# YuePanEdward/MULLS

Measured on AMD Instinct MI355X. Metric: scan-pair registrations/sec (64-beam ~120k pts, 20 ICP iters); dT vs ref, higher is better.
Workload: dtype f32

## Files before the change

### mulls_amd/csrc/batch.cpp

```cpp
#include "batch.h"

namespace mulls_drv
{
void rows12(const double colmajor[16], double out[12])
{
	for (int r = 0; r < 3; r++)
		for (int c = 0; c < 4; c++)
			out[r * 4 + c] = colmajor[r + 4 * c];
}


void fill_crop_box(const RunParams &rp, const double tgt_bound[6], const uint32_t keys[6], mulls_result &R)
{
	R.cropped = rp.crop ? 1 : 0;
	for (int k = 0; k < 3 && rp.crop; k++)
	{
		const uint32_t kmin = keys[k], kmax = keys[3 + k];
		const bool none = kmin == 0xffffffffu && kmax == 0u;
		const double mmin = none ? 1.7976931348623157e308 : (double)ord_to_float(kmin);
		const double mmax = none ? -1.7976931348623157e308 : (double)ord_to_float(kmax);
		const double b1min = tgt_bound[k], b1max = tgt_bound[3 + k];
		const float pad = 1.0f;
		R.crop_box[k] = ((b1min > mmin) ? b1min : mmin) - pad;
		R.crop_box[3 + k] = ((b1max < mmax) ? b1max : mmax) + pad;
// ... 537 lines not shown
			d.src_off = (uint32_t)so;
			d.tgt_off = (uint32_t)to;
			so += d.src_cap;
			to += t.n;
			if (t.n > MULLS_BIG_CLOUD)
			{
				const uint32_t slot = (uint32_t)B->big_clouds_h.size(), first = (uint32_t)B->big_segs_h.size();
				d.big_slot = slot + 1u;
				for (uint32_t k = 0; k < t.n; k += MULLS_SEG)
					B->big_segs_h.push_back({(uint32_t)p, (uint32_t)c, k, slot});
				B->big_clouds_h.push_back({(uint32_t)p, (uint32_t)c, first, (uint32_t)B->big_segs_h.size() - first});
				B->n_big_tgt++;
			}
			if (d.src_cap > MULLS_BIG_CLOUD)
			{
				const uint32_t slot = (uint32_t)B->big_clouds_h.size(), first = (uint32_t)B->big_segs_h.size();
				d.src_big_slot = slot + 1u;
				for (uint32_t k = 0; k < d.src_cap; k += MULLS_SEG)
					B->big_segs_h.push_back({(uint32_t)p, (uint32_t)c | MULLS_BIG_SRC_SIDE, k, slot});
				B->big_clouds_h.push_back({(uint32_t)p, (uint32_t)c | MULLS_BIG_SRC_SIDE, first, (uint32_t)B->big_segs_h.size() - first});
			}
		}
		{
			uint64_t src_total = 0;
			bool seg = false;
			for (int c = 0; c < MULLS_NC; c++)
			{
				const CloudDesc &d = B->descs_h[p * MULLS_NC + c];
				src_total += d.src_n0;
				seg = seg || d.src_big_slot != 0u;
			}
			B->src_one_wg[p] = !seg && src_total <= MULLS_SRC_SETUP_CAP;
		}
		for (int c = 0; c < MULLS_NC; c++)
		{
			const CloudDesc &d = B->descs_h[p * MULLS_NC + c];
			const uint32_t chunks = d.src_cap > 8192u ? 8u : 1u;
			for (uint32_t k = 0; k < d.src_cap; k += MULLS_BLOCK * chunks)
			{
				Job j = {(uint32_t)p, (uint32_t)c, k, chunks};
				(B->src_one_wg[p] ? one_wg_jobs : B->setup_jobs_h).push_back(j);
			}
		}
		rows12(pairs[p].init_guess, B->setup_h[p].guess);
		std::memcpy(B->setup_h[p].tgt_bound, pairs[p].tgt_bound, sizeof(double) * 6);
		{
			Mat4 g;
			std::memcpy(g.v, pairs[p].init_guess, sizeof(g.v));
			const Mat4 gi = mulls::invert4(g);
			mulls::rotation_quaternion(gi, B->setup_h[p].inv_q);
			B->setup_h[p].inv_t[0] = gi.at(0, 3);
			B->setup_h[p].inv_t[1] = gi.at(1, 3);
			B->setup_h[p].inv_t[2] = gi.at(2, 3);
			B->setup_h[p].inv_t[3] = std::acos(std::min(1.0, std::fabs(B->setup_h[p].inv_q[0])));
		}
	}
	B->n_setup_jobs_rest = (uint32_t)B->setup_jobs_h.size();
	B->setup_jobs_h.insert(B->setup_jobs_h.end(), one_wg_jobs.begin(), one_wg_jobs.end());
	if (stage_rec >= (1ull << 32) || so >= (1ull << 31) || to >= (1ull << 31))
	{
		ctx->err = "batch too large (>= 2^31 points)";
		return MULLS_E_INVALID;
	}
	B->n_src = so;
	B->n_tgt = to;

	int rc = MULLS_OK;
	auto A = [&](int r) { if (rc == MULLS_OK) rc = r; };
	bool winner_grew = false, cand_grew = false;
	const size_t SG = (size_t)ctx->opt[MULLS_OPT_STAGGER];
	A(grow(ctx, &B->stage, &B->cap_stage, stage_rec));
	A(grow(ctx, &B->tmp_pos, &B->cap_src[0], so, nullptr, 12 * SG));
	A(grow(ctx, &B->tmp_nrm, &B->cap_src[1], so, nullptr, 13 * SG));
	A(grow(ctx, &B->spos, &B->cap_src[2], so, nullptr, 1 * SG));
	A(grow(ctx, &B->snrm, &B->cap_src[3], so, nullptr, 2 * SG));
	A(grow(ctx, &B->flag, &B->cap_src[4], so, nullptr, 3 * SG));
	A(grow(ctx, &B->match, &B->cap_src[5], so, nullptr, 4 * SG));
	A(grow(ctx, &B->nn_idx, &B->cap_src[6], so, nullptr, 5 * SG));
	A(grow(ctx, &B->wd, &B->cap_src[7], so, nullptr, 6 * SG));
	A(grow(ctx, &B->nn_d2, &B->cap_src[8], so, nullptr, 7 * SG));
	A(grow(ctx, &B->nn_hint, &B->cap_src[9], 2 * so, nullptr, 8 * SG));
	A(grow(ctx, &B->mq, &B->cap_src[10], 2 * so, nullptr, 9 * SG));
	A(grow(ctx, &B->nn_cand, &B->cap_src[11], so, &cand_grew, 14 * SG));
	A(grow(ctx, &B->tpos, &B->cap_tgt[0], to));
	A(grow(ctx, &B->tnrm, &B->cap_tgt[1], to));
	A(grow(ctx, &B->tsorted, &B->cap_tgt[2], to, nullptr, 10 * SG));
	A(grow(ctx, &B->tmap, &B->cap_tgt[4], to, nullptr, 11 * SG));
	A(grow(ctx, &B->winner, &B->cap_tgt[3], to, &winner_grew));
	A(grow(ctx, &B->descs, &B->cap_pairs[0], (size_t)n * MULLS_NC));
	A(grow(ctx, &B->setup, &B->cap_pairs[1], (size_t)n));
	A(grow(ctx, &B->states, &B->cap_pairs[2], (size_t)n));
	A(grow(ctx, &B->outs, &B->cap_outs, (size_t)n));
	A(grow(ctx, &B->bbox, &B->cap_pairs[3], (size_t)n * 6));
	A(grow(ctx, &B->grids, &B->cap_pairs[4], (size_t)n * MULLS_NC));
	A(grow(ctx, &B->setup_jobs, &B->cap_setup_jobs, B->setup_jobs_h.size()));
	A(grow(ctx, &B->big_segs, &B->cap_big[0], B->big_segs_h.size()));
	A(grow(ctx, &B->big_clouds, &B->cap_big[1], B->big_clouds_h.size()));
	A(grow(ctx, &B->seg_cnt, &B->cap_big[2], B->big_segs_h.size()));
	A(grow(ctx, &B->big_box, &B->cap_big[3], (B->big_clouds_h.size() + B->big_segs_h.size()) * 6));
	if (!B->ticket)
	{
		A(dmalloc(ctx, &B->ticket, 32));
		if (rc == MULLS_OK && hipMemset(B->ticket, 0, 32 * sizeof(uint32_t)) != hipSuccess)
			rc = MULLS_E_HIP;
	}
	A(grow_pinned(ctx, &B->states_h, &B->cap_pin[0], (size_t)n, hipHostMallocMapped));
	A(grow_pinned(ctx, &B->outs_h, &B->cap_pin[1], (size_t)n, hipHostMallocMapped));
	A(grow_pinned(ctx, &B->bbox_h, &B->cap_pin[2], (size_t)n * 6, hipHostMallocDefault));
	A(grow_pinned(ctx, &B->upload_h, &B->cap_pin[3], std::max<size_t>(stage_rec, 1) * 16, hipHostMallocDefault));
	if (rc == MULLS_OK && !B->epoch_h)
	{
		if (hipHostMalloc((void **)&B->epoch_h, 256, hipHostMallocMapped) != hipSuccess)
			rc = MULLS_E_HIP;
		else
			std::memset((void *)B->epoch_h, 0, 256);
	}
	if (rc != MULLS_OK)
		return rc;
	if (hipHostGetDevicePointer((void **)&B->states_pin, B->states_h, 0) != hipSuccess ||
		hipHostGetDevicePointer((void **)&B->outs_pin, B->outs_h, 0) != hipSuccess ||
		hipHostGetDevicePointer((void **)&B->epoch_dev, (void *)B->epoch_h, 0) != hipSuccess)
	{
		ctx->err = "pinned host memory setup failed";
		return MULLS_E_HIP;
	}
	std::memset(B->states_h, 0, sizeof(PairState) * n);
	for (int p = 0; p < n; p++)
		for (int k = 0; k < 6; k++)
			B->bbox_h[p * 6 + k] = k < 3 ? 0xffffffffu : 0u;

	struct DevCopy
	{
		size_t dst;
		const void *src;
		size_t bytes;
	};
	std::vector<DevCopy> dev_copies;
	struct HostCopy
	{
		uint8_t *dst;
		const uint8_t *src;
		uint32_t n, stride, fmt;
	};
	std::vector<HostCopy> host_copies;
	std::vector<size_t> first_copy_of_pair(n + 1, 0);
	for (int p = 0; p < n; p++)
	{
		first_copy_of_pair[p] = host_copies.size();
		for (int c = 0; c < MULLS_NC; c++)
		{
			const CloudDesc &d = B->descs_h[p * MULLS_NC + c];
			const mulls_cloud *cl[3] = {&pairs[p].src[c], &pairs[p].tgt[c], &pairs[p].src_down[c]};
			const uint32_t off[3] = {d.src_stage, d.tgt_stage, d.sd_stage}, cnt[3] = {d.src_n0, d.tgt_n0, d.sd_n0};
			const uint32_t fmt[3] = {d.stage_fmt & 3u, (d.stage_fmt >> 2) & 3u, (d.stage_fmt >> 4) & 3u};
			for (int k = 0; k < (d.sd_stage != d.src_stage ? 3 : 2); k++)
			{
				if (!cnt[k])
					continue;
				const uint8_t *src = (const uint8_t *)cl[k]->pts;
				if (fmt[k] == MULLS_STAGE_AOS48)
				{
					if (cl[k]->stride != MULLS_POINT_BYTES)
					{
						ctx->err = "device-resident cloud with stride != 48";
						return MULLS_E_INVALID;
					}
// ... 324 lines not shown
```

### mulls_amd/csrc/batch.h

```cpp
#pragma once
#include <hip/hip_runtime_api.h>

#include <algorithm>
#include <atomic>
#include <chrono>
#include <cmath>
#include <cstdio>
#include <cstdlib>
#include <cstring>
#include <string>
#include <vector>

#include "../../include/mulls_hip.h"
#include "device_types.h"
#include "hostmath.h"
#include "icp_step.h"
#include "launch.h"
#include "ctx.h"

struct SegCopier
{
	mulls_ctx *ctx;
	std::vector<CopySeg> segs;
	struct Pending
	{
		void *dst;
		const void *src;
		size_t bytes;
	};
	std::vector<Pending> host;
	explicit SegCopier(mulls_ctx *c) : ctx(c) {}
	void add_host(void *dst, const void *src, size_t bytes)
	{
		if (bytes)
			host.push_back({dst, src, bytes});
	}
	void add_dev(void *dst, const void *src, size_t bytes)
	{
		const size_t piece = (size_t)0xfffffff0u;
		for (size_t off = 0; off < bytes; off += piece)
		{
			const size_t b = std::min(piece, bytes - off);
			segs.push_back({(unsigned long long)(uintptr_t)dst + off, (unsigned long long)(uintptr_t)src + off, (uint32_t)b, 0u});
		}
	}
	int flush(hipStream_t st);
};

struct mulls_batch : BatchDev
{
	int n = 0;
	size_t n_src = 0, n_tgt = 0;
	std::vector<CloudDesc> descs_h;
	std::vector<PairSetup> setup_h;
	std::vector<Job> setup_jobs_h;
	uint32_t n_setup_jobs_rest = 0;
	std::vector<uint8_t> src_one_wg;
	std::vector<uint32_t> setup_tab_h;
	uint32_t tg_split[MULLS_TG_BUCKETS + 1] = {}, crop_split[4] = {}, srcp_split[2] = {};
	size_t cap_setup_tab = 0;
	std::vector<Job> big_segs_h, big_clouds_h;
	uint32_t n_big_tgt = 0;
	std::vector<Job> jobs_h;
	std::vector<Job> cjobs_h;
	std::vector<Job> cjobs_dev_h;
	std::vector<Job> bjobs_h;
	std::vector<Job> fjobs_h;
	std::vector<Job> ejobs_h;
	std::vector<uint32_t> lclouds_h;
	int tier_mode = -1;
	std::vector<Job> tjobs_h;
	std::vector<uint32_t> ajobs_h;
	uint32_t ajob_split[2][4] = {{0, 0, 0, 0}, {0, 0, 0, 0}};
	IcpOut *icp_outs_pin = nullptr;
	size_t cap_icp_pin = 0;
	std::string jobs_key;
	uint32_t njobs = 0;
	uint4 *nn_cand = nullptr;
	uint32_t tick = 1;
	size_t cap_outs = 0;
	size_t cap_big[4] = {};
	size_t cap_bjobs[4] = {};
	size_t cap_bm_cs = 0;
	size_t cap_bm_rank = 0;
	size_t cap_ajobs = 0;
	size_t cap_icp_outs = 0;
	size_t cap_steps = 0;
	uint32_t epoch2 = 0, epoch3 = 0;
	int nsub = 1;
	double fill_ms = 0.0, fill_pack_ms = 0.0;
	uint64_t fill_bytes = 0;
	size_t cap_wl = 0;
	unsigned long long *dbg = nullptr;
	size_t cap_bm = 0, cap_pf = 0;
	PairState *states_h = nullptr;
	PairOut *outs_h = nullptr;
	volatile uint32_t *epoch_h = nullptr;
	uint32_t *epoch_dev = nullptr;
	uint32_t epoch = 0;
	uint32_t epoch1 = 0;
	uint32_t *bbox_h = nullptr;
	uint8_t *upload_h = nullptr;
	CloudDesc *descs_init = nullptr;
	uint32_t *bbox_init = nullptr;
	std::string dev_key;
	size_t cap_jobs[6] = {}, cap_cells[2] = {};
	size_t cap_stage = 0, cap_src[13] = {}, cap_tgt[5] = {}, cap_pairs[5] = {}, cap_setup_jobs = 0, cap_pin[4] = {};
};

namespace mulls_drv
{
using mulls::Mat4;
using mulls::Mat6;

inline float ord_to_float(uint32_t k)
{
	const uint32_t u = (k & 0x80000000u) ? (k & 0x7fffffffu) : ~k;
	float f;
	std::memcpy(&f, &u, sizeof(f));
	return f;
}
inline int metric_of(int c) { return (c == MULLS_PILLAR || c == MULLS_BEAM) ? 1 : (c == MULLS_VERTEX ? 2 : 0); }
inline int packed(int r, int c) { return r * 6 - r * (r - 1) / 2 + (c - r); }
void rows12(const double colmajor[16], double out[12]);

struct PairHost : mulls::PairIter
{
	bool first = true;
	uint32_t alive_prev[MULLS_NC];
};

void fill_crop_box(const RunParams &rp, const double tgt_bound[6], const uint32_t keys[6], mulls_result &R);
int check_params(mulls_ctx *ctx, const mulls_params *P);
void init_cert(const mulls_ctx *ctx, RunParams &rp);
int subbatch_count(const mulls_ctx *ctx, int n);
void options_init(mulls_ctx *ctx);
bool option_value_ok(int option, double *value);
uint32_t lds_dedup_max_pts();
void assign_tiers(mulls_batch *B, const uint8_t used[MULLS_NC], int mode);
void build_jobs(mulls_batch *B, const mulls_params *P, int nsub, int mode);
int wait_epoch_word(mulls_ctx *ctx, volatile uint32_t *word, uint32_t want, hipEvent_t last = nullptr, hipStream_t stream = nullptr);
inline int wait_epoch(mulls_ctx *ctx, mulls_batch *B) { return wait_epoch_word(ctx, B->epoch_h, B->epoch); }
void unpack_out(const mulls_batch *B, const uint8_t used[MULLS_NC], int p, PairOut &o, bool comb = false);
uint32_t lds_cells_for(uint32_t cap);
int choose_tier(const mulls_ctx *ctx, const mulls_batch *B, const uint8_t used[MULLS_NC], uint32_t *lds_cap, const mulls_params *P_mixed = nullptr);
int batch_fill(mulls_ctx *ctx, mulls_batch *B, const mulls_pair *pairs, int n, const mulls_params *P = nullptr);
int prepare_run(mulls_ctx *ctx, mulls_batch *B, const mulls_params *P_jobs, RunParams &rp, uint32_t *lds_cap_out, int *tier_out, int nsub = 0, bool allow_mixed = false);
void queue_clone_crop(hipStream_t st, const mulls_batch *B, const RunParams &rp);
bool setup_former_shape(const RunParams &rp);
int apply_keep_masks(mulls_ctx *ctx, const mulls_batch *B, const std::vector<uint8_t> &skeep, const std::vector<uint8_t> &tkeep, const char *what);
void queue_target_grids(hipStream_t st, const mulls_batch *B, const RunParams &rp, int tier, bool fused_tgt);
int queue_tier_search(mulls_ctx *ctx, const mulls_batch *B, const RunParams &rp, int tier, uint32_t lds_cap, uint32_t parity);
mulls::IcpConst icp_const(const mulls_params *P);
int take_epochs(mulls_ctx *ctx, mulls_batch *B, uint32_t n, RunParams &rp);

struct EvTimer
{
	mulls_ctx *ctx;
	hipStream_t stream = nullptr;
	int base = 0;
	int used = 0;
// ... 36 lines not shown
```

### mulls_amd/csrc/device_types.h

```cpp
#pragma once
#include <stdint.h>

#define MULLS_NC 6
#define MULLS_NTERM 27
#define MULLS_BLOCK 256
#define MULLS_SRC_PER_THREAD 2
#define MULLS_SRC_PER_BLOCK (MULLS_BLOCK * MULLS_SRC_PER_THREAD)
#define MULLS_NN_BLOCK 128
#define MULLS_NN_PTS 4
#define MULLS_TILE 2048

#define MULLS_MAXCELLS 65536u
#define MULLS_BM_MAXWORDS (1u << 22)
#define MULLS_BM_TOTALWORDS (1u << 28)
#define MULLS_BM_H0 0.25f
#define MULLS_LDS_BLOCK 1024
#define MULLS_LDS_MAXPTS 9728u
#define MULLS_ACC_BLOCK 128
#define MULLS_LDS_QCHUNK 1024u
#define MULLS_LDS_AUX (320u + 2u * MULLS_LDS_QCHUNK)
#define MULLS_CERT_BLOCK 512
#define MULLS_CERT_SMALL 64u
#define MULLS_CERT_SMALL_LOCKSTEP 512u
#define MULLS_LDS_CELL_RESERVE 9216
#ifndef MULLS_LDS_GROUP
#define MULLS_LDS_GROUP 8u
#endif
#define MULLS_TG_BUCKETS 4
#define MULLS_SRC_SETUP_CAP 4096u
#define MULLS_BIG_CLOUD 16384u
#define MULLS_BIG_SRC_SIDE 0x100u
#define MULLS_SEG 4096u
#define MULLS_GRID_GROUP 16u
#define MULLS_BIG_BLOCK 512
#define MULLS_BIG_CLASS_MAX (3u * MULLS_BIG_BLOCK)
#define MULLS_JOB_CLASS 0x80000000u
#define MULLS_SMALL_SRC_MAX 4096u
#define MULLS_TIER_BRUTE 0u
#define MULLS_TIER_BM 1u
#define MULLS_TIER_LDS 2u
#define MULLS_GRID_H0 1.3f

#define MULLS_F_ALIVE 1u
#define MULLS_F_VALID 2u

struct CloudDesc
{
	uint32_t src_stage;
	uint32_t tgt_stage;
	uint32_t src_n0;
	uint32_t tgt_n0;
	uint32_t src_off;
	uint32_t tgt_off;
	uint32_t src_n;
	uint32_t tgt_n;
	uint32_t alive_cur;
	uint32_t alive_next;
	uint32_t n_matched;
	uint32_t valid_next;
	uint32_t n_valid;
	uint32_t job_begin;
	uint32_t job_end;
	uint32_t sd_stage;
	uint32_t sd_n0;
	uint32_t src_cap;
	uint32_t big_slot;
	uint32_t src_big_slot;
	uint32_t n_search;
	uint32_t stage_fmt;
	uint32_t tier;
	uint32_t grid_slot;
};
#define MULLS_STAGE_AOS48 0u
#define MULLS_STAGE_PACK32 1u
#define MULLS_STAGE_PACK28 2u

struct GridDesc
{
	float ox, oy, oz;
	float inv_h, h;
	uint32_t nx, ny, nz;
	uint32_t ncell;
	uint32_t cell_off;
	uint32_t wpr;
	uint32_t nocc;
};

struct PairState
{
	double T[12];
	double x[6];
	float thr[MULLS_NC];
	int32_t iter;
	int32_t active;
	int32_t want_residual;
	int32_t pad_[3];
};

struct PairSetup
{
	double guess[12];
	double tgt_bound[6];
	double inv_q[4];
	double inv_t[4];
};

#define MULLS_NTERM_PAD 28
struct PairOut
{
	double sums[MULLS_NC][MULLS_NTERM_PAD];
	double comb[MULLS_NTERM_PAD];
	uint32_t n_valid[MULLS_NC];
	uint32_t n_alive[MULLS_NC];
	uint32_t src_n[MULLS_NC];
	uint32_t tgt_n[MULLS_NC];
	uint32_t bbox[6];
	uint32_t pad_[2];
};

struct IcpOut
{
	double T[16];
	double info[36];
	double sigma2;
	unsigned long long src_pts, tgt_pts, corr_pts;
	float ratio;
	int32_t code, iters, singular, trace_len;
	uint32_t ncorr[MULLS_NC], nsrc0[MULLS_NC], ntgt0[MULLS_NC], bbox[6];
	uint32_t pad_;
	unsigned long long tgt_job_pts, pair_evals;
};

struct Job
{
	uint32_t pair;
	uint32_t cls;
	uint32_t start;
	uint32_t count;
};

#define MULLS_COPY_SEGS 24
struct CopySeg
{
	unsigned long long dst, src;
	uint32_t bytes, pad_;
};
struct CopyArgs
{
	CopySeg seg[MULLS_COPY_SEGS];
};

struct RunParams
{
	uint8_t used[MULLS_NC];
	uint8_t w_balance, w_resid, w_dist, w_inten;
	uint8_t crop;
	uint8_t undistort;
	uint8_t normal_shooting;
	uint8_t faithful;
	uint8_t rej_strict;
	float z_xy_ratio;
	float win_pt, win_pl, win_li;
	uint8_t force_class_w;
	uint8_t bm_auto;
	float class_w_value;
	double cos_bearing;
	int32_t resid_from_iter;
	uint32_t debug_stop;
	uint32_t cell_stride;
	uint32_t grid_maxcells;
	float grid_h0;
	float bm_h0;
	uint32_t bm_maxwords;
	uint32_t bm_stride;
	uint32_t pull_comb;
	uint32_t lds_dedup;
	uint32_t tick_base;
	uint32_t cert;
	float cert_slack_min, cert_slack_max, cert_slack_rate;
	uint32_t kcert;
	uint32_t kcert_min;
	uint4 *cand;
	const float4 *tgt_stage;
	const uint16_t *tgt_map;
	unsigned long long *dbg_ticks;
};
```

### mulls_amd/csrc/device_util.h

```cpp

#pragma once
#include <hip/hip_runtime.h>
#include <stdint.h>

#include "device_types.h"

#pragma clang fp contract(off)

__device__ __forceinline__ uint32_t xcd_job(uint32_t b, uint32_t n)
{
	const uint32_t q = n >> 3, r = n & 7u, x = b & 7u;
	return x * q + min(x, r) + (b >> 3);
}

namespace
{

typedef float f2 __attribute__((ext_vector_type(2)));

__device__ __forceinline__ uint32_t f2ord(float f)
{
	uint32_t u = __float_as_uint(f);
	return (u & 0x80000000u) ? ~u : (u | 0x80000000u);
}
__device__ __forceinline__ float ord2f(uint32_t k)
{
	uint32_t u = (k & 0x80000000u) ? (k & 0x7fffffffu) : ~k;
	return __uint_as_float(u);
}

__device__ __forceinline__ void load_staged(const float4 *__restrict__ stage, uint32_t off, uint32_t fmt, uint32_t n, uint32_t i, float4 &pos, float4 &nrm)
{
	if (fmt == MULLS_STAGE_PACK32)
	{
		pos = stage[(size_t)off + i];
		nrm = stage[(size_t)off + n + i];
	}
	else if (fmt == MULLS_STAGE_PACK28)
	{
		pos = stage[(size_t)off + i];
		const float *f = reinterpret_cast<const float *>(stage + (size_t)off + n) + 3u * (size_t)i;
		nrm = make_float4(f[0], f[1], f[2], 0.0f);
	}
	else
	{
		const float4 *rec = stage + (size_t)off + (size_t)i * 3;
		const float4 a = rec[0], b = rec[1], c = rec[2];
		pos = make_float4(a.x, a.y, a.z, c.x);
		nrm = make_float4(b.x, b.y, b.z, c.y);
	}
}
__device__ __forceinline__ void identity_step(float4 &p, float4 &n)
{
	const double x = p.x, y = p.y, z = p.z, nx = n.x, ny = n.y, nz = n.z;
	p.x = (float)(1.0 * x + 0.0 * y + 0.0 * z + 0.0);
	p.y = (float)(0.0 * x + 1.0 * y + 0.0 * z + 0.0);
	p.z = (float)(0.0 * x + 0.0 * y + 1.0 * z + 0.0);
	n.x = (float)(1.0 * nx + 0.0 * ny + 0.0 * nz);
	n.y = (float)(0.0 * nx + 1.0 * ny + 0.0 * nz);
	n.z = (float)(0.0 * nx + 0.0 * ny + 1.0 * nz);
}
__device__ __forceinline__ float4 load_staged_pos(const float4 *__restrict__ stage, uint32_t off, uint32_t fmt, uint32_t i)
{
	return fmt == MULLS_STAGE_AOS48 ? stage[(size_t)off + (size_t)i * 3] : stage[(size_t)off + i];
}

__device__ __forceinline__ void tgt_record(const float4 *__restrict__ tgt_stage, const uint16_t *__restrict__ tgt_map, const CloudDesc &d, uint32_t m,
											const float4 *__restrict__ tpos, const float4 *__restrict__ tnrm, float4 &q, float4 &n)
{
	if (tgt_map)
		load_staged(tgt_stage, d.tgt_stage, (d.stage_fmt >> 2) & 3u, d.tgt_n0, tgt_map[d.tgt_off + m], q, n);
	else
		q = tpos[d.tgt_off + m], n = tnrm[d.tgt_off + m];
}
__device__ __forceinline__ float4 tgt_point(const float4 *__restrict__ tgt_stage, const uint16_t *__restrict__ tgt_map, const CloudDesc &d, uint32_t m,
											 const float4 *__restrict__ tpos)
{
	return tgt_map ? load_staged_pos(tgt_stage, d.tgt_stage, (d.stage_fmt >> 2) & 3u, tgt_map[d.tgt_off + m]) : tpos[d.tgt_off + m];
}

__device__ __forceinline__ bool class_called(const RunParams &rp, const CloudDesc &d, int cls)
{
	return rp.used[cls] && d.alive_cur >= 3u && d.tgt_n >= 3u;
}

__device__ __forceinline__ uint32_t block_sum_u32(uint32_t v, uint32_t *lds4)
{
	for (int off = 32; off > 0; off >>= 1)
		v += __shfl_down(v, off);
	int lane = threadIdx.x & 63, wave = threadIdx.x >> 6;
	__syncthreads();
	if (lane == 0)
		lds4[wave] = v;
	__syncthreads();
	return lds4[0] + lds4[1] + lds4[2] + lds4[3];
}

}

namespace
{
__device__ __forceinline__ int grid_cell(float v, float o, float inv_h, uint32_t n)
{
	const float c = floorf((v - o) * inv_h);
	return (int)fminf(fmaxf(c, 0.0f), (float)(n - 1u));
}
__device__ __forceinline__ uint32_t grid_cell_id(const GridDesc &g, float x, float y, float z)
{
	return ((uint32_t)grid_cell(z, g.oz, g.inv_h, g.nz) * g.ny + (uint32_t)grid_cell(y, g.oy, g.inv_h, g.ny)) * g.nx +
		   (uint32_t)grid_cell(x, g.ox, g.inv_h, g.nx);
}
struct BmGrid
{
	const unsigned long long *bm;
	const uint32_t *pf;
	const uint32_t *cs;
};
__device__ __forceinline__ void bm_row_range(const BmGrid &B, uint32_t rowword, uint32_t xa, uint32_t xb, uint32_t &lo, uint32_t &hi)
{
	const uint32_t wa = rowword + (xa >> 6), wb = rowword + (xb >> 6);
	const unsigned long long A = B.bm[wa], Z = B.bm[wb];
	const uint32_t r0 = B.pf[wa] + (uint32_t)__popcll(A & ((1ull << (xa & 63u)) - 1ull));
	const uint32_t r1 = B.pf[wb] + (uint32_t)__popcll(Z & (~0ull >> (63u - (xb & 63u))));
	lo = hi = 0;
	if (r1 > r0)
	{
		lo = B.cs[r0];
		hi = B.cs[r1];
	}
}
__device__ __forceinline__ void grid_scan_box(const GridDesc &g, const BmGrid &B, const float4 *__restrict__ ts,
											   float px, float py, float pz, float R, uint32_t sub, float &best, int &bi)
{
	const float Rm = R * 1.0001f + 1e-4f;
	const int x0 = grid_cell(px - Rm, g.ox, g.inv_h, g.nx), x1 = grid_cell(px + Rm, g.ox, g.inv_h, g.nx);
	const int y0 = grid_cell(py - Rm, g.oy, g.inv_h, g.ny), y1 = grid_cell(py + Rm, g.oy, g.inv_h, g.ny);
	const int z0 = grid_cell(pz - Rm, g.oz, g.inv_h, g.nz), z1 = grid_cell(pz + Rm, g.oz, g.inv_h, g.nz);
	const int nyc = y1 - y0 + 1, nrows = nyc * (z1 - z0 + 1);
	const uint32_t gshift = (threadIdx.x & 63u) & ~(MULLS_GRID_GROUP - 1u);
	for (int base = 0; base < nrows; base += (int)MULLS_GRID_GROUP)
	{
		const int j = base + (int)sub;
		uint32_t lo = 0, hi = 0;
		if (j < nrows)
		{
			const uint32_t rowword = ((uint32_t)(z0 + j / nyc) * g.ny + (uint32_t)(y0 + j % nyc)) * g.wpr;
			bm_row_range(B, rowword, (uint32_t)x0, (uint32_t)x1, lo, hi);
		}
		const uint32_t nonempty = (uint32_t)(__ballot(hi > lo) >> gshift) & 0xffffu;
		if (!nonempty)
			continue;
#pragma unroll
		for (int half = 0; half < 2; half++)
		{
			if (!((nonempty >> (8 * half)) & 0xffu))
				continue;
			float4 q[8];
			bool ok[8];
#pragma unroll
			for (int jj = 0; jj < 8; jj++)
			{
				const uint32_t t = __shfl(lo, 8 * half + jj, MULLS_GRID_GROUP) + sub;
// ... 122 lines not shown
```

### mulls_amd/csrc/driver.cpp

```cpp
#include "batch.h"

#include <sched.h>
#include <cstdio>
#include <cstdlib>

#include <mutex>
#include <unordered_map>
namespace
{
std::mutex g_stagger_mu;
std::unordered_map<void *, void *> g_stagger;
}
void staggered_note(void *p, void *base)
{
	std::lock_guard<std::mutex> lk(g_stagger_mu);
	g_stagger[p] = base;
}
void *staggered_base(void *p, bool forget)
{
	std::lock_guard<std::mutex> lk(g_stagger_mu);
	auto it = g_stagger.find(p);
	if (it == g_stagger.end())
		return p;
	void *b = it->second;
// ... 233 lines not shown
		while (!ctx->blocks.empty())
			mulls_block_destroy(ctx, ctx->blocks.back());
		for (auto &e : ctx->ev)
			if (e)
				(void)hipEventDestroy(e);
		if (ctx->ev_setup)
			(void)hipEventDestroy(ctx->ev_setup);
		if (ctx->stream2)
			(void)hipStreamDestroy(ctx->stream2);
		if (ctx->stream)
			(void)hipStreamDestroy(ctx->stream);
		delete ctx;
	}

	const char *mulls_last_error(const mulls_ctx *ctx) { return ctx ? ctx->err.c_str() : "null context"; }

	int mulls_set_profiling(mulls_ctx *ctx, int on)
	try
	{
		if (!ctx)
			return MULLS_E_INVALID;
		ctx->profiling = on == 2 ? 2 : (on != 0 ? 1 : 0);
		return MULLS_OK;
	}
	catch (...)
	{
		return mulls::abi_caught(const_cast<mulls_ctx *>(ctx));
	}

	int mulls_get_profile(const mulls_ctx *ctx, mulls_profile *out)
	try
	{
		if (!ctx || !out)
			return MULLS_E_INVALID;
		*out = ctx->prof;
		return MULLS_OK;
	}
	catch (...)
	{
		return mulls::abi_caught(const_cast<mulls_ctx *>(ctx));
	}

	void *mulls_stream(mulls_ctx *ctx) { return ctx ? (void *)ctx->stream : nullptr; }

	int mulls_set_option(mulls_ctx *ctx, int option, double value)
	{
		if (!ctx || !option_known(option))
			return MULLS_E_INVALID;
		if (!option_value_ok(option, &value))
		{
			ctx->err = "mulls_set_option: value out of the option's range";
			return MULLS_E_INVALID;
		}
		ctx->opt[option] = value;
		return MULLS_OK;
	}
	int mulls_get_option(const mulls_ctx *ctx, int option, double *value)
	{
		if (!ctx || !value || !option_known(option))
			return MULLS_E_INVALID;
		*value = ctx->opt[option];
		return MULLS_OK;
	}

	int mulls_set_nn_mode(mulls_ctx *ctx, int mode)
	try
	{
		if (!ctx || mode < 0 || mode > 4)
			return MULLS_E_INVALID;
		ctx->nn_mode = mode;
		return MULLS_OK;
	}
	catch (...)
	{
		return mulls::abi_caught(const_cast<mulls_ctx *>(ctx));
	}

	void mulls_batch_destroy(mulls_ctx *ctx, mulls_batch *B)
	{
		if (!B)
			return;
		if (ctx)
			(void)hipSetDevice(ctx->device);
		void *dev[] = {B->stage, B->tmp_pos, B->tmp_nrm, B->spos, B->snrm, B->tpos, B->tnrm, B->flag, B->match, B->nn_idx, B->nn_hint, B->nn_cand, B->mq, B->wd,
					   B->nn_d2, B->winner, B->descs, B->setup, B->states, B->outs, B->ticket, B->bbox, B->setup_jobs, B->big_segs, B->big_clouds, B->seg_cnt, B->big_box, B->jobs, B->partial,
					   B->tjobs, B->cjobs, B->bjobs, B->fjobs, B->ejobs, B->lclouds, B->bm_cs, B->wl, B->wl_ctr, B->grids, B->tsorted, B->tmap, B->dbg, B->cell_cnt, B->cell_start, B->bm, B->pf, B->descs_init, B->bbox_init,
					   B->ajobs, B->icp_outs, B->steps, B->bm_rank, B->setup_tab};
		for (void *p : dev)
			if (p)
				staggered_free(p);
		if (B->states_h)
			(void)hipHostFree(B->states_h);
		if (B->outs_h)
			(void)hipHostFree(B->outs_h);
		if (B->bbox_h)
			(void)hipHostFree(B->bbox_h);
		if (B->epoch_h)
			(void)hipHostFree((void *)B->epoch_h);
		if (B->upload_h)
			(void)hipHostFree(B->upload_h);
		if (B->icp_outs_pin)
			(void)hipHostFree(B->icp_outs_pin);
		delete B;
	}

	int mulls_batch_create(mulls_ctx *ctx, const mulls_pair *pairs, int n, mulls_batch **out)
	try
	{
		if (!ctx || !pairs || n <= 0 || !out)
			return MULLS_E_INVALID;
		*out = nullptr;
		mulls_batch *B = new mulls_batch();
		const int rc = batch_fill(ctx, B, pairs, n);
		if (rc != MULLS_OK)
		{
			mulls_batch_destroy(ctx, B);
			return rc;
		}
		*out = B;
		return MULLS_OK;
	}
	catch (...)
	{
		return mulls::abi_caught(const_cast<mulls_ctx *>(ctx));
	}


	int mulls_icp_batch(mulls_ctx *ctx, const mulls_pair *pairs, int n, const mulls_params *params, mulls_result *results)
	try
	{
		if (!ctx)
			return MULLS_E_INVALID;
		int rc = check_params(ctx, params);
		if (rc != MULLS_OK)
			return rc;
		if (!pairs || n <= 0 || !results)
			return MULLS_E_INVALID;
		if (!ctx->scratch)
			ctx->scratch = new mulls_batch();
		rc = batch_fill(ctx, ctx->scratch, pairs, n, params);
		if (rc != MULLS_OK)
			return rc;
		rc = mulls_batch_run(ctx, ctx->scratch, params, results);
		ctx->prof.ms_stage = ctx->scratch->fill_ms, ctx->prof.ms_stage_pack = ctx->scratch->fill_pack_ms, ctx->prof.stage_bytes = ctx->scratch->fill_bytes;
		return rc;
	}
	catch (...)
	{
		return mulls::abi_caught(const_cast<mulls_ctx *>(ctx));
	}

	int mulls_icp(mulls_ctx *ctx, const mulls_pair *pair, const mulls_params *params, mulls_result *result)
	try
	{
		return mulls_icp_batch(ctx, pair, 1, params, result);
	}
	catch (...)
	{
		return mulls::abi_caught(const_cast<mulls_ctx *>(ctx));
	}

}
```

### mulls_amd/csrc/k_reduce.hip

```cpp
#include "device_util.h"
#include "accum.h"
#include "solve_wave.h"

template <int LANES, int MIN_WG>
__global__ __launch_bounds__(LANES, MIN_WG) void k_accum(const uint32_t *__restrict__ leaders, const Job *__restrict__ jobs, const CloudDesc *__restrict__ descs,
														 const PairState *__restrict__ states, RunParams rp, const float4 *__restrict__ spos,
														 const float4 *__restrict__ mq, const uint8_t *__restrict__ flag, float *__restrict__ wd,
														 double *__restrict__ partial)
{
	extern __shared__ __attribute__((aligned(16))) unsigned char lds_raw[];
	__shared__ double part[MULLS_NTERM_PAD];
	const uint32_t job_idx = leaders[xcd_job(blockIdx.x, gridDim.x)];
	const Job job = jobs[job_idx];
	const PairState &ps = states[job.pair];
	if (!ps.active && !ps.want_residual)
		return;
	const CloudDesc *pd = descs + job.pair * MULLS_NC;
	const bool residual_pass = ps.want_residual != 0;
	int cnt[MULLS_NC];
	for (int c = 0; c < MULLS_NC; c++)
		cnt[c] = (int)(class_called(rp, pd[c], c) ? pd[c].valid_next : pd[c].n_valid);
	const AccumCtx A = accum_ctx(rp, job.cls, ps.iter, residual_pass, class_weight(rp, job.cls, residual_pass, cnt));
	trip_sum<true, LANES>(A, ps.x, pd[job.cls], job.start, spos, mq, flag, wd, lds_raw, part);
	if (threadIdx.x < MULLS_NTERM)
		partial[(size_t)job_idx * MULLS_NTERM + threadIdx.x] = part[threadIdx.x];
}

namespace
{
template <typename TS, int W0, int WIN, int MODE, int METRIC, int A0>
__device__ __forceinline__ void add_window(const AccumCtx &A, const double *x, const float4 P, const float4 Q, const float4 N, float wi, float &w, double *acc, const float *wpre)
{
	TS t[WIN];
#pragma unroll
	for (int k = 0; k < WIN; k++)
		t[k] = (TS)0;
	point_terms<TS, W0, WIN, MODE, METRIC>(A, x, P, Q, N, wi, w, t, wpre);
#pragma unroll
	for (int k = 0; k < WIN; k++)
		acc[W0 - A0 + k] += (double)t[k];
}
#ifndef MULLS_ACCW_WIN
#define MULLS_ACCW_WIN 9
#endif
#ifndef MULLS_ACCW_WIN_D
#define MULLS_ACCW_WIN_D 12
#endif
template <typename TS, int W0, int REM, int MODE, int METRIC, int A0>
__device__ __forceinline__ void add_windows(const AccumCtx &A, const double *x, const float4 P, const float4 Q, const float4 N, float wi, float &w, double *acc, const float *wpre)
{
	constexpr int WMAX = sizeof(TS) == 8 ? MULLS_ACCW_WIN_D : MULLS_ACCW_WIN;
	constexpr int WIN = REM < WMAX ? REM : WMAX;
	add_window<TS, W0, WIN, MODE, METRIC, A0>(A, x, P, Q, N, wi, w, acc, wpre);
	if constexpr (REM > WIN)
		add_windows<TS, W0 + WIN, REM - WIN, MODE, METRIC, A0>(A, x, P, Q, N, wi, w, acc, wpre);
}
template <typename TS, int NT, int MODE, int METRIC, int T0, int NTW>
__device__ __forceinline__ void wave_trip(const AccumCtx &A, const double *x, const CloudDesc &d, uint32_t trip0, const float4 *__restrict__ spos, const float4 *__restrict__ mq,
										   const uint8_t *__restrict__ flag, float *__restrict__ wd, double *__restrict__ out, bool owner)
{
	const uint32_t lane = threadIdx.x & 63u;
	const uint32_t src_n = d.src_n, src_off = d.src_off;
	const uint32_t n_here = min(src_n - trip0, (uint32_t)MULLS_ACC_LANES), iters = (n_here + 63u) >> 6;
	const uint32_t last = src_off + src_n - 1u;
	struct Rec
	{
		uint32_t f;
		float4 P, Q;
		float3 N;
		float w;
	};
	const bool need_w = A.residual_pass, writes_w = !A.residual_pass && (METRIC != 2 || !A.faithful);
	auto load = [&](uint32_t i) {
		Rec r;
		const uint32_t g = min(src_off + trip0 + lane + 64u * i, last);
		r.f = flag[g];
		r.P = spos[g], r.Q = mq[2u * g], r.N = *reinterpret_cast<const float3 *>(mq + 2u * g + 1u);
		r.w = need_w ? wd[g] : 0.0f;
		return r;
	};
	double acc[NTW];
#pragma unroll
	for (int k = 0; k < NTW; k++)
		acc[k] = -0.0;
#define MULLS_PIN_REC(r) asm volatile("" : "+v"((r).f), "+v"((r).P.x), "+v"((r).Q.x), "+v"((r).N.x), "+v"((r).w))
#if MULLS_ACCW_PREFETCH
	Rec cur = load(0);
#endif
	for (uint32_t i = 0; i < iters; i++)
	{
#if MULLS_ACCW_PREFETCH
		MULLS_PIN_REC(cur);
		Rec nxt = cur;
		if (i + 1u < iters)
			nxt = load(i + 1u);
#else
		Rec cur = load(i);
		MULLS_PIN_REC(cur);
#endif
		const uint32_t s = trip0 + lane + 64u * i;
		const bool valid = s < src_n && (cur.f & (MULLS_F_ALIVE | MULLS_F_VALID)) == (MULLS_F_ALIVE | MULLS_F_VALID);
		if (valid)
		{
			float w = cur.w;
			const float4 N4 = make_float4(cur.N.x, cur.N.y, cur.N.z, 0.0f);
			const float wi = (A.inten_w && !A.residual_pass) ? point_wi(cur.P, cur.Q) : 1.0f;
			const float wpre = A.residual_pass ? 0.0f : corr_weight(A, METRIC, cur.P, cur.Q, N4, wi);
			add_windows<TS, T0, NTW, MODE, METRIC, T0>(A, x, cur.P, cur.Q, N4, wi, w, acc, A.residual_pass ? nullptr : &wpre);
			if (owner && writes_w)
				wd[src_off + s] = w;
		}
#if MULLS_ACCW_PREFETCH
		cur = nxt;
#endif
	}
	if (NTW == NT && lane < MULLS_NTERM)
	{
		const bool has = MODE == 1 ? li_slot((int)lane) >= 0 : (int)lane < NT;
		if (!has)
			out[lane] = 0.0;
	}
#pragma unroll
	for (int k = 0; k < NTW; k++)
	{
		double sum = acc[k];
		sum = dpp_add_f64<0xB1>(sum);
		sum = dpp_add_f64<0x4E>(sum);
		sum = dpp_add_f64<0x141>(sum);
		sum = dpp_add_f64<0x140>(sum);
		sum = dpp_add_f64_rows<0x142, 0xa>(sum);
		sum = dpp_add_f64_rows<0x143, 0xc>(sum);
		acc[k] = sum;
	}
	if (lane == 63u)
	{
#pragma unroll
		for (int k = 0; k < NTW; k++)
			out[MODE == 1 ? li_term(T0 + k) : T0 + k] = acc[k];
	}
}
}

#ifndef MULLS_ACCW_SPLIT
#define MULLS_ACCW_SPLIT 1
#endif
#ifndef MULLS_ACCW_PREFETCH
#define MULLS_ACCW_PREFETCH 0
#endif
#ifndef MULLS_ACCW_OCC
#define MULLS_ACCW_OCC 4
#endif
#define MULLS_ACCW_WAVES 4
__global__ __launch_bounds__(64 * MULLS_ACCW_WAVES, MULLS_ACCW_OCC) void k_accum_wave(const uint32_t *__restrict__ leaders, uint32_t n_trips, const Job *__restrict__ jobs,
																					   const CloudDesc *__restrict__ descs, const PairState *__restrict__ states, RunParams rp,
																					   const float4 *__restrict__ spos, const float4 *__restrict__ mq, const uint8_t *__restrict__ flag,
																					   float *__restrict__ wd, double *__restrict__ partial)
{
	const uint32_t wave = threadIdx.x >> 6, part = wave % MULLS_ACCW_SPLIT;
	const uint32_t trip = blockIdx.x * (MULLS_ACCW_WAVES / MULLS_ACCW_SPLIT) + wave / MULLS_ACCW_SPLIT;
	if (trip >= n_trips)
		return;
	const uint32_t job_idx = leaders[trip];
	const Job job = jobs[job_idx];
	const PairState &ps = states[job.pair];
	if (!ps.active && !ps.want_residual)
		return;
	const CloudDesc *pd = descs + job.pair * MULLS_NC;
	const bool residual_pass = ps.want_residual != 0;
	int cnt[MULLS_NC];
	for (int c = 0; c < MULLS_NC; c++)
		cnt[c] = (int)(class_called(rp, pd[c], c) ? pd[c].valid_next : pd[c].n_valid);
	const AccumCtx A = accum_ctx(rp, job.cls, ps.iter, residual_pass, class_weight(rp, job.cls, residual_pass, cnt));
	const CloudDesc &d = pd[job.cls];
	double *out = partial + (size_t)job_idx * MULLS_NTERM;
	if (d.src_n <= job.start)
	{
		if (part == 0u && (threadIdx.x & 63u) < MULLS_NTERM)
			out[threadIdx.x & 63u] = 0.0;
		return;
	}
	if (residual_pass || A.metric == 1)
	{
		if (part)
			return;
		if (!residual_pass)
			wave_trip<double, 12, 1, 1, 0, 12>(A, ps.x, d, job.start, spos, mq, flag, wd, out, true);
		else if (A.metric == 0)
			wave_trip<double, 2, 0, 0, 0, 2>(A, ps.x, d, job.start, spos, mq, flag, wd, out, true);
		else if (A.metric == 1)
			wave_trip<double, 2, 0, 1, 0, 2>(A, ps.x, d, job.start, spos, mq, flag, wd, out, true);
		else
			wave_trip<double, 2, 0, 2, 0, 2>(A, ps.x, d, job.start, spos, mq, flag, wd, out, true);
	}
#if MULLS_ACCW_SPLIT == 2
	else if (A.metric == 0)
	{
		if (part == 0u)
			wave_trip<float, 27, 0, 0, 0, 14>(A, ps.x, d, job.start, spos, mq, flag, wd, out, true);
		else
			wave_trip<float, 27, 0, 0, 14, 13>(A, ps.x, d, job.start, spos, mq, flag, wd, out, false);
	}
	else
	{
		if (part == 0u)
			wave_trip<float, 27, 0, 2, 0, 14>(A, ps.x, d, job.start, spos, mq, flag, wd, out, true);
		else
			wave_trip<float, 27, 0, 2, 14, 13>(A, ps.x, d, job.start, spos, mq, flag, wd, out, false);
	}
#else
	else if (A.metric == 0)
		wave_trip<float, 27, 0, 0, 0, 27>(A, ps.x, d, job.start, spos, mq, flag, wd, out, true);
	else
		wave_trip<float, 27, 0, 2, 0, 27>(A, ps.x, d, job.start, spos, mq, flag, wd, out, true);
#endif
}

namespace
{
struct FinishLds
{
	double sums[MULLS_NC][MULLS_NTERM_PAD], comb[MULLS_NTERM_PAD];
	uint32_t cnt[32];
};
__device__ __forceinline__ void finish_pair(CloudDesc *pd, const PairState &ps, const RunParams &rp, const double *__restrict__ partial,
											 PairOut &o, const uint32_t *__restrict__ pair_bbox, FinishLds *M = nullptr)
{
	if (threadIdx.x >= 192 && threadIdx.x < 198)
	{
		const uint32_t v = pair_bbox[threadIdx.x - 192];
		o.bbox[threadIdx.x - 192] = v;
		if (M)
			M->cnt[24 + threadIdx.x - 192] = v;
	}
	if (threadIdx.x < MULLS_NC * MULLS_NTERM)
	{
		const int c = threadIdx.x / MULLS_NTERM, t = threadIdx.x % MULLS_NTERM;
		if (rp.used[c])
		{
			constexpr uint32_t STEP = MULLS_ACC_LANES / MULLS_SRC_PER_BLOCK;
			double sum = 0.0;
			uint32_t j = pd[c].job_begin;
			const uint32_t je = pd[c].job_end;
			for (; j + 32u * STEP <= je; j += 32u * STEP)
			{
				double v[32];
#pragma unroll
				for (uint32_t k = 0; k < 32u; k++)
					v[k] = partial[(size_t)(j + k * STEP) * MULLS_NTERM + t];
#pragma unroll
				for (uint32_t k = 0; k < 32u; k++)
					sum += v[k];
			}
			for (; j + 16u * STEP <= je; j += 16u * STEP)
			{
				double v[16];
#pragma unroll
				for (uint32_t k = 0; k < 16u; k++)
					v[k] = partial[(size_t)(j + k * STEP) * MULLS_NTERM + t];
#pragma unroll
				for (uint32_t k = 0; k < 16u; k++)
					sum += v[k];
			}
			for (; j < je; j += STEP)
				sum += partial[(size_t)j * MULLS_NTERM + t];
			o.sums[c][t] = sum;
			if (M)
				M->sums[c][t] = sum;
		}
	}
	__syncthreads();
	if (rp.pull_comb && threadIdx.x >= 64 && threadIdx.x < 64 + MULLS_NTERM)
	{
		if (M)
		{
			combine_rows(rp, ps.want_residual != 0, M->sums, M->comb, (int)threadIdx.x - 64);
			o.comb[threadIdx.x - 64] = M->comb[threadIdx.x - 64];
		}
		else
			combine_rows(rp, ps.want_residual != 0, o.sums, o.comb, (int)threadIdx.x - 64);
	}
	if (threadIdx.x < MULLS_NC)
	{
		const int c = threadIdx.x;
		CloudDesc &d = pd[c];
		if (ps.active)
		{
			if (class_called(rp, d, c))
			{
				d.n_valid = d.valid_next;
				d.alive_cur = d.alive_next;
			}
			d.alive_next = 0;
			d.valid_next = 0;
			d.n_matched = 0;
		}
		o.n_valid[c] = d.n_valid;
// ... 411 lines not shown
	__syncthreads();
	if (threadIdx.x < MULLS_NTERM_PAD)
		L.comb[threadIdx.x] = F.comb[threadIdx.x];
	else if (threadIdx.x >= 64u && threadIdx.x < 94u)
		L.cnt[threadIdx.x - 64u] = F.cnt[threadIdx.x - 64u];
	const bool left = step_pair(pair, descs, states, rp, K, out, steps, results, brute, L, sw);
	if (threadIdx.x == 0)
	{
		unsigned long long *t64 = reinterpret_cast<unsigned long long *>(ticket);
		const unsigned long long old = atomicAdd(t64, ((unsigned long long)(left ? 1u : 0u) << 32) | 1ull);
		if ((uint32_t)old == gridDim.x - 1u)
		{
			const uint32_t n_left = (uint32_t)(old >> 32) + (left ? 1u : 0u);
			*t64 = 0ull;
			__threadfence_system();
			*host_word = (unsigned long long)epoch << 32 | n_left;
		}
	}
}

__global__ __launch_bounds__(1024) void k_step_publish(const PairState *__restrict__ states, uint32_t npairs, volatile unsigned long long *host_word, uint32_t epoch)
{
	int mine = 0;
	for (uint32_t p = threadIdx.x; p < npairs; p += 1024u)
		mine += (states[p].active || states[p].want_residual) ? 1 : 0;
	__shared__ uint32_t s_left;
	if (threadIdx.x == 0)
		s_left = 0u;
	__syncthreads();
	for (int off = 32; off > 0; off >>= 1)
		mine += __shfl_down(mine, off);
	if ((threadIdx.x & 63u) == 0u && mine)
		atomicAdd(&s_left, (uint32_t)mine);
	__syncthreads();
	if (threadIdx.x == 0)
	{
		__threadfence_system();
		*host_word = (unsigned long long)epoch << 32 | s_left;
	}
}

static_assert(sizeof(PairState) % 16 == 0, "PairState must be a whole number of uint4 words");
__global__ void k_push_states(const uint4 *__restrict__ host_words, uint4 *__restrict__ dev_words, uint32_t nwords)
{
	const uint32_t i = blockIdx.x * blockDim.x + threadIdx.x;
	if (i < nwords)
		dev_words[i] = host_words[i];
}

__global__ void k_transform_aos(float4 *__restrict__ recs, uint32_t n, const double *__restrict__ T )
{
	const uint32_t i = blockIdx.x * blockDim.x + threadIdx.x;
	if (i >= n)
		return;
	float4 a = recs[(size_t)i * 3], b = recs[(size_t)i * 3 + 1];
	double x = a.x, y = a.y, z = a.z, nx = b.x, ny = b.y, nz = b.z;
	a.x = (float)(T[0] * x + T[1] * y + T[2] * z + T[3]);
	a.y = (float)(T[4] * x + T[5] * y + T[6] * z + T[7]);
	a.z = (float)(T[8] * x + T[9] * y + T[10] * z + T[11]);
	b.x = (float)(T[0] * nx + T[1] * ny + T[2] * nz);
	b.y = (float)(T[4] * nx + T[5] * ny + T[6] * nz);
	b.z = (float)(T[8] * nx + T[9] * ny + T[10] * nz);
	recs[(size_t)i * 3] = a;
	recs[(size_t)i * 3 + 1] = b;
}

__global__ void k_set_corr(uint32_t src_off, const int32_t *__restrict__ cs, const int32_t *__restrict__ ct, const float *__restrict__ cd,
						   uint32_t n, uint8_t *__restrict__ flag, int32_t *__restrict__ match, float *__restrict__ wd, uint32_t tgt_off,
						   const float4 *__restrict__ tpos, const float4 *__restrict__ tnrm, float4 *__restrict__ mq)
{
	const uint32_t i = blockIdx.x * blockDim.x + threadIdx.x;
	if (i >= n)
		return;
	const uint32_t g = src_off + (uint32_t)cs[i];
	flag[g] = MULLS_F_ALIVE | MULLS_F_VALID;
	match[g] = ct[i];
	mq[2u * g] = tpos[tgt_off + (uint32_t)ct[i]];
	mq[2u * g + 1u] = tnrm[tgt_off + (uint32_t)ct[i]];
	wd[g] = cd ? cd[i] : 0.0f;
}

#include "launch.h"

void launch_accum(hipStream_t st, const BatchDev &b, const RunParams &rp, const uint32_t split[4], bool single, uint32_t wave_min_trips)
{
	(void)dev_launch<3>([](DevLaunch &) {
		return hipFuncSetAttribute(reinterpret_cast<const void *>(k_accum<1024, 2>), hipFuncAttributeMaxDynamicSharedMemorySize, (int)MULLS_RED_BYTES_HALF) == hipSuccess;
	});
	const uint32_t n_trips = split[3] - split[0];
	if (wave_min_trips && n_trips >= wave_min_trips && rp.faithful && rp.pull_comb)
	{
		hipLaunchKernelGGL(k_accum_wave, dim3((n_trips + MULLS_ACCW_WAVES / MULLS_ACCW_SPLIT - 1u) / (MULLS_ACCW_WAVES / MULLS_ACCW_SPLIT)), dim3(64 * MULLS_ACCW_WAVES), 0, st, b.ajobs + split[0], n_trips, b.jobs, b.descs, b.states, rp, b.spos,
						   b.mq, b.flag, b.wd, b.partial);
		return;
	}
	if (single)
	{
		if (split[3] > split[0])
			hipLaunchKernelGGL((k_accum<1024, 2>), dim3(split[3] - split[0]), dim3(1024), MULLS_RED_BYTES_HALF, st, b.ajobs + split[0], b.jobs, b.descs, b.states, rp, b.spos, b.mq,
							   b.flag, b.wd, b.partial);
		return;
	}
	if (split[1] > split[0])
		hipLaunchKernelGGL((k_accum<1024, 2>), dim3(split[1] - split[0]), dim3(1024), MULLS_RED_BYTES_HALF, st, b.ajobs + split[0], b.jobs, b.descs, b.states, rp, b.spos, b.mq, b.flag,
						   b.wd, b.partial);
	if (split[2] > split[1])
		hipLaunchKernelGGL((k_accum<512, 4>), dim3(split[2] - split[1]), dim3(512), MULLS_RED_BYTES_HALF / 2, st, b.ajobs + split[1], b.jobs, b.descs, b.states, rp, b.spos, b.mq, b.flag,
						   b.wd, b.partial);
	if (split[3] > split[2])
		hipLaunchKernelGGL((k_accum<256, 8>), dim3(split[3] - split[2]), dim3(256), MULLS_RED_BYTES_HALF / 4, st, b.ajobs + split[2], b.jobs, b.descs, b.states, rp, b.spos, b.mq, b.flag,
						   b.wd, b.partial);
}

void launch_finish(hipStream_t st, const BatchDev &b, const RunParams &rp, uint32_t pair_base, uint32_t npairs, uint32_t *ticket, volatile uint32_t *host_epoch, uint32_t epoch)
{
	if (!npairs)
		return;
	const bool direct = rp.pull_comb && npairs <= 64u;
	hipLaunchKernelGGL(k_finish, dim3(npairs), dim3(MULLS_BLOCK), 0, st, b.descs, b.states, rp, b.partial, b.outs, b.bbox, pair_base,
					   direct ? reinterpret_cast<uint4 *>(b.outs_pin) : nullptr, ticket, host_epoch, epoch);
	if (direct)
		return;
	uint32_t n_used = 0;
	for (int c = 0; c < MULLS_NC; c++)
		n_used += rp.used[c] ? 1u : 0u;
	const uint32_t nwords = npairs * (8u + (MULLS_NTERM_PAD / 2u) * (rp.pull_comb ? 1u : n_used));
	hipLaunchKernelGGL(k_pull_outs, dim3((nwords + MULLS_BLOCK - 1) / MULLS_BLOCK), dim3(MULLS_BLOCK), 0, st, reinterpret_cast<const uint4 *>(b.outs),
					   reinterpret_cast<uint4 *>(b.outs_pin), rp, pair_base, npairs, ticket, host_epoch, epoch);
}

void launch_step_init(hipStream_t st, const BatchDev &b, const mulls::IcpConst &K, uint32_t npairs)
{
	if (npairs)
		hipLaunchKernelGGL(k_step_init, dim3((npairs + 63u) / 64u), dim3(64), 0, st, npairs, b.setup, K, b.steps, b.states);
}

void launch_finish_step(hipStream_t st, const BatchDev &b, const RunParams &rp, const mulls::IcpConst &K, uint32_t pair_base, uint32_t npairs, unsigned long long *host_word, uint32_t epoch,
						int brute, uint32_t *ticket, bool sum_step)
{
	if (!npairs)
		return;
	if (ticket)
	{
		hipLaunchKernelGGL(k_finish_step, dim3(npairs), dim3(MULLS_BLOCK), 0, st, b.descs, b.states, rp, K, b.partial, b.outs, b.bbox, b.steps, b.icp_outs, brute, ticket, host_word, epoch,
						   pair_base);
		return;
	}
	if (sum_step && rp.pull_comb)
		hipLaunchKernelGGL(k_sum_step, dim3(npairs), dim3(64), 0, st, b.descs, b.states, rp, K, b.partial, b.outs, b.bbox, b.steps, b.icp_outs, brute, pair_base);
	else
	{
		hipLaunchKernelGGL(k_finish, dim3(npairs), dim3(MULLS_BLOCK), 0, st, b.descs, b.states, rp, b.partial, b.outs, b.bbox, pair_base, static_cast<uint4 *>(nullptr),
						   static_cast<uint32_t *>(nullptr), static_cast<volatile uint32_t *>(nullptr), 0u);
		hipLaunchKernelGGL(k_step, dim3(npairs), dim3(64), 0, st, b.descs, b.states, rp, K, b.outs, b.steps, b.icp_outs, brute, pair_base);
	}
	hipLaunchKernelGGL(k_step_publish, dim3(1), dim3(1024), 0, st, b.states + pair_base, npairs, host_word, epoch);
}

void launch_push_states(hipStream_t st, const BatchDev &b, uint32_t pair_base, uint32_t npairs)
{
	const PairState *host_states = b.states_pin + pair_base;
	PairState *dev_states = b.states + pair_base;
	const uint32_t nwords = npairs * (uint32_t)(sizeof(PairState) / 16);
	if (nwords)
		hipLaunchKernelGGL(k_push_states, dim3((nwords + 255) / 256), dim3(256), 0, st, reinterpret_cast<const uint4 *>(host_states),
						   reinterpret_cast<uint4 *>(dev_states), nwords);
}

void launch_transform_aos(hipStream_t st, float4 *recs, uint32_t n, const double *T12)
{
	if (n)
		hipLaunchKernelGGL(k_transform_aos, dim3((n + 255) / 256), dim3(256), 0, st, recs, n, T12);
}
// ... 7 lines not shown
```

### mulls_amd/csrc/k_search.hip

```cpp
#include "device_util.h"
#include "lds_tier.h"
#include "big_tier.h"

template <int NPTS>
__device__ __forceinline__ void nn_scan_group(const float *__restrict__ X, const float *__restrict__ Y, const float *__restrict__ Z, uint32_t j,
											   const float (&px)[NPTS], const float (&py)[NPTS], const float (&pz)[NPTS], float (&best)[NPTS],
											   uint32_t (&grp)[NPTS], uint32_t gidx)
{
	const float4 x0 = *reinterpret_cast<const float4 *>(X + j), x1 = *reinterpret_cast<const float4 *>(X + j + 4);
	const float4 y0 = *reinterpret_cast<const float4 *>(Y + j), y1 = *reinterpret_cast<const float4 *>(Y + j + 4);
	const float4 z0 = *reinterpret_cast<const float4 *>(Z + j), z1 = *reinterpret_cast<const float4 *>(Z + j + 4);
	const float tx[8] = {x0.x, x0.y, x0.z, x0.w, x1.x, x1.y, x1.z, x1.w};
	const float ty[8] = {y0.x, y0.y, y0.z, y0.w, y1.x, y1.y, y1.z, y1.w};
	const float tz[8] = {z0.x, z0.y, z0.z, z0.w, z1.x, z1.y, z1.z, z1.w};
#pragma unroll
	for (int u = 0; u < NPTS; u++)
	{
		float dd[8];
#pragma unroll
		for (int v = 0; v < 8; v++)
		{
			const float dx = px[u] - tx[v], dy = py[u] - ty[v], dz = pz[u] - tz[v];
			dd[v] = (dx * dx + dy * dy) + dz * dz;
		}
// ... 251 lines not shown
	const Job job = cjobs[blockIdx.x];
	const PairState &ps = states[job.pair];
	if (!ps.active || (rp.normal_shooting && (job.cls == 0 || job.cls == 2 || job.cls == 4)))
		return;
	CloudDesc &d = descs[job.pair * MULLS_NC + job.cls];
	const GridDesc g = grids[job.pair * MULLS_NC + job.cls];
	__shared__ CertLds<MULLS_CERT_SMALL> s_cert;
	const bool direct = first && first_goes_direct(rp, d, job.cls);
	if (!direct)
	{
		if (cert_job<MULLS_LDS_BLOCK, MULLS_CERT_SMALL, true, 3>(s_cert, rp, ps, job, d, g, reinterpret_cast<uint32_t *>(lds_raw), spos, snrm, cell_start, tsorted, flag, nn_idx, nn_d2, winner,
																 tnrm, match, wd, tpos, nn_hint, mq, fused_park(lds_raw, cap)))
			return;
		__syncthreads();
	}
	lds_search_class(rp, ps, job, d, g, lds_layout(lds_raw, cap, rp.grid_maxcells), lds_raw, spos, snrm, cell_start, tsorted, flag, nn_idx, nn_d2, winner, tnrm, match,
					 wd, tpos, nn_hint, mq, direct);
}

__global__ __launch_bounds__(MULLS_LDS_BLOCK) void k_cert_mixed(uint32_t n_lds, const Job *__restrict__ cjobs, const Job *__restrict__ bjobs, uint32_t split,
																 CloudDesc *__restrict__ descs, const PairState *__restrict__ states, RunParams rp, float4 *__restrict__ spos,
																 float4 *__restrict__ snrm, const GridDesc *__restrict__ grids, const uint32_t *__restrict__ cell_start,
																 const unsigned long long *__restrict__ bm, const uint32_t *__restrict__ pf, const uint32_t *__restrict__ cs,
																 const float4 *__restrict__ tsorted, uint8_t *flag, int32_t *__restrict__ nn_idx, float *__restrict__ nn_d2,
																 unsigned long long *__restrict__ winner, const float4 *__restrict__ tnrm, int32_t *__restrict__ match,
																 float *__restrict__ wd, const float4 *__restrict__ tpos, int32_t *__restrict__ nn_hint, float4 *__restrict__ mq, uint32_t cap,
																 uint32_t first)
{
	extern __shared__ __attribute__((aligned(16))) unsigned char lds_raw[];
	if (blockIdx.x < n_lds)
	{
		const Job job = cjobs[blockIdx.x];
		const PairState &ps = states[job.pair];
		if (!ps.active)
			return;
		CloudDesc &d = descs[job.pair * MULLS_NC + job.cls];
		const GridDesc g = grids[job.pair * MULLS_NC + job.cls];
		__shared__ CertLds<MULLS_CERT_SMALL> s_cert;
		const bool direct = first && first_goes_direct(rp, d, job.cls);
		if (!direct)
		{
			if (cert_job<MULLS_LDS_BLOCK, MULLS_CERT_SMALL, true, 3>(s_cert, rp, ps, job, d, g, reinterpret_cast<uint32_t *>(lds_raw), spos, snrm, cell_start, tsorted, flag, nn_idx, nn_d2,
																	 winner, tnrm, match, wd, tpos, nn_hint, mq, fused_park(lds_raw, cap)))
				return;
			__syncthreads();
		}
		lds_search_class(rp, ps, job, d, g, lds_layout(lds_raw, cap, rp.grid_maxcells), lds_raw, spos, snrm, cell_start, tsorted, flag, nn_idx, nn_d2, winner, tnrm, match, wd, tpos,
						 nn_hint, mq, direct);
		return;
	}
	if (threadIdx.x >= MULLS_BIG_BLOCK)
		return;
	const uint32_t wg = blockIdx.x - n_lds;
	const Job job = bjobs[wg / split];
	const uint32_t part = wg % split;
	const PairState &ps = states[job.pair];
	if (!ps.active)
		return;
	const uint32_t ci = job.pair * MULLS_NC + job.cls;
	CloudDesc &d = descs[ci];
	const bool class_level = (job.count & MULLS_JOB_CLASS) != 0u;
	const uint32_t cnt = (job.count & ~MULLS_JOB_CLASS) ? (job.count & ~MULLS_JOB_CLASS) : (uint32_t)MULLS_SRC_PER_BLOCK;
	uint32_t q0, q1;
	if (class_level)
	{
		if (part)
			return;
		q0 = 0u, q1 = min(d.src_n, cnt);
	}
	else
	{
		const uint32_t per = cnt / split;
		q0 = job.start + part * per, q1 = min(d.src_n, q0 + per);
		if (q0 >= q1)
			return;
	}
	const GridDesc g = grids[ci];
	const BmGrid B = {bm + g.cell_off, pf + g.cell_off, cs + d.tgt_off + ci};
	cert_big<MULLS_BIG_BLOCK, 3>(*reinterpret_cast<BigLds<MULLS_BIG_BLOCK * 3> *>(lds_raw), rp, ps, job.cls, q0, q1, class_level, d, g, B, tsorted + d.tgt_off, spos, snrm, flag, nn_idx,
								 nn_d2, winner, tnrm, match, wd, tpos, reinterpret_cast<int2 *>(nn_hint), mq);
}

__global__ __launch_bounds__(MULLS_LDS_BLOCK) void k_nn_lds(const Job *__restrict__ cjobs, CloudDesc *__restrict__ descs,
															 const PairState *__restrict__ states, RunParams rp, const float4 *__restrict__ spos,
															 const float4 *__restrict__ snrm, const GridDesc *__restrict__ grids,
															 const uint32_t *__restrict__ cell_start, const float4 *__restrict__ tsorted,
															 uint8_t *flag, int32_t *__restrict__ nn_idx, float *__restrict__ nn_d2,
															 unsigned long long *__restrict__ winner, const float4 *__restrict__ tnrm, int32_t *__restrict__ match,
															 float *__restrict__ wd, const float4 *__restrict__ tpos, int32_t *__restrict__ nn_hint, float4 *__restrict__ mq,
															 uint32_t cap, const uint32_t *__restrict__ wl, uint32_t *__restrict__ wl_ctr, uint32_t parity, uint32_t first_njobs)
{
	extern __shared__ __attribute__((aligned(16))) unsigned char lds_raw[];
	const LdsLayout Y = lds_layout(lds_raw, cap, rp.grid_maxcells);

	const uint32_t n_queued = first_njobs ? first_njobs : wl_ctr[2u * parity];
	for (;;)
	{
		__syncthreads();
		if (threadIdx.x == 0)
			Y.HIST[65] = atomicAdd(&wl_ctr[2u * parity + 1u], 1u);
		__syncthreads();
		const uint32_t ticket = Y.HIST[65];
		if (ticket >= n_queued)
			return;
		const Job job = cjobs[first_njobs ? ticket : wl[ticket]];
		CloudDesc &d = descs[job.pair * MULLS_NC + job.cls];
		if (first_njobs && !(states[job.pair].active && first_goes_direct(rp, d, job.cls)))
			continue;
		lds_search_class(rp, states[job.pair], job, d, grids[job.pair * MULLS_NC + job.cls], Y, lds_raw, spos, snrm, cell_start, tsorted, flag, nn_idx, nn_d2, winner, tnrm,
						 match, wd, tpos, nn_hint, mq, first_njobs != 0u);
	}
}

__global__ __launch_bounds__(MULLS_BLOCK) void k_nn_shoot(const Job *__restrict__ jobs, CloudDesc *__restrict__ descs,
														   const PairState *__restrict__ states, RunParams rp, float4 *__restrict__ spos,
														   float4 *__restrict__ snrm, const float4 *__restrict__ tpos,
														   const uint8_t *__restrict__ flag, int32_t *__restrict__ nn_idx, float *__restrict__ nn_d2,
														   unsigned long long *__restrict__ winner)
{
	__shared__ float4 tile[1024];
	const Job job = jobs[blockIdx.x];
	if (!(job.cls == 0 || job.cls == 2 || job.cls == 4))
		return;
	const PairState &ps = states[job.pair];
	if (!ps.active)
		return;
	CloudDesc &d = descs[job.pair * MULLS_NC + job.cls];
	const uint32_t src_n = d.src_n, tgt_n = d.tgt_n, alive_cur = d.alive_cur;
	const bool called = class_called(rp, d, job.cls);
	const float r = 2.5f * ps.thr[job.cls];
	const double max_distance = (double)r;
	const bool gate = alive_cur >= 500u;
	const unsigned long long key_hi = (unsigned long long)(0xffffffffu - (rp.tick_base + (uint32_t)ps.iter)) << 32;
	uint32_t matched_cnt = 0;
	for (int u = 0; u < MULLS_SRC_PER_THREAD; u++)
	{
		const uint32_t s = job.start + threadIdx.x + u * MULLS_BLOCK;
		const bool alive = s < src_n && (flag[d.src_off + s] & MULLS_F_ALIVE);
		float px = 0, py = 0, pz = 0, nx = 0, ny = 0, nz = 0;
		if (alive)
		{
			const float4 p = spos[d.src_off + s], n = snrm[d.src_off + s];
			const double *T = ps.T;
			const double x = p.x, y = p.y, z = p.z, ax = n.x, ay = n.y, az = n.z;
			px = (float)(T[0] * x + T[1] * y + T[2] * z + T[3]);
			py = (float)(T[4] * x + T[5] * y + T[6] * z + T[7]);
			pz = (float)(T[8] * x + T[9] * y + T[10] * z + T[11]);
			nx = (float)(T[0] * ax + T[1] * ay + T[2] * az);
			ny = (float)(T[4] * ax + T[5] * ay + T[6] * az);
			nz = (float)(T[8] * ax + T[9] * ay + T[10] * az);
			spos[d.src_off + s] = make_float4(px, py, pz, p.w);
			snrm[d.src_off + s] = make_float4(nx, ny, nz, n.w);
		}
		if (!called)
			continue;
		float kd[10];
		int ki[10];
#pragma unroll
		for (int j = 0; j < 10; j++)
		{
			kd[j] = __builtin_inff();
			ki[j] = 0x7fffffff;
		}
		for (uint32_t base = 0; base < tgt_n; base += 1024)
		{
			const uint32_t nt = min(1024u, tgt_n - base);
			__syncthreads();
			for (uint32_t k = threadIdx.x; k < nt; k += MULLS_BLOCK)
// ... 198 lines not shown
```

### mulls_amd/csrc/k_setup.hip

```cpp
#include "device_util.h"
#include "crop_grid.h"
#include "detmath.h"
#include "scan_math.h"

__global__ __launch_bounds__(MULLS_BLOCK) void k_clone_src(const Job *__restrict__ jobs, const CloudDesc *__restrict__ descs,
															const PairSetup *__restrict__ setup, const float4 *__restrict__ stage,
															float4 *__restrict__ tmp_pos, float4 *__restrict__ tmp_nrm,
															uint32_t *__restrict__ bbox , RunParams rp)
{
	__shared__ uint32_t box_red[MULLS_BLOCK / 64][6];
	const Job job = jobs[blockIdx.x];
	const CloudDesc &d = descs[job.pair * MULLS_NC + job.cls];
	const bool regen = rp.undistort && job.cls != 5;
	const uint32_t n_in = regen ? d.sd_n0 : d.src_n0;
	const PairSetup &su = setup[job.pair];
	const double *G = su.guess;
	uint32_t k[6] = {0xffffffffu, 0xffffffffu, 0xffffffffu, 0u, 0u, 0u};
	const uint32_t reps = job.count ? job.count : 1u;
	for (uint32_t rep_chunk = 0; rep_chunk < reps; rep_chunk++)
	{
		const uint32_t s = job.start + rep_chunk * MULLS_BLOCK + threadIdx.x;
		if (s >= n_in)
			continue;
		float x = 0, y = 0, z = 0;
// ... 121 lines not shown
			{
				load_staged(stage, d.tgt_stage, (d.stage_fmt >> 2) & 3u, d.tgt_n0, i, p, q);
			}
			else
			{
				p = tmp_pos[off + i];
				q = tmp_nrm[off + i];
			}
		}
		bool keep = in;
		if (crop && in)
			keep = crop_keep(p, lo, hi);
		const unsigned long long bal = __ballot(keep);
		const uint32_t before = __popcll(bal & ((1ull << lane) - 1ull));
		__syncthreads();
		if (lane == 0)
			wave_cnt[wave] = __popcll(bal);
		__syncthreads();
		uint32_t wbase = 0, total = 0;
		for (int w = 0; w < 4; w++)
		{
			if (w < wave)
				wbase += wave_cnt[w];
			total += wave_cnt[w];
		}
		if (keep)
		{
			const uint32_t dst = off + running + wbase + before;
			if (side)
			{
				tpos[dst] = p;
				tnrm[dst] = q;
				if (fabsf(p.x) <= 1.0e18f && fabsf(p.y) <= 1.0e18f && fabsf(p.z) <= 1.0e18f)
				{
					bmin[0] = fminf(bmin[0], p.x), bmin[1] = fminf(bmin[1], p.y), bmin[2] = fminf(bmin[2], p.z);
					bmax[0] = fmaxf(bmax[0], p.x), bmax[1] = fmaxf(bmax[1], p.y), bmax[2] = fmaxf(bmax[2], p.z);
				}
			}
			else
			{
				identity_step(p, q);
				spos[dst] = p;
				snrm[dst] = q;
				flag[dst] = MULLS_F_ALIVE;
				match[dst] = -1;
				wd[dst] = 0.0f;
			}
		}
		running += total;
	}
	if (side && grids)
	{
		for (int k = 0; k < 3; k++)
			for (int off = 32; off > 0; off >>= 1)
			{
				bmin[k] = fminf(bmin[k], __shfl_down(bmin[k], off));
				bmax[k] = fmaxf(bmax[k], __shfl_down(bmax[k], off));
			}
		__syncthreads();
		if (lane == 0)
			for (int k = 0; k < 3; k++)
			{
				box_red[wave][k] = bmin[k];
				box_red[wave][3 + k] = bmax[k];
			}
		__syncthreads();
		if (threadIdx.x == 0)
		{
			float lo3[3], hi3[3];
			for (int k = 0; k < 3; k++)
			{
				lo3[k] = fminf(fminf(box_red[0][k], box_red[1][k]), fminf(box_red[2][k], box_red[3][k]));
				hi3[k] = fmaxf(fmaxf(box_red[0][3 + k], box_red[1][3 + k]), fmaxf(box_red[2][3 + k], box_red[3][3 + k]));
			}
			grids[pair * MULLS_NC + cls] = make_grid(lo3, hi3, running, rp, d, cls);
		}
	}
	if (threadIdx.x == 0)
	{
		if (side)
			d.tgt_n = running;
		else
		{
			d.src_n = running;
			d.alive_cur = running;
			d.alive_next = 0;
			d.n_matched = 0;
			d.valid_next = 0;
			d.n_valid = 0;
		}
	}
}

#define MULLS_SS_LANES 512u
#define MULLS_SS_WAVES (MULLS_SS_LANES / 64u)
#define MULLS_SS_TRIPS (MULLS_SRC_SETUP_CAP / MULLS_SS_LANES)
static_assert(MULLS_SS_TRIPS * MULLS_SS_WAVES == 64u, "one wave scans the (trip, wave) counts, one per lane");
__global__ __launch_bounds__(MULLS_SS_LANES, 4) void k_src_setup(const uint32_t *__restrict__ pairs, CloudDesc *__restrict__ descs, const PairSetup *__restrict__ setup,
																	const float4 *__restrict__ stage, float4 *__restrict__ spos, float4 *__restrict__ snrm, uint8_t *__restrict__ flag,
																	int32_t *__restrict__ match, float *__restrict__ wd, uint32_t *__restrict__ bbox, RunParams rp)
{
	__shared__ uint32_t first[MULLS_NC + 1];
	__shared__ uint32_t c_stage[MULLS_NC], c_fmt[MULLS_NC], c_off[MULLS_NC];
	__shared__ uint32_t ucnt[MULLS_SS_TRIPS * MULLS_SS_WAVES];
	__shared__ uint32_t box_red[MULLS_SS_WAVES][6];
	__shared__ uint32_t box_keys[6];
	__shared__ uint32_t cls_base[MULLS_NC + 1];
	const uint32_t pair = pairs[blockIdx.x];
	CloudDesc *pd = descs + (size_t)pair * MULLS_NC;
	const int lane = threadIdx.x & 63, wave = threadIdx.x >> 6;
	if (threadIdx.x == 0)
	{
		uint32_t at = 0;
		for (int c = 0; c < MULLS_NC; c++)
		{
			first[c] = at;
			at += pd[c].src_n0;
			c_stage[c] = pd[c].src_stage, c_fmt[c] = pd[c].stage_fmt & 3u, c_off[c] = pd[c].src_off;
		}
		first[MULLS_NC] = at;
	}
	__syncthreads();
	uint32_t st_[MULLS_NC + 1];
	for (int c = 0; c <= MULLS_NC; c++)
		st_[c] = first[c];
	const uint32_t total = st_[MULLS_NC];
	const PairSetup &su = setup[pair];
	const double *G = su.guess;
	float4 a[MULLS_SS_TRIPS], b[MULLS_SS_TRIPS];
	uint32_t clsmask = 0;
#pragma unroll
	for (uint32_t t = 0; t < MULLS_SS_TRIPS; t++)
	{
		const uint32_t s = t * MULLS_SS_LANES + threadIdx.x;
		uint32_t c = 0;
		for (int k = 1; k < MULLS_NC; k++)
			c += s >= st_[k] ? 1u : 0u;
		clsmask |= c << (3u * t);
		a[t] = b[t] = make_float4(0, 0, 0, 0);
		if (s < total)
			load_staged(stage, c_stage[c], c_fmt[c], first[c + 1] - first[c], s - first[c], a[t], b[t]);
	}
	__builtin_amdgcn_sched_barrier(0);
	uint32_t k6[6] = {0xffffffffu, 0xffffffffu, 0xffffffffu, 0u, 0u, 0u};
#pragma unroll
	for (uint32_t t = 0; t < MULLS_SS_TRIPS; t++)
	{
		const uint32_t s = t * MULLS_SS_LANES + threadIdx.x, c = (clsmask >> (3u * t)) & 7u;
		if (s < total)
		{
			const double px = a[t].x, py = a[t].y, pz = a[t].z, nx = b[t].x, ny = b[t].y, nz = b[t].z;
			const float x = (float)(G[0] * px + G[1] * py + G[2] * pz + G[3]);
			const float y = (float)(G[4] * px + G[5] * py + G[6] * pz + G[7]);
			const float z = (float)(G[8] * px + G[9] * py + G[10] * pz + G[11]);
			const float onx = (float)(G[0] * nx + G[1] * ny + G[2] * nz);
			const float ony = (float)(G[4] * nx + G[5] * ny + G[6] * nz);
			const float onz = (float)(G[8] * nx + G[9] * ny + G[10] * nz);
			a[t] = make_float4(x, y, z, a[t].w);
			b[t] = make_float4(onx, ony, onz, b[t].w);
			if (c <= 2u)
			{
				k6[0] = min(k6[0], f2ord(x)), k6[1] = min(k6[1], f2ord(y)), k6[2] = min(k6[2], f2ord(z));
				k6[3] = max(k6[3], f2ord(x)), k6[4] = max(k6[4], f2ord(y)), k6[5] = max(k6[5], f2ord(z));
			}
		}
	}
	for (int off = 32; off > 0; off >>= 1)
		for (int j = 0; j < 3; j++)
		{
			k6[j] = min(k6[j], (uint32_t)__shfl_down(k6[j], off));
			k6[3 + j] = max(k6[3 + j], (uint32_t)__shfl_down(k6[3 + j], off));
		}
	if (lane == 0)
		for (int j = 0; j < 6; j++)
			box_red[wave][j] = k6[j];
	__syncthreads();
	if (threadIdx.x < 6)
	{
		uint32_t v = box_red[0][threadIdx.x];
		for (uint32_t w = 1; w < MULLS_SS_WAVES; w++)
			v = threadIdx.x < 3 ? min(v, box_red[w][threadIdx.x]) : max(v, box_red[w][threadIdx.x]);
		box_keys[threadIdx.x] = v;
		bbox[pair * 6 + threadIdx.x] = v;
	}
	__syncthreads();
	double lo[3], hi[3];
	if (rp.crop)
		crop_box_keys(box_keys, su, lo, hi);
	uint32_t keepmask = 0;
#pragma unroll
	for (uint32_t t = 0; t < MULLS_SS_TRIPS; t++)
	{
		const uint32_t s = t * MULLS_SS_LANES + threadIdx.x;
		const bool keep = s < total && (!rp.crop || crop_keep(a[t], lo, hi));
		const unsigned long long bal = __ballot(keep);
		keepmask |= keep ? (1u << t) : 0u;
		if (lane == 0)
			ucnt[t * MULLS_SS_WAVES + (uint32_t)wave] = (uint32_t)__popcll(bal);
	}
	__syncthreads();
	if (wave == 0)
	{
		const uint32_t v = ucnt[lane];
		uint32_t incl = v;
		for (int off = 1; off < 64; off <<= 1)
		{
			const uint32_t o = __shfl_up(incl, off);
			if (lane >= off)
				incl += o;
		}
		ucnt[lane] = incl - v;
		if (lane == 63)
		{
			for (int c = 0; c <= MULLS_NC; c++)
				if (st_[c] >= total)
					cls_base[c] = incl;
		}
	}
	__syncthreads();
	uint32_t rank[MULLS_SS_TRIPS];
#pragma unroll
	for (uint32_t t = 0; t < MULLS_SS_TRIPS; t++)
	{
		const uint32_t s = t * MULLS_SS_LANES + threadIdx.x;
		const bool keep = (keepmask >> t) & 1u;
		rank[t] = ucnt[t * MULLS_SS_WAVES + (uint32_t)wave] + (uint32_t)__popcll(__ballot(keep) & ((1ull << lane) - 1ull));
		if (s < total)
			for (int c = 0; c < MULLS_NC; c++)
				if (s == st_[c])
					cls_base[c] = rank[t];
	}
	__syncthreads();
#pragma unroll
	for (uint32_t t = 0; t < MULLS_SS_TRIPS; t++)
		if ((keepmask >> t) & 1u)
		{
			const uint32_t c = (clsmask >> (3u * t)) & 7u;
			const uint32_t dst = c_off[c] + rank[t] - cls_base[c];
			float4 p = a[t], q = b[t];
			identity_step(p, q);
			spos[dst] = p;
			snrm[dst] = q;
			flag[dst] = MULLS_F_ALIVE;
			match[dst] = -1;
			wd[dst] = 0.0f;
		}
	if (threadIdx.x < MULLS_NC)
	{
		CloudDesc &d = pd[threadIdx.x];
		const uint32_t n = cls_base[threadIdx.x + 1] - cls_base[threadIdx.x];
		d.src_n = n;
		d.alive_cur = n;
		d.alive_next = 0;
		d.n_matched = 0;
		d.valid_next = 0;
		d.n_valid = 0;
	}
}

__global__ __launch_bounds__(MULLS_BLOCK) void k_crop_big_count(const Job *__restrict__ segs, const CloudDesc *__restrict__ descs,
																 const PairSetup *__restrict__ setup, const uint32_t *__restrict__ bbox,
																 const float4 *__restrict__ stage, const float4 *__restrict__ tmp_pos, RunParams rp,
																 uint32_t *__restrict__ seg_cnt, uint32_t *__restrict__ seg_box)
{
	__shared__ uint32_t red4[4];
	const Job sg = segs[blockIdx.x];
	const uint32_t cls = sg.cls & 0xffu;
	const bool src_side = (sg.cls & MULLS_BIG_SRC_SIDE) != 0u;
	const CloudDesc &d = descs[sg.pair * MULLS_NC + cls];
	const uint32_t n0 = src_side ? ((rp.undistort && cls != 5u) ? d.sd_n0 : d.src_n0) : d.tgt_n0;
	double lo[3], hi[3];
	if (rp.crop)
		crop_box(sg.pair, bbox, setup, lo, hi);
	uint32_t mine = 0;
	float bmin[3] = {__builtin_inff(), __builtin_inff(), __builtin_inff()}, bmax[3] = {-__builtin_inff(), -__builtin_inff(), -__builtin_inff()};
	for (uint32_t k = 0; k < MULLS_SEG; k += MULLS_BLOCK)
	{
		const uint32_t i = sg.start + k + threadIdx.x;
		if (i < n0)
		{
			const float4 p = src_side ? tmp_pos[d.src_off + i] : load_staged_pos(stage, d.tgt_stage, (d.stage_fmt >> 2) & 3u, i);
			if (!rp.crop || crop_keep(p, lo, hi))
			{
				mine++;
				if (fabsf(p.x) <= 1.0e18f && fabsf(p.y) <= 1.0e18f && fabsf(p.z) <= 1.0e18f)
				{
					bmin[0] = fminf(bmin[0], p.x), bmin[1] = fminf(bmin[1], p.y), bmin[2] = fminf(bmin[2], p.z);
					bmax[0] = fmaxf(bmax[0], p.x), bmax[1] = fmaxf(bmax[1], p.y), bmax[2] = fmaxf(bmax[2], p.z);
				}
			}
		}
	}
	__shared__ uint32_t box4[4][6];
	for (int k = 0; k < 3; k++)
	{
		for (int off = 32; off > 0; off >>= 1)
		{
			bmin[k] = fminf(bmin[k], __shfl_down(bmin[k], off));
			bmax[k] = fmaxf(bmax[k], __shfl_down(bmax[k], off));
		}
		if ((threadIdx.x & 63) == 0)
		{
			const bool any = bmin[k] <= bmax[k];
			box4[threadIdx.x >> 6][k] = any ? f2ord(bmin[k]) : 0xffffffffu;
			box4[threadIdx.x >> 6][3 + k] = any ? f2ord(bmax[k]) : 0u;
		}
	}
	const uint32_t total = block_sum_u32(mine, red4);
	if (threadIdx.x == 0)
		seg_cnt[blockIdx.x] = total;
	if (threadIdx.x < 6 && !src_side)
	{
		const uint32_t k = threadIdx.x;
		const uint32_t a = box4[0][k], b = box4[1][k], c = box4[2][k], e = box4[3][k];
		seg_box[(size_t)blockIdx.x * 6u + k] = k < 3 ? min(min(a, b), min(c, e)) : max(max(a, b), max(c, e));
	}
}

__global__ __launch_bounds__(64) void k_crop_big_scan(const Job *__restrict__ clouds, CloudDesc *__restrict__ descs, RunParams rp,
													   uint32_t *__restrict__ seg_cnt, const uint32_t *__restrict__ seg_box,
													   GridDesc *__restrict__ grids)
{
	const Job bc = clouds[blockIdx.x];
	const bool want_box = !(bc.cls & MULLS_BIG_SRC_SIDE) && grids != nullptr;
	uint32_t running = 0;
	uint32_t box[6] = {0xffffffffu, 0xffffffffu, 0xffffffffu, 0u, 0u, 0u};
	for (uint32_t base = 0; base < bc.count; base += 64)
	{
		const uint32_t s = base + threadIdx.x;
		if (want_box && s < bc.count)
			for (int k = 0; k < 6; k++)
			{
				const uint32_t b = seg_box[(size_t)(bc.start + s) * 6u + k];
				box[k] = k < 3 ? min(box[k], b) : max(box[k], b);
			}
		const uint32_t v = s < bc.count ? seg_cnt[bc.start + s] : 0u;
		uint32_t incl = v;
		for (int off = 1; off < 64; off <<= 1)
		{
			const uint32_t o = __shfl_up(incl, off);
			if ((int)threadIdx.x >= off)
				incl += o;
		}
		if (s < bc.count)
			seg_cnt[bc.start + s] = running + incl - v;
		running += __shfl(incl, 63);
	}
	if (want_box)
		for (int k = 0; k < 6; k++)
			for (int off = 32; off > 0; off >>= 1)
			{
				const uint32_t o = (uint32_t)__shfl_down((int)box[k], off);
				box[k] = k < 3 ? min(box[k], o) : max(box[k], o);
			}
	if (threadIdx.x == 0 && (bc.cls & MULLS_BIG_SRC_SIDE))
	{
		CloudDesc &d = descs[bc.pair * MULLS_NC + (bc.cls & 0xffu)];
		d.src_n = running;
		d.alive_cur = running;
		d.alive_next = 0;
		d.n_matched = 0;
		d.valid_next = 0;
		d.n_valid = 0;
	}
	else if (threadIdx.x == 0)
	{
		descs[bc.pair * MULLS_NC + bc.cls].tgt_n = running;
		if (grids)
		{
			float lo3[3], hi3[3];
			for (int k = 0; k < 3; k++)
			{
				lo3[k] = running ? ord2f(box[k]) : __builtin_inff();
				hi3[k] = running ? ord2f(box[3 + k]) : -__builtin_inff();
			}
			grids[bc.pair * MULLS_NC + bc.cls] = make_grid(lo3, hi3, running, rp, descs[bc.pair * MULLS_NC + bc.cls], bc.cls);
		}
	}
}

__global__ __launch_bounds__(MULLS_BLOCK) void k_crop_big_scatter(const Job *__restrict__ segs, const CloudDesc *__restrict__ descs,
																   const PairSetup *__restrict__ setup, const uint32_t *__restrict__ bbox,
																   const float4 *__restrict__ stage, RunParams rp,
																   const uint32_t *__restrict__ seg_base, float4 *__restrict__ tpos,
																   float4 *__restrict__ tnrm, const float4 *__restrict__ tmp_pos, const float4 *__restrict__ tmp_nrm,
																   float4 *__restrict__ spos, float4 *__restrict__ snrm, uint8_t *__restrict__ flag,
																   int32_t *__restrict__ match, float *__restrict__ wd)
{
	__shared__ uint32_t wave_cnt[4];
	const Job sg = segs[blockIdx.x];
	const uint32_t cls = sg.cls & 0xffu;
	const bool src_side = (sg.cls & MULLS_BIG_SRC_SIDE) != 0u;
	const CloudDesc &d = descs[sg.pair * MULLS_NC + cls];
	const uint32_t n0 = src_side ? ((rp.undistort && cls != 5u) ? d.sd_n0 : d.src_n0) : d.tgt_n0;
	double lo[3], hi[3];
	if (rp.crop)
		crop_box(sg.pair, bbox, setup, lo, hi);
	const int lane = threadIdx.x & 63, wave = threadIdx.x >> 6;
	uint32_t running = seg_base[blockIdx.x];
	for (uint32_t k = 0; k < MULLS_SEG; k += MULLS_BLOCK)
	{
		const uint32_t i = sg.start + k + threadIdx.x;
		bool keep = false;
		float4 p = make_float4(0, 0, 0, 0), q = make_float4(0, 0, 0, 0);
		if (i < n0)
		{
			if (src_side)
				p = tmp_pos[d.src_off + i], q = tmp_nrm[d.src_off + i];
			else
				load_staged(stage, d.tgt_stage, (d.stage_fmt >> 2) & 3u, d.tgt_n0, i, p, q);
			keep = !rp.crop || crop_keep(p, lo, hi);
		}
		const unsigned long long bal = __ballot(keep);
		const uint32_t before = __popcll(bal & ((1ull << lane) - 1ull));
		__syncthreads();
		if (lane == 0)
			wave_cnt[wave] = __popcll(bal);
		__syncthreads();
		uint32_t wbase = 0, total = 0;
		for (int w = 0; w < 4; w++)
		{
			if (w < wave)
				wbase += wave_cnt[w];
			total += wave_cnt[w];
		}
		if (keep && src_side)
		{
			const uint32_t dst = d.src_off + running + wbase + before;
			identity_step(p, q);
			spos[dst] = p;
			snrm[dst] = q;
			flag[dst] = MULLS_F_ALIVE;
			match[dst] = -1;
			wd[dst] = 0.0f;
		}
		else if (keep)
		{
			tpos[d.tgt_off + running + wbase + before] = p;
			tnrm[d.tgt_off + running + wbase + before] = q;
		}
		running += total;
	}
}

__global__ __launch_bounds__(MULLS_BLOCK) void k_thin(CloudDesc *__restrict__ descs, const uint8_t *__restrict__ src_keep,
													   const uint8_t *__restrict__ tgt_keep, float4 *__restrict__ spos, float4 *__restrict__ snrm,
													   float4 *__restrict__ tpos, float4 *__restrict__ tnrm)
{
	__shared__ uint32_t wave_cnt[4];
	const uint32_t pair = blockIdx.x / (MULLS_NC * 2);
	const uint32_t cls = (blockIdx.x / 2) % MULLS_NC;
	const uint32_t side = blockIdx.x & 1;
	CloudDesc &d = descs[pair * MULLS_NC + cls];
	const uint32_t n0 = side ? d.tgt_n : d.src_n;
	const uint32_t off = side ? d.tgt_off : d.src_off;
	const uint8_t *keepm = (side ? tgt_keep : src_keep) + off;
	float4 *pos = side ? tpos : spos, *nrm = side ? tnrm : snrm;
	const int lane = threadIdx.x & 63, wave = threadIdx.x >> 6;
	uint32_t running = 0;
	for (uint32_t base = 0; base < n0; base += MULLS_BLOCK)
	{
		const uint32_t i = base + threadIdx.x;
		const bool in = i < n0;
		float4 p = make_float4(0, 0, 0, 0), q = make_float4(0, 0, 0, 0);
		bool keep = false;
		if (in)
		{
			p = pos[off + i];
			q = nrm[off + i];
			keep = keepm[i] != 0;
		}
		const unsigned long long bal = __ballot(keep);
		const uint32_t before = __popcll(bal & ((1ull << lane) - 1ull));
		__syncthreads();
		if (lane == 0)
			wave_cnt[wave] = __popcll(bal);
		__syncthreads();
		uint32_t wbase = 0, total = 0;
		for (int w = 0; w < 4; w++)
		{
			if (w < wave)
				wbase += wave_cnt[w];
			total += wave_cnt[w];
		}
		if (keep)
		{
			const uint32_t dst = off + running + wbase + before;
			pos[dst] = p;
			nrm[dst] = q;
		}
		running += total;
	}
	if (threadIdx.x == 0)
	{
		if (side)
			d.tgt_n = running;
		else
		{
			d.src_n = running;
			d.alive_cur = running;
		}
	}
}

using mulls::scan::MotionComp;
__global__ __launch_bounds__(MULLS_BLOCK) void k_motion_comp(float4 *__restrict__ recs, uint32_t n, MotionComp M)
{
	const uint32_t i = blockIdx.x * MULLS_BLOCK + threadIdx.x;
	if (i >= n)
		return;
	float4 a = recs[(size_t)i * 3];
	const float sc = recs[(size_t)i * 3 + 2].y;
	if (mulls::scan::motion_comp_point(a.x, a.y, a.z, sc, M))
		recs[(size_t)i * 3] = a;
}

__global__ __launch_bounds__(256) void k_copy_segs(CopyArgs a)
{
	const CopySeg s = a.seg[blockIdx.y];
	const uint32_t w16 = s.bytes >> 4, first = blockIdx.x * 1024u;
	if (first >= w16 + 1u)
		return;
	const uint4 *__restrict__ src = reinterpret_cast<const uint4 *>(s.src);
	uint4 *__restrict__ dst = reinterpret_cast<uint4 *>(s.dst);
	uint4 v[4];
#pragma unroll
	for (int k = 0; k < 4; k++)
	{
		const uint32_t w = first + threadIdx.x + 256u * (uint32_t)k;
		if (w < w16)
			v[k] = src[w];
	}
#pragma unroll
	for (int k = 0; k < 4; k++)
	{
		const uint32_t w = first + threadIdx.x + 256u * (uint32_t)k;
		if (w < w16)
			dst[w] = v[k];
	}
	if (blockIdx.x == 0 && threadIdx.x < ((s.bytes & 15u) >> 2))
		reinterpret_cast<uint32_t *>(s.dst)[(size_t)w16 * 4u + threadIdx.x] = reinterpret_cast<const uint32_t *>(s.src)[(size_t)w16 * 4u + threadIdx.x];
}

#include "launch.h"

void launch_motion_comp(hipStream_t st, float4 *recs, uint32_t n, const double q[4], const double t[3], float thre)
{
	if (!n)
		return;
	const MotionComp M = mulls::scan::motion_comp_of(q, t, thre);
	hipLaunchKernelGGL(k_motion_comp, dim3((n + MULLS_BLOCK - 1) / MULLS_BLOCK), dim3(MULLS_BLOCK), 0, st, recs, n, M);
}

void launch_clone_src(hipStream_t st, const BatchDev &b, const RunParams &rp, uint32_t njobs)
{
	if (njobs)
		hipLaunchKernelGGL(k_clone_src, dim3(njobs), dim3(MULLS_BLOCK), 0, st, b.setup_jobs, b.descs, b.setup, b.stage, b.tmp_pos, b.tmp_nrm, b.bbox, rp);
}

void launch_src_setup(hipStream_t st, const BatchDev &b, const RunParams &rp, const uint32_t *pairs, uint32_t npairs)
{
	if (npairs)
		hipLaunchKernelGGL(k_src_setup, dim3(npairs), dim3(MULLS_SS_LANES), 0, st, pairs, b.descs, b.setup, b.stage, b.spos, b.snrm, b.flag, b.match, b.wd, b.bbox, rp);
}

void launch_crop(hipStream_t st, const BatchDev &b, const RunParams &rp, uint32_t npairs, uint32_t nbig_segs, uint32_t nbig_clouds, const uint32_t *wgs, uint32_t nwgs)
{
	if (!npairs)
		return;
	if (!wgs)
		nwgs = npairs * MULLS_NC * 2;
	if (nwgs)
		hipLaunchKernelGGL(k_crop, dim3(nwgs), dim3(MULLS_BLOCK), 0, st, wgs, b.descs, b.setup, b.bbox, b.stage, b.tmp_pos, b.tmp_nrm, b.spos, b.snrm, b.tpos, b.tnrm, b.flag,
						   b.match, b.wd, rp, b.grids, b.big_box);
	if (nbig_clouds)
	{
		hipLaunchKernelGGL(k_crop_big_count, dim3(nbig_segs), dim3(MULLS_BLOCK), 0, st, b.big_segs, b.descs, b.setup, b.bbox, b.stage, b.tmp_pos, rp, b.seg_cnt, b.big_box + (size_t)nbig_clouds * 6u);
		hipLaunchKernelGGL(k_crop_big_scan, dim3(nbig_clouds), dim3(64), 0, st, b.big_clouds, b.descs, rp, b.seg_cnt, b.big_box + (size_t)nbig_clouds * 6u, b.grids);
		hipLaunchKernelGGL(k_crop_big_scatter, dim3(nbig_segs), dim3(MULLS_BLOCK), 0, st, b.big_segs, b.descs, b.setup, b.bbox, b.stage, rp, b.seg_cnt, b.tpos,
						   b.tnrm, b.tmp_pos, b.tmp_nrm, b.spos, b.snrm, b.flag, b.match, b.wd);
	}
}
// ... 23 lines not shown
```

### mulls_amd/csrc/launch.h

```cpp
#pragma once
#include <hip/hip_runtime_api.h>
#include <stdint.h>

#include "device_types.h"

#include <hip/hip_vector_types.h>
#include <mutex>

struct DevLaunch
{
	bool ready = false, ok = false;
	size_t dyn_max[2] = {0, 0};
	uint32_t n_cu = 256;
};
template <int TAG, class Init>
inline DevLaunch dev_launch(Init init)
{
	static std::mutex mu;
	static DevLaunch table[64];
	int dev = 0;
	if (hipGetDevice(&dev) != hipSuccess || dev < 0 || dev >= 64)
		dev = 0;
	std::lock_guard<std::mutex> lock(mu);
	DevLaunch &D = table[dev];
	if (!D.ready)
	{
		int cus = 0;
		if (hipDeviceGetAttribute(&cus, hipDeviceAttributeMultiprocessorCount, dev) == hipSuccess && cus > 0)
			D.n_cu = (uint32_t)cus;
		D.ok = init(D);
		D.ready = true;
	}
	return D;
}
namespace mulls
{
struct IcpConst;
struct StepState;
}
struct BatchDev
{
	float4 *stage = nullptr;
	float4 *tmp_pos = nullptr, *tmp_nrm = nullptr;
	float4 *spos = nullptr, *snrm = nullptr, *tpos = nullptr, *tnrm = nullptr;
	uint8_t *flag = nullptr;
	int32_t *match = nullptr, *nn_idx = nullptr, *nn_hint = nullptr;
	float4 *mq = nullptr;
	float *wd = nullptr, *nn_d2 = nullptr;
	unsigned long long *winner = nullptr;
	CloudDesc *descs = nullptr;
	PairSetup *setup = nullptr;
	PairState *states = nullptr;
	PairState *states_pin = nullptr;
	PairOut *outs = nullptr;
	PairOut *outs_pin = nullptr;
	uint32_t *bbox = nullptr;
	Job *setup_jobs = nullptr;
	uint32_t *setup_tab = nullptr;
	Job *big_segs = nullptr, *big_clouds = nullptr;
	uint32_t *seg_cnt = nullptr, *big_box = nullptr;
	Job *jobs = nullptr;
	double *partial = nullptr;
	Job *tjobs = nullptr;
	Job *cjobs = nullptr;
	Job *bjobs = nullptr, *fjobs = nullptr, *ejobs = nullptr;
	uint32_t *lclouds = nullptr;
	uint32_t *bm_cs = nullptr;
	uint32_t *bm_rank = nullptr;
	uint32_t *ajobs = nullptr;
	IcpOut *icp_outs = nullptr;
	mulls::StepState *steps = nullptr;
	uint32_t *wl = nullptr;
	uint32_t *wl_ctr = nullptr;
	GridDesc *grids = nullptr;
	float4 *tsorted = nullptr;
	uint16_t *tmap = nullptr;
	uint32_t *cell_cnt = nullptr, *cell_start = nullptr;
	unsigned long long *bm = nullptr;
	uint32_t *pf = nullptr;
	uint32_t *ticket = nullptr;
};
void launch_clone_src(hipStream_t st, const BatchDev &b, const RunParams &rp, uint32_t njobs);
void launch_crop(hipStream_t st, const BatchDev &b, const RunParams &rp, uint32_t npairs, uint32_t nbig_segs, uint32_t nbig_clouds, const uint32_t *wgs = nullptr, uint32_t nwgs = 0);
void launch_src_setup(hipStream_t st, const BatchDev &b, const RunParams &rp, const uint32_t *pairs, uint32_t npairs);
void launch_copy_segs(hipStream_t st, const CopySeg *segs, uint32_t n);
void launch_motion_comp(hipStream_t st, float4 *recs, uint32_t n, const double q[4], const double t[3], float thre);
void launch_thin(hipStream_t st, const BatchDev &b, uint32_t npairs, const uint8_t *src_keep, const uint8_t *tgt_keep);
int launch_tgt_grid(hipStream_t st, const BatchDev &b, const RunParams &rp, uint32_t npairs, const uint32_t *clouds = nullptr, const uint32_t *split = nullptr);
const uint32_t *tgt_grid_bucket_trips();
void launch_grid_build_sort(hipStream_t st, const BatchDev &b, const RunParams &rp, uint32_t npairs);
void launch_bm_build(hipStream_t st, const BatchDev &b, uint32_t nl, uint32_t ntjobs);
size_t nn_lds_bytes(uint32_t cap, uint32_t maxcells, bool dedup);
int launch_nn_lds(hipStream_t st, const BatchDev &b, const RunParams &rp, const Job *jobs, uint32_t njobs, uint32_t cap, uint32_t *wl, uint32_t *wl_ctr, uint32_t parity,
				  bool first = false);
int launch_cert_mixed(hipStream_t st, const BatchDev &b, const RunParams &rp, const Job *cjobs, uint32_t n_lds, const Job *bjobs, uint32_t n_big, uint32_t max_wgs, uint32_t rounds,
					  uint32_t cap, bool first = false);
void launch_cert_big(hipStream_t st, const BatchDev &b, const RunParams &rp, const Job *jobs, uint32_t njobs, uint32_t max_wgs);
void launch_nn(hipStream_t st, const BatchDev &b, const RunParams &rp, const Job *jobs, uint32_t njobs);
void launch_nn_shoot(hipStream_t st, const BatchDev &b, const RunParams &rp, const Job *jobs, uint32_t njobs);
void launch_filter(hipStream_t st, const BatchDev &b, const RunParams &rp, const Job *jobs, uint32_t njobs, bool big = false);
void launch_accum(hipStream_t st, const BatchDev &b, const RunParams &rp, const uint32_t split[4], bool single = false, uint32_t wave_min_trips = 0);
void launch_finish(hipStream_t st, const BatchDev &b, const RunParams &rp, uint32_t pair_base, uint32_t npairs, uint32_t *ticket, volatile uint32_t *host_epoch, uint32_t epoch);
void launch_push_states(hipStream_t st, const BatchDev &b, uint32_t pair_base, uint32_t npairs);
void launch_step_init(hipStream_t st, const BatchDev &b, const mulls::IcpConst &K, uint32_t npairs);
void launch_finish_step(hipStream_t st, const BatchDev &b, const RunParams &rp, const mulls::IcpConst &K, uint32_t pair_base, uint32_t npairs, unsigned long long *host_word, uint32_t epoch,
						int brute, uint32_t *ticket = nullptr, bool sum_step = false);
void launch_transform_aos(hipStream_t st, float4 *recs, uint32_t n, const double *T12);
void launch_set_corr(hipStream_t st, const BatchDev &b, uint32_t src_off, const int32_t *cs, const int32_t *ct, const float *cd, uint32_t n, uint32_t tgt_off);
```

### mulls_amd/csrc/lds_tier.h

```cpp
#pragma once
#include "device_util.h"
struct FilterCtx
{
	bool gate, any_match, normal_check, dedup_done, strict;
	float max_sqr;
	double cos_thre;
	unsigned long long key_hi;
	const float4 *tgt_stage;
	const uint16_t *tgt_map;
};
__device__ __forceinline__ void filter_point(const FilterCtx &F, const CloudDesc &d, uint32_t s, const float4 *__restrict__ snrm,
											  const float4 *__restrict__ tnrm, uint8_t *__restrict__ flag, const int32_t *__restrict__ nn_idx,
											  const float *__restrict__ nn_d2, int32_t *__restrict__ match, float *__restrict__ wd,
											  const unsigned long long *__restrict__ winner, const float4 *__restrict__ tpos,
											  float4 *__restrict__ mq, uint32_t &n_alive, uint32_t &n_valid)
{
	const uint32_t g = d.src_off + s;
	const uint32_t f = flag[g];
	if (!(f & MULLS_F_ALIVE))
		return;
	bool alive = true, valid, fresh = false;
	int m;
	float4 n2 = make_float4(0.0f, 0.0f, 0.0f, 0.0f);
	if (F.any_match)
// ... 464 lines not shown
	const bool matched = bi >= 0 && !((double)best > C.max_dist_sqr);
	const float lb_new = fminf(sqrtf(sec), Rfin);
	hint2[d.src_off + s] = make_int2((int32_t)(((uint32_t)bi & 0xffffu) | (min(trips, 31u) << 16)), __float_as_int(lb_new));
#if MULLS_LDS_KCERT
	if (C.cand)
		C.cand[d.src_off + s] = make_uint4(co.cx, co.cy, __float_as_uint(fminf(sqrtf(co.b2), Rfin) - lb_new), C.epoch);
#else
	(void)co;
#endif
	const uint32_t w0 = park[s], st = (w0 >> 24) & ~MULLS_FS_SEARCH;
	const int32_t pm = (int32_t)(w0 & 0xffffffu) - 2, m = matched ? bi : -1;
	park[s] = ((st | ((matched && bi == pm) ? MULLS_FS_STANDING : 0u)) << 24) | (uint32_t)(m + 2);
	park[(uint32_t)D0 + s] = __float_as_uint(best);
	if (matched && C.dedup)
		dedup_min<W16>(W, (uint32_t)bi, s);
	return matched;
}

template <int BLK, bool W16 = false>
__device__ __forceinline__ void class_tail(const RunParams &rp, const PairState &ps, const ClassCtx &C, CloudDesc &d, const Job &job, uint32_t q_end,
											uint32_t matched_cnt, uint32_t searched, const uint32_t *W, uint32_t *red, const float4 *__restrict__ snrm,
											const float4 *__restrict__ tnrm, uint8_t *flag, int32_t *__restrict__ nn_idx, float *__restrict__ nn_d2,
											int32_t *__restrict__ match, float *__restrict__ wd, const unsigned long long *__restrict__ winner,
											const float4 *__restrict__ tpos, float4 *__restrict__ mq)
{
	if (C.dedup)
	{
		__threadfence_block();
		__syncthreads();
		for (uint32_t s = job.start + threadIdx.x; s < q_end; s += BLK)
			if (flag[d.src_off + s] & MULLS_F_ALIVE)
			{
				const int m = nn_idx[d.src_off + s];
				if (m >= 0 && !dedup_holds<W16>(W, (uint32_t)m, s))
					nn_idx[d.src_off + s] = -1;
			}
	}
	for (int off = 32; off > 0; off >>= 1)
		matched_cnt += __shfl_down(matched_cnt, off);
	if (!rp.lds_dedup)
	{
		if ((threadIdx.x & 63) == 0 && matched_cnt)
			atomicAdd(&d.n_matched, matched_cnt);
		return;
	}
	__threadfence_block();
	__syncthreads();
	if ((threadIdx.x & 63) == 0)
		red[threadIdx.x >> 6] = matched_cnt;
	__syncthreads();
	uint32_t total_matched = 0;
	for (int w = 0; w < BLK / 64; w++)
		total_matched += red[w];
	const float thr = ps.thr[job.cls];
	const FilterCtx F = {C.gate, total_matched > 0u, job.cls != 5, true, rp.rej_strict != 0, thr * thr, rp.cos_bearing, C.key_hi, rp.tgt_stage, rp.tgt_map};
	uint32_t n_alive = 0, n_valid = 0;
	for (uint32_t s = job.start + threadIdx.x; s < q_end; s += BLK)
		filter_point(F, d, s, snrm, tnrm, flag, nn_idx, nn_d2, match, wd, winner, tpos, mq, n_alive, n_valid);
	for (int off = 32; off > 0; off >>= 1)
	{
		n_alive += __shfl_down(n_alive, off);
		n_valid += __shfl_down(n_valid, off);
	}
	if ((threadIdx.x & 63) == 0)
	{
		red[BLK / 64 + (threadIdx.x >> 6)] = n_alive;
		red[2 * (BLK / 64) + (threadIdx.x >> 6)] = n_valid;
	}
	__syncthreads();
	if (threadIdx.x == 0)
	{
		uint32_t ta = 0, tv = 0;
		for (int w = 0; w < BLK / 64; w++)
		{
			ta += red[BLK / 64 + w];
			tv += red[2 * (BLK / 64) + w];
		}
		d.n_matched = total_matched;
		d.alive_next = ta;
		d.valid_next = tv;
		d.n_search = searched;
	}
}
template <int BLK, int TRIPS, bool W16>
__device__ __forceinline__ void class_tail_flat(const RunParams &rp, const PairState &ps, const ClassCtx &C, CloudDesc &d, const Job &job, uint32_t q_end,
												 uint32_t matched_cnt, uint32_t searched, const uint32_t *W, uint32_t *red, const float4 *__restrict__ snrm,
												 const float4 *__restrict__ tnrm, uint8_t *flag, const int32_t *__restrict__ nn_idx, const float *__restrict__ nn_d2,
												 int32_t *__restrict__ match, float *__restrict__ wd, const float4 *__restrict__ tpos, float4 *__restrict__ mq)
{
	__threadfence_block();
	__syncthreads();
	uint32_t FL[TRIPS];
	int32_t M[TRIPS], PM[TRIPS];
	float D[TRIPS];
	float3 N1[TRIPS], T2[TRIPS];
	const uint32_t last = d.src_off + (q_end ? q_end - 1u : 0u);
#pragma unroll
	for (int k = 0; k < TRIPS; k++)
	{
		const uint32_t gi = min(d.src_off + threadIdx.x + (uint32_t)k * BLK, last);
		FL[k] = flag[gi];
		M[k] = nn_idx[gi];
		D[k] = nn_d2[gi];
		PM[k] = match[gi];
		N1[k] = *reinterpret_cast<const float3 *>(snrm + gi);
		T2[k] = *reinterpret_cast<const float3 *>(mq + 2u * gi + 1u);
	}
	for (int off = 32; off > 0; off >>= 1)
		matched_cnt += __shfl_down(matched_cnt, off);
	if ((threadIdx.x & 63) == 0)
		red[threadIdx.x >> 6] = matched_cnt;
	__syncthreads();
	uint32_t total_matched = 0;
	for (int w = 0; w < BLK / 64; w++)
		total_matched += red[w];
	const float thr = ps.thr[job.cls], max_sqr = thr * thr;
	const bool any_match = total_matched > 0u, normal_check = job.cls != 5, strict = rp.rej_strict != 0;
	uint32_t n_alive = 0, n_valid = 0;
#pragma unroll
	for (int k = 0; k < TRIPS; k++)
	{
		const uint32_t s = threadIdx.x + (uint32_t)k * BLK, gi = d.src_off + s;
		if (s >= q_end || !(FL[k] & MULLS_F_ALIVE))
			continue;
		int32_t m = M[k];
		if (C.dedup && m >= 0 && !dedup_holds<W16>(W, (uint32_t)m, s))
			m = -1;
		bool alive = true, valid;
		float3 n2 = T2[k];
		if (any_match)
		{
			valid = m >= 0;
			if (C.gate && m < 0)
			{
				alive = false;
				valid = false;
			}
			if (valid)
			{
				const float dist = D[k];
				valid = strict ? dist < max_sqr : !(dist > max_sqr);
				if (valid)
				{
					wd[gi] = dist;
					if (PM[k] != m)
					{
						match[gi] = m;
						float4 q2, n4;
						tgt_record(rp.tgt_stage, rp.tgt_map, d, (uint32_t)m, tpos, tnrm, q2, n4);
						mq[2u * gi] = q2;
						mq[2u * gi + 1u] = n4;
						n2 = make_float3(n4.x, n4.y, n4.z);
					}
				}
			}
		}
		else if (C.gate)
		{
			alive = false;
			valid = false;
		}
		else
			valid = (FL[k] & MULLS_F_VALID) != 0;
		if (valid && normal_check)
		{
			const double dot = (double)N1[k].x * (double)n2.x + (double)N1[k].y * (double)n2.y + (double)N1[k].z * (double)n2.z;
			const float c = (float)fabs(dot);
			if ((double)c < rp.cos_bearing)
				valid = false;
		}
		const uint32_t nf = (alive ? MULLS_F_ALIVE : 0u) | (valid ? MULLS_F_VALID : 0u);
		if (nf != FL[k])
			flag[gi] = (uint8_t)nf;
		n_alive += alive ? 1u : 0u;
		n_valid += valid ? 1u : 0u;
	}
	for (int off = 32; off > 0; off >>= 1)
	{
		n_alive += __shfl_down(n_alive, off);
		n_valid += __shfl_down(n_valid, off);
	}
	if ((threadIdx.x & 63) == 0)
	{
		red[BLK / 64 + (threadIdx.x >> 6)] = n_alive;
		red[2 * (BLK / 64) + (threadIdx.x >> 6)] = n_valid;
	}
	__syncthreads();
	if (threadIdx.x == 0)
	{
		uint32_t ta = 0, tv = 0;
		for (int w = 0; w < BLK / 64; w++)
		{
			ta += red[BLK / 64 + w];
			tv += red[2 * (BLK / 64) + w];
		}
		d.n_matched = total_matched;
		d.alive_next = ta;
		d.valid_next = tv;
		d.n_search = searched;
	}
}

template <int SMALL>
struct CertLds
{
	float4 uq[SMALL];
	uint32_t us[SMALL];
	static constexpr bool LOOK = MULLS_LDS_KCERT != 0 && SMALL >= 128 && SMALL <= MULLS_CERT_BLOCK;
	float um[LOOK ? SMALL : 1];
	uint32_t ucount, red[3 * 16];
};

#define MULLS_NEEDS_SEARCH (-2)

template <bool W16, class TPre, class TPos>
__device__ __forceinline__ bool kcert_point(const RunParams &rp, const uint4 cr, const int2 h, uint32_t iter, float px, float py, float pz, float moved, uint32_t tgt_n,
											 const TPre &pre, const TPos &pos, nnkey &bk, float &lb_next, uint4 &cr_next)
{
	constexpr int NO = W16 ? 4 : 2;
	const uint32_t hj = W16 ? ((uint32_t)h.x & 0xffffu) : (uint32_t)h.x;
	if (!(rp.kcert != 0u && cr.w - rp.tick_base <= iter))
		return false;
	const float hy = __int_as_float(h.y), crz = __uint_as_float(cr.z);
	const float Bp = (hy + crz) - 4.0f * 1.1920929e-7f * fmaxf(fabsf(hy), fabsf(crz));
	if (!(moved * 1.00001f < Bp * 0.99999f))
		return false;
	uint32_t ci[NO + 1], tok[NO + 1];
	bool ok[NO + 1];
	ci[0] = hj, ok[0] = true;
#pragma unroll
	for (int j = 0; j < NO; j++)
	{
		const uint32_t w = j < NO / 2 ? cr.x : cr.y, c = W16 ? (w >> ((j & 1) << 4)) & 0xffffu : w;
		ok[j + 1] = c < tgt_n;
		ci[j + 1] = ok[j + 1] ? c : hj;
	}
#pragma unroll
	for (int j = 0; j <= NO; j++)
		tok[j] = pre(ci[j]);
	float4 cp[NO + 1];
#pragma unroll
	for (int j = 0; j <= NO; j++)
		cp[j] = pos(tok[j]);
	bk = NNKEY_NONE;
	float sec = __builtin_inff();
	int slot = -1;
#pragma unroll
	for (int j = 0; j <= NO; j++)
	{
		const float dx = px - cp[j].x, dy = py - cp[j].y, dz = pz - cp[j].z;
		const float dj = ok[j] ? (dx * dx + dy * dy) + dz * dz : __builtin_inff();
		sec = __builtin_amdgcn_fmed3f(sec, dj, key_dist(bk));
		const nnkey kj = ok[j] ? nn_key(dj, ci[j]) : NNKEY_NONE;
		const bool take = kj < bk;
		bk = take ? kj : bk;
		slot = take ? j - 1 : slot;
	}
	const float best = key_dist(bk);
	if (!(best >= 0.0f) || !(sqrtf(best) * 1.00001f + moved * 1.00001f < Bp * 0.99999f))
		return false;
	const float Bn = Bp - moved * 1.00001f;
	lb_next = fminf(sqrtf(sec), Bn);
	if (W16)
	{
		const uint32_t sh = ((uint32_t)slot & 1u) << 4, keepm = ~(0xffffu << sh), put = hj << sh;
		cr_next.x = slot >= 0 && slot < NO / 2 ? (cr.x & keepm) | put : cr.x;
		cr_next.y = slot >= NO / 2 ? (cr.y & keepm) | put : cr.y;
	}
	else
	{
// ... 32 lines not shown
			uint4 cr_next;
			const float moved = CL.um[threadIdx.x];
			const uint32_t tgt_off = d.tgt_off, tgt_n = d.tgt_n, st_off = d.tgt_stage, st_mul = ((d.stage_fmt >> 2) & 3u) == MULLS_STAGE_AOS48 ? 3u : 1u;
			const uint16_t *__restrict__ tmap = rp.tgt_map;
			const float4 *__restrict__ stage = rp.tgt_stage;
			bool pass;
			if (tmap)
			{
				auto pre = [&](uint32_t i) -> uint32_t { return (uint32_t)tmap[tgt_off + i]; };
				auto pos = [&](uint32_t t) -> float4 { return stage[(size_t)st_off + (size_t)t * st_mul]; };
				pass = kcert_point<true>(rp, cr, h, (uint32_t)ps.iter, e.x, e.y, e.z, moved, tgt_n, pre, pos, bk, lb_next, cr_next);
			}
			else
			{
				auto pre = [&](uint32_t i) -> uint32_t { return i; };
				auto pos = [&](uint32_t t) -> float4 { return tpos[tgt_off + t]; };
				pass = kcert_point<true>(rp, cr, h, (uint32_t)ps.iter, e.x, e.y, e.z, moved, tgt_n, pre, pos, bk, lb_next, cr_next);
			}
			if (pass)
			{
				const float best = key_dist(bk);
				const uint32_t bi = (uint32_t)bk;
				const bool matched = !((double)best > C.max_dist_sqr);
				nn_idx[gi] = matched ? (int32_t)bi : -1;
				nn_d2[gi] = best;
				hint2[gi] = make_int2((int32_t)bi, __float_as_int(lb_next));
				C.cand[gi] = cr_next;
				if (matched)
				{
					matched_cnt++;
					if (C.dedup)
						dedup_min<W16>(W, bi, es);
					else if (C.gate)
						atomicMin(&winner[d.tgt_off + bi], C.key_hi | (unsigned long long)es);
				}
				keep = false;
			}
		}
	}
	const unsigned long long bal = __ballot(keep);
	const uint32_t lane = threadIdx.x & 63u, wave = threadIdx.x >> 6;
	if (rp.dbg_ticks)
	{
		const unsigned long long tried = __ballot(threadIdx.x < UL && (CL.us[min(threadIdx.x, (uint32_t)SMALL - 1u)] & MULLS_US_KCERT) != 0u);
		const unsigned long long passed = __ballot(threadIdx.x < UL && !keep);
		if (lane == 0u && tried)
		{
			atomicAdd(&rp.dbg_ticks[14], (unsigned long long)__popcll(tried));
			atomicAdd(&rp.dbg_ticks[15], (unsigned long long)__popcll(passed));
		}
	}
	if (lane == 0u)
		CL.red[wave] = (uint32_t)__popcll(bal);
	__syncthreads();
	uint32_t base = 0u, total = 0u;
	for (uint32_t w = 0; w < (uint32_t)(BLK / 64); w++)
	{
		const uint32_t c = CL.red[w];
		base += w < wave ? c : 0u;
		total += c;
	}
	if (keep)
	{
		const uint32_t k = base + (uint32_t)__popcll(bal & ((1ull << lane) - 1ull));
		CL.uq[k] = e;
		CL.us[k] = es;
	}
	__syncthreads();
	return total;
}

template <int BLK, bool W16, int SMALL>
__device__ __forceinline__ bool cert_class(CertLds<SMALL> &CL, const RunParams &rp, const PairState &ps, const Job &job, CloudDesc &d, const GridDesc &g, uint32_t *W,
											float4 *__restrict__ spos, float4 *__restrict__ snrm, const uint32_t *__restrict__ cell_start,
											const float4 *__restrict__ tsorted, uint8_t *flag, int32_t *__restrict__ nn_idx, float *__restrict__ nn_d2,
											unsigned long long *__restrict__ winner, const float4 *__restrict__ tnrm, int32_t *__restrict__ match,
											float *__restrict__ wd, const float4 *__restrict__ tpos, int32_t *__restrict__ nn_hint, float4 *__restrict__ mq)
{
	float4 *uq = CL.uq;
	uint32_t *us = CL.us, *red = CL.red;
	uint32_t &ucount = CL.ucount;
	int2 *__restrict__ hint2 = reinterpret_cast<int2 *>(nn_hint);

	const uint32_t src_n = d.src_n, tgt_n = d.tgt_n;
	const bool called = class_called(rp, d, job.cls);
	const ClassCtx C = class_ctx(rp, ps, g, job.cls, d.alive_cur, called);
	const bool have_prev = ps.iter > 0;
	const bool use_hint = called && have_prev;
	const bool kc = CertLds<SMALL>::LOOK && rp.kcert != 0u && use_hint && C.cand != nullptr;
	const uint32_t q_end = min(src_n, job.start + (job.count ? job.count : (uint32_t)MULLS_SRC_PER_BLOCK));
	if (C.dedup)
		dedup_init<W16>(W, tgt_n, BLK);
	if (threadIdx.x == 0)
		ucount = 0u;
	__syncthreads();

	uint32_t matched_cnt = 0;
	for (uint32_t s = job.start + threadIdx.x; s < q_end; s += BLK)
	{
		const uint32_t gi = d.src_off + s;
		const uint32_t fl = flag[gi];
		const float4 p = spos[gi], n = snrm[gi];
		const int2 h = hint2[gi];
		const int32_t pm0 = match[gi];
		const float4 q0 = mq[2u * gi];
		if (!(fl & MULLS_F_ALIVE))
			continue;
		uint32_t hv = 0xffffu;
		float lb = 0.0f;
		int32_t pm = -1;
		if (have_prev)
		{
			lb = __int_as_float(h.y);
			if (use_hint)
			{
				hv = (uint32_t)h.x;
				pm = pm0;
			}
		}
		const uint32_t hj = hv & 0xffffu;
		float4 tj = make_float4(0.0f, 0.0f, 0.0f, 0.0f);
		if (hj < tgt_n)
			tj = (int32_t)hj == pm ? q0 : tgt_point(rp.tgt_stage, rp.tgt_map, d, hj, tpos);
		const double *T = ps.T;
		const double x = p.x, y = p.y, z = p.z, nx = n.x, ny = n.y, nz = n.z;
		float4 out;
		out.x = (float)(T[0] * x + T[1] * y + T[2] * z + T[3]);
		out.y = (float)(T[4] * x + T[5] * y + T[6] * z + T[7]);
		out.z = (float)(T[8] * x + T[9] * y + T[10] * z + T[11]);
		const float onx = (float)(T[0] * nx + T[1] * ny + T[2] * nz);
		const float ony = (float)(T[4] * nx + T[5] * ny + T[6] * nz);
		const float onz = (float)(T[8] * nx + T[9] * ny + T[10] * nz);
		spos[gi] = make_float4(out.x, out.y, out.z, p.w);
		snrm[gi] = make_float4(onx, ony, onz, n.w);
		const float mx = out.x - p.x, my = out.y - p.y, mz = out.z - p.z;
		const float moved = sqrtf((mx * mx + my * my) + mz * mz);
		const float lb_next = lb - moved * 1.00001f;
		if (!called)
		{
			nn_hint[2u * gi + 1u] = __float_as_int(have_prev ? lb_next : 0.0f);
			continue;
		}
		out.w = __builtin_inff();
		bool certified = false;
		if (hj < tgt_n)
		{
			const float dx = out.x - tj.x, dy = out.y - tj.y, dz = out.z - tj.z;
			const float d0 = (dx * dx + dy * dy) + dz * dz;
			if (d0 >= 0.0f)
			{
				const float dh = sqrtf(d0);
				certified = rp.cert != 0u && (dh * 1.00001f + moved * 1.00001f < lb * 0.99999f);
				out.w = dh + fminf(fmaxf(rp.cert_slack_rate * moved, rp.cert_slack_min), rp.cert_slack_max);
				if (certified)
				{
					const bool matched = !((double)d0 > C.max_dist_sqr);
					nn_idx[gi] = matched ? (int32_t)hj : -1;
					nn_d2[gi] = d0;
					hint2[gi] = make_int2((int32_t)hj, __float_as_int(lb_next));
					if (matched)
					{
						matched_cnt++;
						if (C.dedup)
							dedup_min<W16>(W, hj, s);
						else if (C.gate)
							atomicMin(&winner[d.tgt_off + hj], C.key_hi | (unsigned long long)s);
					}
				}
			}
		}
		if (!certified)
		{
			nn_idx[gi] = MULLS_NEEDS_SEARCH;
			nn_d2[gi] = out.w;
			const uint32_t k = atomicAdd(&ucount, 1u);
			if (k < (uint32_t)SMALL)
			{
				const bool second = kc && hj < tgt_n;
				uq[k] = out;
				us[k] = second ? s | MULLS_US_KCERT : s;
				if (CertLds<SMALL>::LOOK)
					CL.um[k] = moved;
			}
		}
	}
	if (!called)
		return true;
	__syncthreads();
	uint32_t U = ucount;
	if (kc && U >= rp.kcert_min && U <= (uint32_t)SMALL)
		U = kcert_list<BLK, W16, SMALL>(CL, rp, ps, C, d, U, nn_idx, nn_d2, hint2, W, winner, tpos, matched_cnt);
	if (U > (uint32_t)SMALL)
		return false;
	const GlobGrid L = {tsorted + d.tgt_off, reinterpret_cast<const uint16_t *>(cell_start) + g.cell_off};
	const uint32_t sub = threadIdx.x & (MULLS_LDS_GROUP - 1u), grp = threadIdx.x / MULLS_LDS_GROUP;
	for (uint32_t i = grp; i < U; i += BLK / MULLS_LDS_GROUP)
	{
		nnkey bk;
		float sec, Rfin;
		uint32_t trips;
		CandOut co = {0xffffffffu, 0xffffffffu, 0.0f};
		search_query<MULLS_GLOB_CHUNK>(g, L, uq[i], C.r, C.m, sub, bk, sec, Rfin, trips, co);
		if (sub == 0 && commit_search<W16>(C, d, us[i] & ~MULLS_US_KCERT, bk, sec, Rfin, trips, co, nn_idx, nn_d2, hint2, W, winner))
			matched_cnt++;
	}
	class_tail<BLK, W16>(rp, ps, C, d, job, q_end, matched_cnt, U, W, red, snrm, tnrm, flag, nn_idx, nn_d2, match, wd, winner, tpos, mq);
	return true;
}

template <int BLK, int TRIPS, bool W16, int SMALL, bool PARK = false>
__device__ __forceinline__ bool cert_class_flat(CertLds<SMALL> &CL, const RunParams &rp, const PairState &ps, const Job &job, CloudDesc &d, const GridDesc &g, uint32_t *W,
												 float4 *__restrict__ spos, float4 *__restrict__ snrm, const uint32_t *__restrict__ cell_start,
												 const float4 *__restrict__ tsorted, uint8_t *flag, int32_t *__restrict__ nn_idx, float *__restrict__ nn_d2,
												 unsigned long long *__restrict__ winner, const float4 *__restrict__ tnrm, int32_t *__restrict__ match,
												 float *__restrict__ wd, const float4 *__restrict__ tpos, int32_t *__restrict__ nn_hint, float4 *__restrict__ mq, uint32_t *park = nullptr)
{
	float4 *uq = CL.uq;
	uint32_t *us = CL.us, *red = CL.red;
	uint32_t &ucount = CL.ucount;
	int2 *__restrict__ hint2 = reinterpret_cast<int2 *>(nn_hint);
	const uint32_t src_n = d.src_n, tgt_n = d.tgt_n;
	const ClassCtx C = class_ctx(rp, ps, g, job.cls, d.alive_cur, true);
	const bool have_prev = ps.iter > 0;
	const bool normal_check = job.cls != 5;
	const bool kc = CertLds<SMALL>::LOOK && rp.kcert != 0u && have_prev && C.cand != nullptr;
	const uint32_t q_end = src_n;
	unsigned long long t_prev = rp.dbg_ticks ? wall_clock64() : 0ull;
#define FLAT_TICK(k)                                                  \
	if (rp.dbg_ticks)                                                 \
	{                                                                 \
		const unsigned long long now_ = wall_clock64();               \
		if (threadIdx.x == 0)                                         \
			atomicAdd(&rp.dbg_ticks[k], now_ - t_prev);               \
		t_prev = now_;                                                \
	}

	struct Rec
	{
		uint32_t fl;
		int32_t pm;
		float3 p, n, q, t;
		int2 h;
	};
	const uint32_t last = d.src_off + (q_end ? q_end - 1u : 0u);
	auto load = [&](int k) {
		Rec r;
		const uint32_t gi = min(d.src_off + threadIdx.x + (uint32_t)k * BLK, last);
		r.fl = flag[gi];
		r.p = *reinterpret_cast<const float3 *>(spos + gi), r.n = *reinterpret_cast<const float3 *>(snrm + gi);
		r.h = hint2[gi];
		r.pm = match[gi];
		r.q = *reinterpret_cast<const float3 *>(mq + 2u * gi), r.t = *reinterpret_cast<const float3 *>(mq + 2u * gi + 1u);
		return r;
	};
	uint32_t STr[PARK ? 1 : TRIPS];
	int32_t Mr[PARK ? 1 : TRIPS];
	float D0r[PARK ? 1 : TRIPS];
	auto setSM = [&](int k, uint32_t st, int32_t m) {
		if (PARK)
			park[(uint32_t)k * BLK + threadIdx.x] = (st << 24) | (uint32_t)(m + 2);
		else
			STr[PARK ? 0 : k] = st, Mr[PARK ? 0 : k] = m;
	};
	auto getST = [&](int k) -> uint32_t { return PARK ? park[(uint32_t)k * BLK + threadIdx.x] >> 24 : STr[PARK ? 0 : k]; };
	auto getM = [&](int k) -> int32_t { return PARK ? (int32_t)(park[(uint32_t)k * BLK + threadIdx.x] & 0xffffffu) - 2 : Mr[PARK ? 0 : k]; };
	auto setD0 = [&](int k, float v) {
		if (PARK)
			park[(uint32_t)(TRIPS + k) * BLK + threadIdx.x] = __float_as_uint(v);
		else
			D0r[PARK ? 0 : k] = v;
	};
	auto getD0 = [&](int k) -> float { return PARK ? __uint_as_float(park[(uint32_t)(TRIPS + k) * BLK + threadIdx.x]) : D0r[PARK ? 0 : k]; };
	auto waits = [&](int k) -> bool { return PARK ? (getST(k) & MULLS_FS_SEARCH) != 0u : getM(k) == MULLS_NEEDS_SEARCH; };
	uint32_t matched_cnt = 0;
	auto cert = [&](int k, const Rec &r) {
		const uint32_t s = threadIdx.x + (uint32_t)k * BLK, gi = d.src_off + s;
		uint32_t st_k = 0u;
		int32_t m_k = -1;
		setSM(k, 0u, -1), setD0(k, 0.0f);
		if (s >= q_end || !(r.fl & MULLS_F_ALIVE))
			return;
		st_k = r.fl & (MULLS_FS_ALIVE | MULLS_FS_VALID);
		const float3 p = r.p, n = r.n;
		uint32_t hv = 0xffffu;
		float lb = 0.0f;
		int32_t pm = -1;
		if (have_prev)
		{
			lb = __int_as_float(r.h.y);
			hv = (uint32_t)r.h.x;
			pm = r.pm;
		}
		const uint32_t hj = hv & 0xffffu;
		float4 tj = make_float4(0.0f, 0.0f, 0.0f, 0.0f);
		if (hj < tgt_n)
			tj = (int32_t)hj == pm ? make_float4(r.q.x, r.q.y, r.q.z, 0.0f) : tgt_point(rp.tgt_stage, rp.tgt_map, d, hj, tpos);
		const double *T = ps.T;
		const double x = p.x, y = p.y, z = p.z, nx = n.x, ny = n.y, nz = n.z;
		float4 out;
		out.x = (float)(T[0] * x + T[1] * y + T[2] * z + T[3]);
		out.y = (float)(T[4] * x + T[5] * y + T[6] * z + T[7]);
		out.z = (float)(T[8] * x + T[9] * y + T[10] * z + T[11]);
		const float onx = (float)(T[0] * nx + T[1] * ny + T[2] * nz);
		const float ony = (float)(T[4] * nx + T[5] * ny + T[6] * nz);
// ... 181 lines not shown
					if (normal_check)
					{
						const float3 n1 = *reinterpret_cast<const float3 *>(snrm + gi);
						const double dot = (double)n1.x * (double)n2.x + (double)n1.y * (double)n2.y + (double)n1.z * (double)n2.z;
						const float c = (float)fabs(dot);
						dir_ok = !((double)c < rp.cos_bearing);
					}
				}
				valid = strict ? dist < max_sqr : !(dist > max_sqr);
				if (valid)
					wd[gi] = dist;
			}
		}
		else if (C.gate)
		{
			alive = false;
			valid = false;
		}
		else
			valid = (st & MULLS_FS_VALID) != 0;
		if (valid && normal_check && !dir_ok)
			valid = false;
		const uint32_t nf = (alive ? MULLS_F_ALIVE : 0u) | (valid ? MULLS_F_VALID : 0u);
		if (nf != (st & (MULLS_FS_ALIVE | MULLS_FS_VALID)))
			flag[gi] = (uint8_t)nf;
		n_alive += alive ? 1u : 0u;
		n_valid += valid ? 1u : 0u;
	}
	for (int off = 32; off > 0; off >>= 1)
	{
		n_alive += __shfl_down(n_alive, off);
		n_valid += __shfl_down(n_valid, off);
	}
	if ((threadIdx.x & 63) == 0)
	{
		red[BLK / 64 + (threadIdx.x >> 6)] = n_alive;
		red[2 * (BLK / 64) + (threadIdx.x >> 6)] = n_valid;
	}
	__syncthreads();
	if (threadIdx.x == 0)
	{
		uint32_t ta = 0, tv = 0;
		for (int w = 0; w < BLK / 64; w++)
		{
			ta += red[BLK / 64 + w];
			tv += red[2 * (BLK / 64) + w];
		}
		d.n_matched = total_matched;
		d.alive_next = ta;
		d.valid_next = tv;
		d.n_search = U;
	}
	FLAT_TICK(4)
	if (rp.dbg_ticks && threadIdx.x == 0)
		atomicAdd(&rp.dbg_ticks[6], 1ull);
#undef FLAT_TICK
	return true;
}

struct LdsLayout
{
	float4 *qpos;
	uint32_t *HIST;
	uint16_t *ORDER;
	float *P;
	uint16_t *IDX;
	uint16_t *CS;
	uint32_t *W;
};
__device__ __forceinline__ LdsLayout lds_layout(unsigned char *lds_raw, uint32_t cap, uint32_t grid_maxcells)
{
	LdsLayout L;
	L.qpos = reinterpret_cast<float4 *>(lds_raw);
	L.HIST = reinterpret_cast<uint32_t *>(L.qpos + MULLS_LDS_QCHUNK);
	L.ORDER = reinterpret_cast<uint16_t *>(L.HIST + 80);
	L.P = reinterpret_cast<float *>(reinterpret_cast<unsigned char *>(L.HIST) + MULLS_LDS_AUX);
	L.IDX = reinterpret_cast<uint16_t *>(L.P + 3u * cap);
	L.CS = L.IDX + cap;
	L.W = reinterpret_cast<uint32_t *>(L.CS + ((grid_maxcells + 8u) & ~1u));
	return L;
}

__device__ __forceinline__ void lds_search_class(const RunParams &rp, const PairState &ps, const Job &job, CloudDesc &d, const GridDesc &g,
												  const LdsLayout &Y, unsigned char *lds_raw, const float4 *__restrict__ spos,
												  const float4 *__restrict__ snrm, const uint32_t *__restrict__ cell_start,
												  const float4 *__restrict__ tsorted, uint8_t *flag, int32_t *__restrict__ nn_idx, float *__restrict__ nn_d2,
												  unsigned long long *__restrict__ winner, const float4 *__restrict__ tnrm, int32_t *__restrict__ match,
												  float *__restrict__ wd, const float4 *__restrict__ tpos, int32_t *__restrict__ nn_hint, float4 *__restrict__ mq,
												  bool first = false)
{
	unsigned long long t_prev = rp.dbg_ticks ? wall_clock64() : 0ull;
#define HEAVY_TICK(k)                                                 \
	if (rp.dbg_ticks)                                                 \
	{                                                                 \
		const unsigned long long now_ = wall_clock64();               \
		if (threadIdx.x == 0)                                         \
			atomicAdd(&rp.dbg_ticks[k], now_ - t_prev);               \
		t_prev = now_;                                                \
	}
	float4 *qpos = Y.qpos;
	uint32_t *HIST = Y.HIST;
	uint16_t *ORDER = Y.ORDER;
	float *P = Y.P;
	uint16_t *IDX = Y.IDX, *CS = Y.CS;
	uint32_t *W = Y.W;
	int2 *__restrict__ hint2 = reinterpret_cast<int2 *>(nn_hint);
	const uint32_t src_n = d.src_n, tgt_n = d.tgt_n;
	const ClassCtx C = class_ctx(rp, ps, g, job.cls, d.alive_cur, true);
	const uint32_t q_end = min(src_n, job.start + (job.count ? job.count : (uint32_t)MULLS_SRC_PER_BLOCK));
	const uint32_t q_cnt = q_end > job.start ? q_end - job.start : 0u, n_chunks = (q_cnt + MULLS_LDS_QCHUNK - 1u) / MULLS_LDS_QCHUNK;
	const uint32_t q_step = n_chunks ? (q_cnt + n_chunks - 1u) / n_chunks : 1u;

	float4 pf_p = make_float4(0.0f, 0.0f, 0.0f, 0.0f);
	float pf_w = 0.0f;
	uint32_t pf_hv = 0u, pf_f = 0u;
	int32_t pf_i = -1;
	auto prefetch = [&](uint32_t chunk) {
		const uint32_t s = chunk + threadIdx.x, gi = d.src_off + s;
		pf_f = 0u;
		pf_i = -1;
		if (chunk < q_end && s < min(q_end, chunk + q_step))
		{
			pf_f = flag[gi];
			pf_p = spos[gi];
			if (first)
				pf_i = MULLS_NEEDS_SEARCH, pf_w = __builtin_inff(), pf_hv = 0u;
			else
			{
				pf_i = nn_idx[gi];
				pf_w = nn_d2[gi];
				pf_hv = (uint32_t)hint2[gi].x;
			}
		}
	};
	prefetch(job.start);

	{
		const float4 *__restrict__ ts = tsorted + d.tgt_off;
		for (uint32_t k0 = threadIdx.x; k0 < tgt_n; k0 += 8 * MULLS_LDS_BLOCK)
		{
			float4 t[8];
#pragma unroll
			for (int u = 0; u < 8; u++)
			{
				const uint32_t k = k0 + u * MULLS_LDS_BLOCK;
				if (k < tgt_n)
					t[u] = ts[k];
			}
#pragma unroll
			for (int u = 0; u < 8; u++)
			{
				const uint32_t k = k0 + u * MULLS_LDS_BLOCK;
				if (k < tgt_n)
				{
					P[3u * k] = t[u].x;
					P[3u * k + 1u] = t[u].y;
					P[3u * k + 2u] = t[u].z;
					IDX[k] = (uint16_t)__float_as_int(t[u].w);
				}
			}
		}
		const uint4 *__restrict__ cs4 = reinterpret_cast<const uint4 *>(reinterpret_cast<const uint16_t *>(cell_start) + g.cell_off);
		const uint32_t nw = (g.ncell + 1u + 7u) >> 3;
		for (uint32_t w0 = threadIdx.x; w0 < nw; w0 += 2 * MULLS_LDS_BLOCK)
		{
			const uint32_t w1 = w0 + MULLS_LDS_BLOCK;
			const uint4 va = cs4[w0], vb = cs4[min(w1, nw - 1u)];
			reinterpret_cast<uint4 *>(CS)[w0] = va;
			if (w1 < nw)
				reinterpret_cast<uint4 *>(CS)[w1] = vb;
		}
	}
	if (C.dedup)
		for (uint32_t t = threadIdx.x; t < tgt_n; t += MULLS_LDS_BLOCK)
			W[t] = 0xffffffffu;
	const LdsGrid L = {P, IDX, CS};
	const uint32_t sub = threadIdx.x & (MULLS_LDS_GROUP - 1u);
	uint32_t matched_cnt = 0, searched = 0;

	if (threadIdx.x < 32u)
		HIST[threadIdx.x] = 0u;
	for (uint32_t chunk = job.start; chunk < q_end; chunk += q_step)
	{
		__syncthreads();
		HEAVY_TICK(chunk == job.start ? 8 : 10)
		uint32_t bucket = 0, rank = 0xffffffffu;
		if (threadIdx.x < MULLS_LDS_QCHUNK && (pf_f & MULLS_F_ALIVE))
		{
			if (pf_i == MULLS_NEEDS_SEARCH)
			{
				qpos[threadIdx.x] = make_float4(pf_p.x, pf_p.y, pf_p.z, pf_w);
				bucket = 31u - ((pf_hv >> 16) & 31u);
				if (!(pf_w < __builtin_inff()))
				{
					const uint32_t c = grid_cell_id(g, pf_p.x, pf_p.y, pf_p.z);
					bucket = CS[c + 1u] > CS[c] ? 8u : 0u;
				}
				rank = atomicAdd(&HIST[bucket], 1u);
			}
			else if (pf_i >= 0)
			{
				matched_cnt++;
				if (C.dedup)
					atomicMin(&W[pf_i], chunk + threadIdx.x);
			}
		}
		prefetch(chunk + q_step);
		__syncthreads();
		if (threadIdx.x < 32u)
		{
			const uint32_t v = HIST[threadIdx.x];
			uint32_t incl = v;
			for (int off = 1; off < 32; off <<= 1)
			{
				const uint32_t o = __shfl_up(incl, off);
				if ((int)threadIdx.x >= off)
					incl += o;
			}
			HIST[32u + threadIdx.x] = incl - v;
			HIST[threadIdx.x] = 0u;
			if (threadIdx.x == 31u)
			{
				HIST[64] = incl;
				HIST[66] = 0u;
			}
		}
		__syncthreads();
		if (rank != 0xffffffffu)
			ORDER[HIST[32u + bucket] + rank] = (uint16_t)threadIdx.x;
		__syncthreads();
		const uint32_t n_live = HIST[64];
		searched += n_live;
		HEAVY_TICK(9)

		for (;;)
		{
			uint32_t base = 0;
			if ((threadIdx.x & 63u) == 0u)
				base = atomicAdd(&HIST[66], 64u / MULLS_LDS_GROUP);
			base = (uint32_t)__builtin_amdgcn_readfirstlane((int)base);
			if (base >= n_live)
				break;
			const uint32_t i = base + (threadIdx.x & 63u) / MULLS_LDS_GROUP;
			if (i < n_live)
			{
				const uint32_t k = ORDER[i];
				nnkey bk;
				float sec, Rfin;
				uint32_t trips;
				CandOut co = {0xffffffffu, 0xffffffffu, 0.0f};
				search_query(g, L, qpos[k], C.r, C.m, sub, bk, sec, Rfin, trips, co);
				if (sub == 0 && commit_search(C, d, chunk + k, bk, sec, Rfin, trips, co, nn_idx, nn_d2, hint2, W, winner))
					matched_cnt++;
			}
		}
	}
	HEAVY_TICK(10)
	uint32_t *red = reinterpret_cast<uint32_t *>(lds_raw);
	if (rp.lds_dedup && rp.debug_stop != 9u && job.start == 0u && q_end <= 2u * MULLS_LDS_BLOCK)
		class_tail_flat<MULLS_LDS_BLOCK, 2, false>(rp, ps, C, d, job, q_end, matched_cnt, searched, W, red, snrm, tnrm, flag, nn_idx, nn_d2, match, wd, tpos, mq);
	else
		class_tail<MULLS_LDS_BLOCK>(rp, ps, C, d, job, q_end, matched_cnt, searched, W, red, snrm, tnrm, flag, nn_idx, nn_d2, match, wd, winner, tpos, mq);
	HEAVY_TICK(11)
	if (rp.dbg_ticks && threadIdx.x == 0)
		atomicAdd(&rp.dbg_ticks[12], 1ull);
#undef HEAVY_TICK
}
}
```

### mulls_amd/csrc/loop.cpp

```cpp
#include "batch.h"

using namespace mulls_drv;

namespace
{
struct Run
{
	mulls_ctx *ctx;
	mulls_batch *B;
	const mulls_params *P;
	mulls_result *results;
	int n;
	hipStream_t st;
	std::chrono::steady_clock::time_point wall0;
	EvTimer evt;
	RunParams rp;
	mulls::IcpConst K;
	uint32_t lds_cap = 0;
	uint32_t max_big_tgt = 0;
	int tier = 0;
	bool use_grid = false, dstep = false;
};
struct DrainOnError
{
// ... 2 lines not shown
	~DrainOnError()
	{
		if (armed)
		{
			(void)hipStreamSynchronize(ctx->stream);
			(void)hipStreamSynchronize(ctx->stream2);
		}
	}
};

int run_setup(Run &R)
{
	mulls_ctx *ctx = R.ctx;
	mulls_batch *B = R.B;
	const mulls_params *P = R.P;
	mulls_result *results = R.results;
	const int n = R.n;
	hipStream_t st = R.st;
	EvTimer &evt = R.evt;
	int rc;

	RunParams &rp = R.rp;
	std::memset(&rp, 0, sizeof(rp));
	rp.pull_comb = 1;
	for (int c = 0; c < MULLS_NC; c++)
		rp.used[c] = P->used_feature_type[c] == '1';
	rp.w_balance = P->weight_strategy[0] == '1';
	rp.w_resid = P->weight_strategy[1] == '1';
	rp.w_dist = P->weight_strategy[2] == '1';
	rp.w_inten = P->weight_strategy[3] == '1';
	rp.normal_shooting = P->normal_shooting_on != 0;
	rp.undistort = P->apply_motion_undistortion != 0;
	rp.crop = P->apply_intersection_filter != 0 && !rp.undistort;
	rp.faithful = P->faithful != 0;
	rp.rej_strict = P->rejector_strict != 0;
	rp.z_xy_ratio = P->z_xy_balanced_ratio;
	rp.win_pt = P->pt2pt_residual_window;
	rp.win_pl = P->pt2pl_residual_window;
	rp.win_li = P->pt2li_residual_window;
	rp.cos_bearing = std::cos(P->normal_bearing / 180.0 * M_PI);
	rp.resid_from_iter = 2;
	init_cert(ctx, rp);
	if ((rc = take_epochs(ctx, B, (uint32_t)std::max(P->max_iter_num, 0) + 2u, rp)) != MULLS_OK)
		return rc;
	rp.debug_stop = (uint32_t)ctx->opt[MULLS_OPT_DEBUG_STOP];

	bool dstep = P->max_iter_num > 0;
	for (int p = 0; p < n && dstep; p++)
		dstep = !(results[p].trace && results[p].trace_cap > 0);
	dstep = dstep && ctx->opt[MULLS_OPT_HOST_STEP] == 0.0;
	uint32_t lds_cap = 0;
	int tier = 0;
	const int dstep_nsub = (ctx->profiling == 0 && n >= (int)ctx->opt[MULLS_OPT_SPLIT_MIN_PAIRS] && n <= (int)ctx->opt[MULLS_OPT_SPLIT_MAX_PAIRS]) ? 2 : 1;
	rc = prepare_run(ctx, B, P, rp, &lds_cap, &tier, dstep ? dstep_nsub : 0, true);
	if (rc != MULLS_OK)
		return rc;
	const bool use_grid = tier != 0;
	R.lds_cap = lds_cap, R.tier = tier, R.use_grid = use_grid, R.dstep = dstep;
	R.max_big_tgt = 0;
	if (tier == 3)
		for (const CloudDesc &d : B->descs_h)
			if (d.tier == MULLS_TIER_BM)
				R.max_big_tgt = std::max(R.max_big_tgt, d.tgt_n0);

	bool fused_tgt = tier == 2 && ctx->opt[MULLS_OPT_FUSED_TGT_SETUP] != 0.0 && !P->keep_less_source_points && !rp.normal_shooting && B->n_big_tgt == 0;
	for (size_t k = 0; k < B->descs_h.size() && fused_tgt; k++)
		fused_tgt = B->descs_h[k].tgt_n0 <= MULLS_LDS_MAXPTS;
	fused_tgt = fused_tgt || tier == 3;
	if (fused_tgt)
	{
		rp.tgt_stage = B->stage;
		rp.tgt_map = B->tmap;
		rp.grid_maxcells = std::min(rp.grid_maxcells, 32767u);
	}

	if (rp.debug_stop == 20u || rp.debug_stop == 21u)
	{
		if (!B->dbg && dmalloc(ctx, &B->dbg, 16) != MULLS_OK)
			return MULLS_E_HIP;
		HIPCHK(ctx, hipMemsetAsync(B->dbg, 0, 16 * sizeof(unsigned long long), st));
		rp.dbg_ticks = B->dbg;
	}

	evt.begin(&ctx->prof.ms_setup);
	queue_clone_crop(st, B, rp);
	if (P->keep_less_source_points && !rp.undistort)
	{
		std::vector<CloudDesc> back(B->descs_h.size());
		HIPCHK(ctx, hipMemcpyAsync(back.data(), B->descs, sizeof(CloudDesc) * back.size(), hipMemcpyDeviceToHost, st));
		HIPCHK(ctx, hipStreamSynchronize(st));
		std::vector<uint8_t> skeep(std::max<size_t>(B->n_src, 1), 1), tkeep(std::max<size_t>(B->n_tgt, 1), 1);
		for (int p = 0; p < n; p++)
		{
			const CloudDesc *pd = &back[(size_t)p * MULLS_NC];
			auto T = [&](int c, int keep) { return thin_mask(tkeep.data() + pd[c].tgt_off, pd[c].tgt_n, keep, P->rng_seed, 0 * 6 + c); };
			auto S = [&](int c, int keep) { return thin_mask(skeep.data() + pd[c].src_off, pd[c].src_n, keep, P->rng_seed, 1 * 6 + c); };
			const uint32_t tg = T(MULLS_GROUND, (int)(pd[MULLS_GROUND].tgt_n / 2));
			const uint32_t tf = T(MULLS_FACADE, (int)(pd[MULLS_FACADE].tgt_n / 2));
			S(MULLS_GROUND, (int)(tg / 4));
			S(MULLS_FACADE, (int)(tf / 2));
			S(MULLS_PILLAR, (int)pd[MULLS_PILLAR].tgt_n);
			S(MULLS_BEAM, (int)pd[MULLS_BEAM].tgt_n);
			S(MULLS_ROOF, (int)pd[MULLS_ROOF].tgt_n);
			S(MULLS_VERTEX, (int)pd[MULLS_VERTEX].tgt_n);
		}
		if ((rc = apply_keep_masks(ctx, B, skeep, tkeep, "keep_less_source_points: ")) != MULLS_OK)
			return rc;
	}
	queue_target_grids(st, B, rp, tier, fused_tgt);
	evt.end();

	R.K = icp_const(P);
	return MULLS_OK;
}

struct Slice
{
	uint32_t job_lo = 0, job_n = 0, cjob_lo = 0, cjob_n = 0, bjob_lo = 0, bjob_n = 0, fjob_lo = 0, fjob_n = 0, ejob_lo = 0, ejob_n = 0;
	const uint32_t *ajob_split = nullptr;
};
Slice slice_of(const mulls_batch *B, int lo, int hi, int k)
{
	auto first_of = [](const std::vector<Job> &v, uint32_t pair) {
		return (uint32_t)(std::lower_bound(v.begin(), v.end(), pair, [](const Job &j, uint32_t q) { return j.pair < q; }) - v.begin());
	};
	Slice L;
	L.job_lo = first_of(B->jobs_h, (uint32_t)lo);
	L.job_n = first_of(B->jobs_h, (uint32_t)hi) - L.job_lo;
	L.cjob_lo = first_of(B->cjobs_h, (uint32_t)lo);
	L.cjob_n = first_of(B->cjobs_h, (uint32_t)hi) - L.cjob_lo;
	L.bjob_lo = first_of(B->bjobs_h, (uint32_t)lo);
	L.bjob_n = first_of(B->bjobs_h, (uint32_t)hi) - L.bjob_lo;
	L.fjob_lo = first_of(B->fjobs_h, (uint32_t)lo);
	L.fjob_n = first_of(B->fjobs_h, (uint32_t)hi) - L.fjob_lo;
	L.ejob_lo = first_of(B->ejobs_h, (uint32_t)lo);
	L.ejob_n = first_of(B->ejobs_h, (uint32_t)hi) - L.ejob_lo;
	L.ajob_split = B->ajob_split[k];
	return L;
}

int launch_search(Run &R, hipStream_t sst, const Slice &L, uint32_t *wl, uint32_t *wl_ctr, uint32_t parity, EvTimer &ev, int iter)
{
	mulls_ctx *ctx = R.ctx;
	const mulls_batch *B = R.B;
	const RunParams &rp = R.rp;
	const int tier = R.tier;
	const Job *jobs = B->jobs + L.job_lo;
	ev.begin(&ctx->prof.ms_nn);
	if (tier == 0)
		launch_nn(sst, *B, rp, jobs, L.job_n);
	const bool early = L.ejob_n && (iter < (int)ctx->opt[MULLS_OPT_BIG_EARLY_SETS] || (L.bjob_n - L.fjob_n < 64u && R.max_big_tgt > 100000u));
	const uint32_t max_wgs = iter < std::max(3, (int)ctx->opt[MULLS_OPT_BIG_EARLY_SETS]) ? 2048u : 512u;
#ifndef MULLS_MIXED_WIDE_ITERS
#define MULLS_MIXED_WIDE_ITERS 2
#endif
#ifndef MULLS_MIXED_ROUNDS
#define MULLS_MIXED_ROUNDS 3u
#endif
	const uint32_t mixed_rounds = early && iter < MULLS_MIXED_WIDE_ITERS ? MULLS_MIXED_ROUNDS : 1u;
	const uint32_t big_n = early ? L.ejob_n : L.bjob_n;
	const Job *big_jobs = early ? B->ejobs + L.ejob_lo : B->bjobs + L.bjob_lo;
	const bool first = iter == 0 && rp.lds_dedup != 0u && !rp.normal_shooting && ctx->opt[MULLS_OPT_FIRST_DIRECT] != 0.0;
	const bool together = tier == 3 && L.cjob_n && big_n &&
						  launch_cert_mixed(sst, *B, rp, B->cjobs + L.cjob_lo, L.cjob_n, big_jobs, big_n, max_wgs, mixed_rounds, R.lds_cap, first) != 0;
	if (!together && L.cjob_n && launch_nn_lds(sst, *B, rp, B->cjobs + L.cjob_lo, L.cjob_n, R.lds_cap, wl, wl_ctr, parity, first) != 0)
	{
		ctx->err = "could not raise the dynamic LDS limit of k_nn_lds";
		return MULLS_E_HIP;
	}
	if (!together && (early || L.bjob_n))
		launch_cert_big(sst, *B, rp, big_jobs, big_n, max_wgs);
	if (rp.normal_shooting)
		launch_nn_shoot(sst, *B, rp, jobs, L.job_n);
	ev.end();
	ev.begin(&ctx->prof.ms_filter);
	if (tier == 0 || (tier == 2 && !rp.lds_dedup))
		launch_filter(sst, *B, rp, jobs, L.job_n);
	else if (early)
		launch_filter(sst, *B, rp, B->ejobs + L.ejob_lo, L.ejob_n, true);
	else if (L.fjob_n)
		launch_filter(sst, *B, rp, B->fjobs + L.fjob_lo, L.fjob_n, true);
	ev.end();
	const hipError_t e = hipGetLastError();
	if (e != hipSuccess)
	{
		ctx->err = std::string("correspondence search launch: ") + hipGetErrorString(e);
		return MULLS_E_HIP;
	}
	return MULLS_OK;
}

int results_from_device(Run &R)
{
	mulls_ctx *ctx = R.ctx;
	mulls_batch *B = R.B;
	mulls_result *results = R.results;
	const RunParams &rp = R.rp;
	const int n = R.n;

	if (grow_pinned(ctx, &B->icp_outs_pin, &B->cap_icp_pin, (size_t)n, hipHostMallocDefault) != MULLS_OK)
		return MULLS_E_NOMEM;
	HIPCHK(ctx, hipMemcpyAsync(B->icp_outs_pin, B->icp_outs, sizeof(IcpOut) * (size_t)n, hipMemcpyDeviceToHost, R.st));
	HIPCHK(ctx, hipStreamSynchronize(R.st));
	R.evt.collect();
	const double wall_ms = std::chrono::duration<double>(std::chrono::steady_clock::now() - R.wall0).count() * 1e3;
	int max_it = 0;
	for (int p = 0; p < n; p++)
	{
		const IcpOut &o = B->icp_outs_pin[p];
		mulls_result &R = results[p];
		R.code = o.code;
		R.iters = o.iters;
		std::memcpy(R.T, o.T, sizeof(R.T));
		std::memcpy(R.info, o.info, sizeof(R.info));
		R.sigma = (float)std::sqrt(o.sigma2);
		R.confidence = o.ratio;
		R.singular = o.singular;
		R.ms_total = (float)(wall_ms / n);
		for (int c = 0; c < MULLS_NC; c++)
		{
			R.ncorr[c] = o.ncorr[c];
			R.nsrc0[c] = o.nsrc0[c];
			R.ntgt0[c] = o.ntgt0[c];
		}
		R.cropped = 0;
		std::memset(R.crop_box, 0, sizeof(R.crop_box));
		fill_crop_box(rp, B->setup_h[p].tgt_bound, o.bbox, R);
		R.trace_len = 0;
		ctx->prof.nn_src_pts += o.src_pts;
		ctx->prof.nn_tgt_unique += o.tgt_pts;
		ctx->prof.nn_tgt_pts += o.tgt_job_pts;
		ctx->prof.nn_corr_pts += o.corr_pts;
		ctx->prof.nn_pair_evals += o.pair_evals;
		max_it = std::max(max_it, o.iters);
	}
	ctx->prof.iterations = max_it;
	if (rp.dbg_ticks)
	{
		unsigned long long t[16];
		HIPCHK(ctx, hipMemcpy(t, rp.dbg_ticks, sizeof(t), hipMemcpyDeviceToHost));
		if (rp.debug_stop == 21u)
		{
			ctx->prof.icp_fused_ms[0] += (double)t[13], ctx->prof.icp_fused_ms[1] += (double)t[7] * 1e-5;
			return MULLS_OK;
		}
		for (int k = 0; k < 5; k++)
			ctx->prof.icp_fused_ms[k] += (double)t[k] * 1e-5;
		ctx->prof.icp_fused_ms[5] += (double)t[6];
		ctx->prof.icp_search_ms[0] += (double)t[13], ctx->prof.icp_search_ms[1] += (double)t[14], ctx->prof.icp_search_ms[2] += (double)t[15], ctx->prof.icp_search_ms[3] += (double)t[7];
		for (int k = 0; k < 4; k++)
			ctx->prof.icp_phase_ms[k] += (double)t[8 + k] * 1e-5;
		ctx->prof.icp_phase_ms[4] += (double)t[12];
	}
	return MULLS_OK;
}

int run_device_step(Run &R)
{
	mulls_ctx *ctx = R.ctx;
	mulls_batch *B = R.B;
	const mulls_params *P = R.P;
	const RunParams &rp = R.rp;
	EvTimer &evt = R.evt;
	const int n = R.n;
	hipStream_t st = R.st;
	int rc;
	if (grow(ctx, &B->steps, &B->cap_steps, (size_t)n) != MULLS_OK || grow(ctx, &B->icp_outs, &B->cap_icp_outs, (size_t)n) != MULLS_OK)
		return MULLS_E_HIP;
	HIPCHK(ctx, hipMemsetAsync(B->icp_outs, 0, sizeof(IcpOut) * (size_t)n, st));
	launch_step_init(st, *B, R.K, (uint32_t)n);
	const bool few_launches = n <= (int)ctx->opt[MULLS_OPT_FEW_LAUNCHES_MAX_PAIRS];
	bool sum_step = ctx->opt[MULLS_OPT_SUM_STEP] != 0.0;
	for (size_t k = 0; sum_step && k < B->descs_h.size(); k++)
		sum_step = B->descs_h[k].job_end - B->descs_h[k].job_begin <= 4u * (1024u / MULLS_SRC_PER_BLOCK);
	struct Sub
	{
		int lo = 0, hi = 0;
		Slice L;
		hipStream_t st = nullptr;
		volatile unsigned long long *word = nullptr;
		unsigned long long *word_dev = nullptr;
		uint32_t *epoch_ctr = nullptr, *ticket = nullptr, *wl = nullptr, *wl_ctr = nullptr;
		uint32_t epoch0 = 0, nn_launches = 0, left = 0;
		int s = 0;
		bool done = false;
		EvTimer ev2[2] = {EvTimer{nullptr}, EvTimer{nullptr}};
	};
	const int nsub = B->nsub;
	Sub subs[2];
	for (int k = 0; k < nsub; k++)
	{
		Sub &S = subs[k];
		S.lo = (int)((long)n * k / nsub);
		S.hi = (int)((long)n * (k + 1) / nsub);
		S.L = slice_of(B, S.lo, S.hi, k);
		S.st = k == 0 ? ctx->stream : ctx->stream2;
		S.word = reinterpret_cast<volatile unsigned long long *>(B->epoch_h + 32 + 16 * k);
		S.word_dev = reinterpret_cast<unsigned long long *>(B->epoch_dev + 32 + 16 * k);
		S.epoch_ctr = k == 0 ? &B->epoch2 : &B->epoch3;
		S.epoch0 = *S.epoch_ctr;
		S.ticket = B->ticket + 2 + 4 * k;
		S.wl = B->wl + S.L.cjob_lo;
		S.wl_ctr = B->wl_ctr + 8 * k;
		S.left = (uint32_t)(S.hi - S.lo);
		for (int e = 0; e < 2; e++)
		{
			S.ev2[e].ctx = ctx;
			S.ev2[e].base = 10 * e;
		}
	}
	subs[0].ev2[0].used = evt.used;
	for (int k = 0; k < 5; k++)
		subs[0].ev2[0].slot[k] = evt.slot[k];
	evt.used = 0;
	if (nsub == 2)
	{
		HIPCHK(ctx, hipEventRecord(ctx->ev_setup, ctx->stream));
		HIPCHK(ctx, hipStreamWaitEvent(ctx->stream2, ctx->ev_setup, 0));
	}
	DrainOnError drain{ctx};
	auto wait_set = [&](Sub &S, int set) -> int {
		const uint32_t want = S.epoch0 + (uint32_t)set + 1u;
		const auto t0 = std::chrono::steady_clock::now();
		bool synced = false;
		for (uint64_t spins = 0;; spins++)
		{
			const unsigned long long w = *S.word;
			if ((int32_t)((uint32_t)(w >> 32) - want) >= 0)
			{
				std::atomic_thread_fence(std::memory_order_acquire);
				S.left = (uint32_t)w;
				return MULLS_OK;
// ... 403 lines not shown
```

Measured before the change: 273,400.

## Compact alive source points after first LDS search and use live masks in accumulation

On the first ICP iteration for small flat LDS-tier classes, the tail pass compacts surviving source points (positions, normals, hints, flags, matches, weights) into a dense prefix and records per-64-point alive bitmasks with prefix counts. Later search passes iterate only over the compacted count, and the wave-level accumulation kernel uses the live words to map lanes to compacted indices. The goal is to stop spending search and reduction work on points that were rejected in the first iteration. It adds an extra buffer, ballot/prefix bookkeeping and in-place scatter writes, and it only turns on when the tier, dedup and wave-accum conditions all hold.

```diff
diff --git a/mulls_amd/csrc/batch.cpp b/mulls_amd/csrc/batch.cpp
--- a/mulls_amd/csrc/batch.cpp
+++ b/mulls_amd/csrc/batch.cpp
@@ -643,6 +643,7 @@
 	A(grow(ctx, &B->nn_hint, &B->cap_src[9], 2 * so, nullptr, 8 * SG));
 	A(grow(ctx, &B->mq, &B->cap_src[10], 2 * so, nullptr, 9 * SG));
 	A(grow(ctx, &B->nn_cand, &B->cap_src[11], so, &cand_grew, 14 * SG));
+	A(grow(ctx, &B->live_mask, &B->cap_live, (so >> 6) + (size_t)n * MULLS_NC + 1u));
 	A(grow(ctx, &B->tpos, &B->cap_tgt[0], to));
 	A(grow(ctx, &B->tnrm, &B->cap_tgt[1], to));
 	A(grow(ctx, &B->tsorted, &B->cap_tgt[2], to, nullptr, 10 * SG));
diff --git a/mulls_amd/csrc/batch.h b/mulls_amd/csrc/batch.h
--- a/mulls_amd/csrc/batch.h
+++ b/mulls_amd/csrc/batch.h
@@ -77,6 +77,8 @@
 	std::string jobs_key;
 	uint32_t njobs = 0;
 	uint4 *nn_cand = nullptr;
+	LiveWord *live_mask = nullptr;
+	size_t cap_live = 0;
 	uint32_t tick = 1;
 	size_t cap_outs = 0;
 	size_t cap_big[4] = {};
diff --git a/mulls_amd/csrc/device_types.h b/mulls_amd/csrc/device_types.h
--- a/mulls_amd/csrc/device_types.h
+++ b/mulls_amd/csrc/device_types.h
@@ -70,6 +70,13 @@
 	uint32_t stage_fmt;
 	uint32_t tier;
 	uint32_t grid_slot;
+	uint32_t src_c;
+	uint32_t compacted;
+};
+struct LiveWord
+{
+	unsigned long long alive;
+	uint32_t below, pad_;
 };
 #define MULLS_STAGE_AOS48 0u
 #define MULLS_STAGE_PACK32 1u
@@ -184,4 +191,6 @@
 	const float4 *tgt_stage;
 	const uint16_t *tgt_map;
 	unsigned long long *dbg_ticks;
+	LiveWord *live_mask;
 };
+#define MULLS_COMPACT_MAX (3u * MULLS_CERT_BLOCK)
diff --git a/mulls_amd/csrc/device_util.h b/mulls_amd/csrc/device_util.h
--- a/mulls_amd/csrc/device_util.h
+++ b/mulls_amd/csrc/device_util.h
@@ -78,6 +78,8 @@
 {
 	return tgt_map ? load_staged_pos(tgt_stage, d.tgt_stage, (d.stage_fmt >> 2) & 3u, tgt_map[d.tgt_off + m]) : tpos[d.tgt_off + m];
 }
+
+__device__ __forceinline__ uint32_t live_word_base(const CloudDesc &d, uint32_t cloud) { return (d.src_off >> 6) + cloud; }
 
 __device__ __forceinline__ bool class_called(const RunParams &rp, const CloudDesc &d, int cls)
 {
diff --git a/mulls_amd/csrc/driver.cpp b/mulls_amd/csrc/driver.cpp
--- a/mulls_amd/csrc/driver.cpp
+++ b/mulls_amd/csrc/driver.cpp
@@ -339,7 +339,7 @@
 			return;
 		if (ctx)
 			(void)hipSetDevice(ctx->device);
-		void *dev[] = {B->stage, B->tmp_pos, B->tmp_nrm, B->spos, B->snrm, B->tpos, B->tnrm, B->flag, B->match, B->nn_idx, B->nn_hint, B->nn_cand, B->mq, B->wd,
+		void *dev[] = {B->stage, B->tmp_pos, B->tmp_nrm, B->spos, B->snrm, B->tpos, B->tnrm, B->flag, B->match, B->nn_idx, B->nn_hint, B->nn_cand, B->live_mask, B->mq, B->wd,
 					   B->nn_d2, B->winner, B->descs, B->setup, B->states, B->outs, B->ticket, B->bbox, B->setup_jobs, B->big_segs, B->big_clouds, B->seg_cnt, B->big_box, B->jobs, B->partial,
 					   B->tjobs, B->cjobs, B->bjobs, B->fjobs, B->ejobs, B->lclouds, B->bm_cs, B->wl, B->wl_ctr, B->grids, B->tsorted, B->tmap, B->dbg, B->cell_cnt, B->cell_start, B->bm, B->pf, B->descs_init, B->bbox_init,
 					   B->ajobs, B->icp_outs, B->steps, B->bm_rank, B->setup_tab};
diff --git a/mulls_amd/csrc/k_reduce.hip b/mulls_amd/csrc/k_reduce.hip
--- a/mulls_amd/csrc/k_reduce.hip
+++ b/mulls_amd/csrc/k_reduce.hip
@@ -57,15 +57,26 @@
 }
 template <typename TS, int NT, int MODE, int METRIC, int T0, int NTW>
 __device__ __forceinline__ void wave_trip(const AccumCtx &A, const double *x, const CloudDesc &d, uint32_t trip0, const float4 *__restrict__ spos, const float4 *__restrict__ mq,
-										   const uint8_t *__restrict__ flag, float *__restrict__ wd, double *__restrict__ out, bool owner)
+										   const uint8_t *__restrict__ flag, float *__restrict__ wd, double *__restrict__ out, bool owner, const LiveWord *__restrict__ live,
+										   uint32_t cloud)
 {
 	const uint32_t lane = threadIdx.x & 63u;
 	const uint32_t src_n = d.src_n, src_off = d.src_off;
 	const uint32_t n_here = min(src_n - trip0, (uint32_t)MULLS_ACC_LANES), iters = (n_here + 63u) >> 6;
-	const uint32_t last = src_off + src_n - 1u;
+	const bool compacted = d.compacted != 0u;
+	const uint32_t last = src_off + (compacted ? max(d.src_c, 1u) : src_n) - 1u;
+	const unsigned long long below_me = (1ull << lane) - 1ull;
+	static_assert(MULLS_ACC_LANES / 64 <= 64, "one LiveWord per lane covers a trip");
+	uint32_t lw_lo = 0u, lw_hi = 0u, lw_below = 0u;
+	if (compacted)
+	{
+		const LiveWord w = live[live_word_base(d, cloud) + (trip0 >> 6) + min(lane, iters - 1u)];
+		lw_lo = (uint32_t)w.alive, lw_hi = (uint32_t)(w.alive >> 32), lw_below = w.below;
+	}
 	struct Rec
 	{
-		uint32_t f;
+		uint32_t f, g;
+		bool live;
 		float4 P, Q;
 		float3 N;
 		float w;
@@ -73,7 +84,16 @@
 	const bool need_w = A.residual_pass, writes_w = !A.residual_pass && (METRIC != 2 || !A.faithful);
 	auto load = [&](uint32_t i) {
 		Rec r;
-		const uint32_t g = min(src_off + trip0 + lane + 64u * i, last);
+		uint32_t g = src_off + trip0 + lane + 64u * i;
+		r.live = true;
+		if (compacted)
+		{
+			const unsigned long long alive = ((unsigned long long)(uint32_t)__builtin_amdgcn_readlane((int)lw_hi, (int)i) << 32) | (uint32_t)__builtin_amdgcn_readlane((int)lw_lo, (int)i);
+			g = src_off + (uint32_t)__builtin_amdgcn_readlane((int)lw_below, (int)i) + (uint32_t)__popcll(alive & below_me);
+			r.live = ((alive >> lane) & 1ull) != 0ull;
+		}
+		g = min(g, last);
+		r.g = g;
 		r.f = flag[g];
 		r.P = spos[g], r.Q = mq[2u * g], r.N = *reinterpret_cast<const float3 *>(mq + 2u * g + 1u);
 		r.w = need_w ? wd[g] : 0.0f;
@@ -99,7 +119,7 @@
 		MULLS_PIN_REC(cur);
 #endif
 		const uint32_t s = trip0 + lane + 64u * i;
-		const bool valid = s < src_n && (cur.f & (MULLS_F_ALIVE | MULLS_F_VALID)) == (MULLS_F_ALIVE | MULLS_F_VALID);
+		const bool valid = s < src_n && cur.live && (cur.f & (MULLS_F_ALIVE | MULLS_F_VALID)) == (MULLS_F_ALIVE | MULLS_F_VALID);
 		if (valid)
 		{
 			float w = cur.w;
@@ -108,7 +128,7 @@
 			const float wpre = A.residual_pass ? 0.0f : corr_weight(A, METRIC, cur.P, cur.Q, N4, wi);
 			add_windows<TS, T0, NTW, MODE, METRIC, T0>(A, x, cur.P, cur.Q, N4, wi, w, acc, A.residual_pass ? nullptr : &wpre);
 			if (owner && writes_w)
-				wd[src_off + s] = w;
+				wd[cur.g] = w;
 		}
 #if MULLS_ACCW_PREFETCH
 		cur = nxt;
@@ -172,6 +192,7 @@
 		cnt[c] = (int)(class_called(rp, pd[c], c) ? pd[c].valid_next : pd[c].n_valid);
 	const AccumCtx A = accum_ctx(rp, job.cls, ps.iter, residual_pass, class_weight(rp, job.cls, residual_pass, cnt));
 	const CloudDesc &d = pd[job.cls];
+	const uint32_t ci = job.pair * MULLS_NC + job.cls;
 	double *out = partial + (size_t)job_idx * MULLS_NTERM;
 	if (d.src_n <= job.start)
 	{
@@ -184,34 +205,34 @@
 		if (part)
 			return;
 		if (!residual_pass)
-			wave_trip<double, 12, 1, 1, 0, 12>(A, ps.x, d, job.start, spos, mq, flag, wd, out, true);
+			wave_trip<double, 12, 1, 1, 0, 12>(A, ps.x, d, job.start, spos, mq, flag, wd, out, true, rp.live_mask, ci);
 		else if (A.metric == 0)
-			wave_trip<double, 2, 0, 0, 0, 2>(A, ps.x, d, job.start, spos, mq, flag, wd, out, true);
+			wave_trip<double, 2, 0, 0, 0, 2>(A, ps.x, d, job.start, spos, mq, flag, wd, out, true, rp.live_mask, ci);
 		else if (A.metric == 1)
-			wave_trip<double, 2, 0, 1, 0, 2>(A, ps.x, d, job.start, spos, mq, flag, wd, out, true);
+			wave_trip<double, 2, 0, 1, 0, 2>(A, ps.x, d, job.start, spos, mq, flag, wd, out, true, rp.live_mask, ci);
 		else
-			wave_trip<double, 2, 0, 2, 0, 2>(A, ps.x, d, job.start, spos, mq, flag, wd, out, true);
+			wave_trip<double, 2, 0, 2, 0, 2>(A, ps.x, d, job.start, spos, mq, flag, wd, out, true, rp.live_mask, ci);
 	}
 #if MULLS_ACCW_SPLIT == 2
 	else if (A.metric == 0)
 	{
 		if (part == 0u)
-			wave_trip<float, 27, 0, 0, 0, 14>(A, ps.x, d, job.start, spos, mq, flag, wd, out, true);
+			wave_trip<float, 27, 0, 0, 0, 14>(A, ps.x, d, job.start, spos, mq, flag, wd, out, true, rp.live_mask, ci);
 		else
-			wave_trip<float, 27, 0, 0, 14, 13>(A, ps.x, d, job.start, spos, mq, flag, wd, out, false);
+			wave_trip<float, 27, 0, 0, 14, 13>(A, ps.x, d, job.start, spos, mq, flag, wd, out, false, rp.live_mask, ci);
 	}
 	else
 	{
 		if (part == 0u)
-			wave_trip<float, 27, 0, 2, 0, 14>(A, ps.x, d, job.start, spos, mq, flag, wd, out, true);
+			wave_trip<float, 27, 0, 2, 0, 14>(A, ps.x, d, job.start, spos, mq, flag, wd, out, true, rp.live_mask, ci);
 		else
-			wave_trip<float, 27, 0, 2, 14, 13>(A, ps.x, d, job.start, spos, mq, flag, wd, out, false);
+			wave_trip<float, 27, 0, 2, 14, 13>(A, ps.x, d, job.start, spos, mq, flag, wd, out, false, rp.live_mask, ci);
 	}
 #else
 	else if (A.metric == 0)
-		wave_trip<float, 27, 0, 0, 0, 27>(A, ps.x, d, job.start, spos, mq, flag, wd, out, true);
+		wave_trip<float, 27, 0, 0, 0, 27>(A, ps.x, d, job.start, spos, mq, flag, wd, out, true, rp.live_mask, ci);
 	else
-		wave_trip<float, 27, 0, 2, 0, 27>(A, ps.x, d, job.start, spos, mq, flag, wd, out, true);
+		wave_trip<float, 27, 0, 2, 0, 27>(A, ps.x, d, job.start, spos, mq, flag, wd, out, true, rp.live_mask, ci);
 #endif
 }
 
@@ -789,13 +810,19 @@
 
 #include "launch.h"
 
+bool accum_takes_waves(const RunParams &rp, const uint32_t split[4], uint32_t wave_min_trips)
+{
+	const uint32_t n_trips = split[3] - split[0];
+	return wave_min_trips && n_trips >= wave_min_trips && rp.faithful && rp.pull_comb;
+}
+
 void launch_accum(hipStream_t st, const BatchDev &b, const RunParams &rp, const uint32_t split[4], bool single, uint32_t wave_min_trips)
 {
 	(void)dev_launch<3>([](DevLaunch &) {
 		return hipFuncSetAttribute(reinterpret_cast<const void *>(k_accum<1024, 2>), hipFuncAttributeMaxDynamicSharedMemorySize, (int)MULLS_RED_BYTES_HALF) == hipSuccess;
 	});
 	const uint32_t n_trips = split[3] - split[0];
-	if (wave_min_trips && n_trips >= wave_min_trips && rp.faithful && rp.pull_comb)
+	if (accum_takes_waves(rp, split, wave_min_trips))
 	{
 		hipLaunchKernelGGL(k_accum_wave, dim3((n_trips + MULLS_ACCW_WAVES / MULLS_ACCW_SPLIT - 1u) / (MULLS_ACCW_WAVES / MULLS_ACCW_SPLIT)), dim3(64 * MULLS_ACCW_WAVES), 0, st, b.ajobs + split[0], n_trips, b.jobs, b.descs, b.states, rp, b.spos,
 						   b.mq, b.flag, b.wd, b.partial);
diff --git a/mulls_amd/csrc/k_search.hip b/mulls_amd/csrc/k_search.hip
--- a/mulls_amd/csrc/k_search.hip
+++ b/mulls_amd/csrc/k_search.hip
@@ -357,8 +357,8 @@
 }
 
 __global__ __launch_bounds__(MULLS_LDS_BLOCK) void k_nn_lds(const Job *__restrict__ cjobs, CloudDesc *__restrict__ descs,
-															 const PairState *__restrict__ states, RunParams rp, const float4 *__restrict__ spos,
-															 const float4 *__restrict__ snrm, const GridDesc *__restrict__ grids,
+															 const PairState *__restrict__ states, RunParams rp, float4 *spos,
+															 float4 *snrm, const GridDesc *__restrict__ grids,
 															 const uint32_t *__restrict__ cell_start, const float4 *__restrict__ tsorted,
 															 uint8_t *flag, int32_t *__restrict__ nn_idx, float *__restrict__ nn_d2,
 															 unsigned long long *__restrict__ winner, const float4 *__restrict__ tnrm, int32_t *__restrict__ match,
diff --git a/mulls_amd/csrc/k_setup.hip b/mulls_amd/csrc/k_setup.hip
--- a/mulls_amd/csrc/k_setup.hip
+++ b/mulls_amd/csrc/k_setup.hip
@@ -227,7 +227,7 @@
 			d.tgt_n = running;
 		else
 		{
-			d.src_n = running;
+			d.src_n = d.src_c = running;
 			d.alive_cur = running;
 			d.alive_next = 0;
 			d.n_matched = 0;
@@ -394,7 +394,7 @@
 	{
 		CloudDesc &d = pd[threadIdx.x];
 		const uint32_t n = cls_base[threadIdx.x + 1] - cls_base[threadIdx.x];
-		d.src_n = n;
+		d.src_n = d.src_c = n;
 		d.alive_cur = n;
 		d.alive_next = 0;
 		d.n_matched = 0;
@@ -501,7 +501,7 @@
 	if (threadIdx.x == 0 && (bc.cls & MULLS_BIG_SRC_SIDE))
 	{
 		CloudDesc &d = descs[bc.pair * MULLS_NC + (bc.cls & 0xffu)];
-		d.src_n = running;
+		d.src_n = d.src_c = running;
 		d.alive_cur = running;
 		d.alive_next = 0;
 		d.n_matched = 0;
@@ -642,7 +642,7 @@
 			d.tgt_n = running;
 		else
 		{
-			d.src_n = running;
+			d.src_n = d.src_c = running;
 			d.alive_cur = running;
 		}
 	}
diff --git a/mulls_amd/csrc/launch.h b/mulls_amd/csrc/launch.h
--- a/mulls_amd/csrc/launch.h
+++ b/mulls_amd/csrc/launch.h
@@ -100,6 +100,7 @@
 void launch_nn_shoot(hipStream_t st, const BatchDev &b, const RunParams &rp, const Job *jobs, uint32_t njobs);
 void launch_filter(hipStream_t st, const BatchDev &b, const RunParams &rp, const Job *jobs, uint32_t njobs, bool big = false);
 void launch_accum(hipStream_t st, const BatchDev &b, const RunParams &rp, const uint32_t split[4], bool single = false, uint32_t wave_min_trips = 0);
+bool accum_takes_waves(const RunParams &rp, const uint32_t split[4], uint32_t wave_min_trips);
 void launch_finish(hipStream_t st, const BatchDev &b, const RunParams &rp, uint32_t pair_base, uint32_t npairs, uint32_t *ticket, volatile uint32_t *host_epoch, uint32_t epoch);
 void launch_push_states(hipStream_t st, const BatchDev &b, uint32_t pair_base, uint32_t npairs);
 void launch_step_init(hipStream_t st, const BatchDev &b, const mulls::IcpConst &K, uint32_t npairs);
diff --git a/mulls_amd/csrc/lds_tier.h b/mulls_amd/csrc/lds_tier.h
--- a/mulls_amd/csrc/lds_tier.h
+++ b/mulls_amd/csrc/lds_tier.h
@@ -570,11 +570,12 @@
 		d.n_search = searched;
 	}
 }
-template <int BLK, int TRIPS, bool W16>
+template <int BLK, int TRIPS, bool W16, bool COMPACT = false>
 __device__ __forceinline__ void class_tail_flat(const RunParams &rp, const PairState &ps, const ClassCtx &C, CloudDesc &d, const Job &job, uint32_t q_end,
-												 uint32_t matched_cnt, uint32_t searched, const uint32_t *W, uint32_t *red, const float4 *__restrict__ snrm,
+												 uint32_t matched_cnt, uint32_t searched, const uint32_t *W, uint32_t *red, float4 *snrm,
 												 const float4 *__restrict__ tnrm, uint8_t *flag, const int32_t *__restrict__ nn_idx, const float *__restrict__ nn_d2,
-												 int32_t *__restrict__ match, float *__restrict__ wd, const float4 *__restrict__ tpos, float4 *__restrict__ mq)
+												 int32_t *__restrict__ match, float *__restrict__ wd, const float4 *__restrict__ tpos, float4 *__restrict__ mq,
+												 float4 *spos = nullptr, int2 *hint2 = nullptr)
 {
 	__threadfence_block();
 	__syncthreads();
@@ -582,6 +583,12 @@
 	int32_t M[TRIPS], PM[TRIPS];
 	float D[TRIPS];
 	float3 N1[TRIPS], T2[TRIPS];
+	float4 P4[COMPACT ? TRIPS : 1], Q2[COMPACT ? TRIPS : 1], N2[COMPACT ? TRIPS : 1];
+	int2 H[COMPACT ? TRIPS : 1];
+	uint32_t NF[COMPACT ? TRIPS : 1];
+#if MULLS_LDS_KCERT
+	uint4 CR[COMPACT ? TRIPS : 1];
+#endif
 	const uint32_t last = d.src_off + (q_end ? q_end - 1u : 0u);
 #pragma unroll
 	for (int k = 0; k < TRIPS; k++)
@@ -590,9 +597,32 @@
 		FL[k] = flag[gi];
 		M[k] = nn_idx[gi];
 		D[k] = nn_d2[gi];
-		PM[k] = match[gi];
 		N1[k] = *reinterpret_cast<const float3 *>(snrm + gi);
-		T2[k] = *reinterpret_cast<const float3 *>(mq + 2u * gi + 1u);
+		if (COMPACT)
+		{
+			PM[k] = -1, T2[k] = make_float3(0.0f, 0.0f, 0.0f);
+			P4[COMPACT ? k : 0] = spos[gi];
+			H[COMPACT ? k : 0] = hint2[gi];
+#if MULLS_LDS_KCERT
+			CR[COMPACT ? k : 0] = C.cand ? C.cand[gi] : make_uint4(0u, 0u, 0u, 0u);
+#endif
+		}
+		else
+		{
+			PM[k] = match[gi];
+			T2[k] = *reinterpret_cast<const float3 *>(mq + 2u * gi + 1u);
+		}
+	}
+	if (COMPACT)
+	{
+#pragma unroll
+		for (int k = 0; k < TRIPS; k++)
+		{
+			asm volatile("" ::"v"(FL[k]), "v"(M[k]), "v"(D[k]), "v"(N1[k].x), "v"(P4[COMPACT ? k : 0].x), "v"(H[COMPACT ? k : 0].x));
+#if MULLS_LDS_KCERT
+			asm volatile("" ::"v"(CR[COMPACT ? k : 0].x));
+#endif
+		}
 	}
 	for (int off = 32; off > 0; off >>= 1)
 		matched_cnt += __shfl_down(matched_cnt, off);
@@ -609,12 +639,14 @@
 	for (int k = 0; k < TRIPS; k++)
 	{
 		const uint32_t s = threadIdx.x + (uint32_t)k * BLK, gi = d.src_off + s;
+		if (COMPACT)
+			NF[COMPACT ? k : 0] = 0u;
 		if (s >= q_end || !(FL[k] & MULLS_F_ALIVE))
 			continue;
 		int32_t m = M[k];
 		if (C.dedup && m >= 0 && !dedup_holds<W16>(W, (uint32_t)m, s))
 			m = -1;
-		bool alive = true, valid;
+		bool alive = true, valid, newrec = false;
 		float3 n2 = T2[k];
 		if (any_match)
 		{
@@ -630,14 +662,20 @@
 				valid = strict ? dist < max_sqr : !(dist > max_sqr);
 				if (valid)
 				{
-					wd[gi] = dist;
+					if (!COMPACT)
+						wd[gi] = dist;
 					if (PM[k] != m)
 					{
-						match[gi] = m;
 						float4 q2, n4;
 						tgt_record(rp.tgt_stage, rp.tgt_map, d, (uint32_t)m, tpos, tnrm, q2, n4);
-						mq[2u * gi] = q2;
-						mq[2u * gi + 1u] = n4;
+						if (COMPACT)
+							Q2[COMPACT ? k : 0] = q2, N2[COMPACT ? k : 0] = n4, newrec = true;
+						else
+						{
+							match[gi] = m;
+							mq[2u * gi] = q2;
+							mq[2u * gi + 1u] = n4;
+						}
 						n2 = make_float3(n4.x, n4.y, n4.z);
 					}
 				}
@@ -658,11 +696,28 @@
 				valid = false;
 		}
 		const uint32_t nf = (alive ? MULLS_F_ALIVE : 0u) | (valid ? MULLS_F_VALID : 0u);
-		if (nf != FL[k])
+		if (COMPACT)
+		{
+			NF[COMPACT ? k : 0] = nf | (newrec ? 8u : 0u);
+			M[k] = newrec ? m : PM[k];
+		}
+		else if (nf != FL[k])
 			flag[gi] = (uint8_t)nf;
 		n_alive += alive ? 1u : 0u;
 		n_valid += valid ? 1u : 0u;
 	}
+	uint32_t *words = red + 3 * (BLK / 64);
+	unsigned long long bal[COMPACT ? TRIPS : 1];
+	if (COMPACT)
+	{
+#pragma unroll
+		for (int k = 0; k < TRIPS; k++)
+		{
+			bal[COMPACT ? k : 0] = __ballot((NF[COMPACT ? k : 0] & MULLS_F_ALIVE) != 0u);
+			if ((threadIdx.x & 63) == 0)
+				words[k * (BLK / 64) + (threadIdx.x >> 6)] = (uint32_t)__popcll(bal[COMPACT ? k : 0]);
+		}
+	}
 	for (int off = 32; off > 0; off >>= 1)
 	{
 		n_alive += __shfl_down(n_alive, off);
@@ -674,6 +729,67 @@
 		red[2 * (BLK / 64) + (threadIdx.x >> 6)] = n_valid;
 	}
 	__syncthreads();
+	if (COMPACT)
+	{
+		const uint32_t lane = threadIdx.x & 63u, wave = threadIdx.x >> 6, src_off = d.src_off;
+		const unsigned long long below_me = (1ull << lane) - 1ull;
+		LiveWord *lw = rp.live_mask + live_word_base(d, job.pair * MULLS_NC + job.cls);
+		const uint32_t n_words = (q_end + 63u) >> 6;
+		uint32_t run = 0;
+#pragma unroll
+		for (int k = 0; k < TRIPS; k++)
+		{
+			uint32_t below = run;
+			for (int w = 0; w < BLK / 64; w++)
+			{
+				const uint32_t c = words[k * (BLK / 64) + w];
+				below += (uint32_t)w < wave ? c : 0u;
+				run += c;
+			}
+			const uint32_t word = (uint32_t)k * (BLK / 64) + wave;
+			if (lane == 0u && word < n_words)
+			{
+				LiveWord v;
+				v.alive = bal[COMPACT ? k : 0], v.below = below, v.pad_ = 0u;
+				lw[word] = v;
+			}
+			const uint32_t nf = NF[COMPACT ? k : 0];
+			if (nf & MULLS_F_ALIVE)
+			{
+				const uint32_t ci = src_off + below + (uint32_t)__popcll(bal[COMPACT ? k : 0] & below_me);
+				spos[ci] = P4[COMPACT ? k : 0];
+				*reinterpret_cast<float3 *>(snrm + ci) = N1[k];
+				hint2[ci] = H[COMPACT ? k : 0];
+#if MULLS_LDS_KCERT
+				if (C.cand)
+					C.cand[ci] = CR[COMPACT ? k : 0];
+#endif
+				flag[ci] = (uint8_t)(nf & (MULLS_F_ALIVE | MULLS_F_VALID));
+				match[ci] = M[k];
+				if (nf & MULLS_F_VALID)
+					wd[ci] = D[k];
+				if (nf & 8u)
+				{
+					mq[2u * ci] = Q2[COMPACT ? k : 0];
+					mq[2u * ci + 1u] = N2[COMPACT ? k : 0];
+				}
+			}
+		}
+#pragma unroll
+		for (int k = 0; k < TRIPS; k++)
+		{
+			const uint32_t s = threadIdx.x + (uint32_t)k * BLK;
+			if (s >= run && s < q_end)
+				flag[src_off + s] = 0u;
+		}
+		if (threadIdx.x == 0)
+		{
+			d.src_c = run;
+			d.compacted = 1u;
+			if (rp.dbg_ticks)
+				atomicAdd(&rp.dbg_ticks[5], (unsigned long long)(q_end - run));
+		}
+	}
 	if (threadIdx.x == 0)
 	{
 		uint32_t ta = 0, tv = 0;
@@ -872,7 +988,7 @@
 	uint32_t &ucount = CL.ucount;
 	int2 *__restrict__ hint2 = reinterpret_cast<int2 *>(nn_hint);
 
-	const uint32_t src_n = d.src_n, tgt_n = d.tgt_n;
+	const uint32_t src_n = d.src_c, tgt_n = d.tgt_n;
 	const bool called = class_called(rp, d, job.cls);
 	const ClassCtx C = class_ctx(rp, ps, g, job.cls, d.alive_cur, called);
 	const bool have_prev = ps.iter > 0;
@@ -1009,7 +1125,7 @@
 	uint32_t *us = CL.us, *red = CL.red;
 	uint32_t &ucount = CL.ucount;
 	int2 *__restrict__ hint2 = reinterpret_cast<int2 *>(nn_hint);
-	const uint32_t src_n = d.src_n, tgt_n = d.tgt_n;
+	const uint32_t src_n = d.src_c, tgt_n = d.tgt_n;
 	const ClassCtx C = class_ctx(rp, ps, g, job.cls, d.alive_cur, true);
 	const bool have_prev = ps.iter > 0;
 	const bool normal_check = job.cls != 5;
@@ -1357,8 +1473,8 @@
 }
 
 __device__ __forceinline__ void lds_search_class(const RunParams &rp, const PairState &ps, const Job &job, CloudDesc &d, const GridDesc &g,
-												  const LdsLayout &Y, unsigned char *lds_raw, const float4 *__restrict__ spos,
-												  const float4 *__restrict__ snrm, const uint32_t *__restrict__ cell_start,
+												  const LdsLayout &Y, unsigned char *lds_raw, float4 *spos,
+												  float4 *snrm, const uint32_t *__restrict__ cell_start,
 												  const float4 *__restrict__ tsorted, uint8_t *flag, int32_t *__restrict__ nn_idx, float *__restrict__ nn_d2,
 												  unsigned long long *__restrict__ winner, const float4 *__restrict__ tnrm, int32_t *__restrict__ match,
 												  float *__restrict__ wd, const float4 *__restrict__ tpos, int32_t *__restrict__ nn_hint, float4 *__restrict__ mq,
@@ -1380,7 +1496,7 @@
 	uint16_t *IDX = Y.IDX, *CS = Y.CS;
 	uint32_t *W = Y.W;
 	int2 *__restrict__ hint2 = reinterpret_cast<int2 *>(nn_hint);
-	const uint32_t src_n = d.src_n, tgt_n = d.tgt_n;
+	const uint32_t src_n = d.src_c, tgt_n = d.tgt_n;
 	const ClassCtx C = class_ctx(rp, ps, g, job.cls, d.alive_cur, true);
 	const uint32_t q_end = min(src_n, job.start + (job.count ? job.count : (uint32_t)MULLS_SRC_PER_BLOCK));
 	const uint32_t q_cnt = q_end > job.start ? q_end - job.start : 0u, n_chunks = (q_cnt + MULLS_LDS_QCHUNK - 1u) / MULLS_LDS_QCHUNK;
@@ -1533,7 +1649,12 @@
 	HEAVY_TICK(10)
 	uint32_t *red = reinterpret_cast<uint32_t *>(lds_raw);
 	if (rp.lds_dedup && rp.debug_stop != 9u && job.start == 0u && q_end <= 2u * MULLS_LDS_BLOCK)
-		class_tail_flat<MULLS_LDS_BLOCK, 2, false>(rp, ps, C, d, job, q_end, matched_cnt, searched, W, red, snrm, tnrm, flag, nn_idx, nn_d2, match, wd, tpos, mq);
+	{
+		if (first && rp.live_mask != nullptr && job.count >= d.src_n && d.src_n <= MULLS_COMPACT_MAX)
+			class_tail_flat<MULLS_LDS_BLOCK, 2, false, true>(rp, ps, C, d, job, q_end, matched_cnt, searched, W, red, snrm, tnrm, flag, nn_idx, nn_d2, match, wd, tpos, mq, spos, hint2);
+		else
+			class_tail_flat<MULLS_LDS_BLOCK, 2, false>(rp, ps, C, d, job, q_end, matched_cnt, searched, W, red, snrm, tnrm, flag, nn_idx, nn_d2, match, wd, tpos, mq);
+	}
 	else
 		class_tail<MULLS_LDS_BLOCK>(rp, ps, C, d, job, q_end, matched_cnt, searched, W, red, snrm, tnrm, flag, nn_idx, nn_d2, match, wd, winner, tpos, mq);
 	HEAVY_TICK(11)
diff --git a/mulls_amd/csrc/loop.cpp b/mulls_amd/csrc/loop.cpp
--- a/mulls_amd/csrc/loop.cpp
+++ b/mulls_amd/csrc/loop.cpp
@@ -108,6 +108,15 @@
 		rp.dbg_ticks = B->dbg;
 	}
 
+	if (dstep && rp.lds_dedup != 0u && (tier == 2 || tier == 3) && rp.debug_stop != 31u)
+	{
+		bool waves = true;
+		for (int k = 0; k < B->nsub; k++)
+			waves = waves && accum_takes_waves(rp, B->ajob_split[k], (uint32_t)ctx->opt[MULLS_OPT_ACCUM_WAVE_MIN_TRIPS]);
+		if (waves)
+			rp.live_mask = B->live_mask;
+	}
+
 	evt.begin(&ctx->prof.ms_setup);
 	queue_clone_crop(st, B, rp);
 	if (P->keep_less_source_points && !rp.undistort)
@@ -274,6 +283,7 @@
 			ctx->prof.icp_fused_ms[k] += (double)t[k] * 1e-5;
 		ctx->prof.icp_fused_ms[5] += (double)t[6];
 		ctx->prof.icp_search_ms[0] += (double)t[13], ctx->prof.icp_search_ms[1] += (double)t[14], ctx->prof.icp_search_ms[2] += (double)t[15], ctx->prof.icp_search_ms[3] += (double)t[7];
+		ctx->prof.icp_search_ms[4] += (double)t[5];
 		for (int k = 0; k < 4; k++)
 			ctx->prof.icp_phase_ms[k] += (double)t[8 + k] * 1e-5;
 		ctx->prof.icp_phase_ms[4] += (double)t[12];
```

Result: faster. 291,200, median of 6 (+6.5%).
